# ApricityXX/PaddlePaddle

Hardware: AMD Instinct MI355X
Metric: tokens/sec GPT-3-13B sharding-3 + ResNet50 img/s, at 1/2/4/8 MI355X (higher is better)
Workload: dtype bf16; 1 GPU; model=GPT-3 13B (h5120 L40 a40 ffn20480 V50304), global_batch=16, seq_len=2048, micro_batch=4, accum_steps=4, parallelism=sharding_stage3_degree1, recompute=False, fused_head_ce=False, paired_wgrad=False, optimizer=AdamW fp32-master fused HIP, amp=O2 bf16, allocator=native auto-growth best-fit

## Files before the change

### csrc/dispatch/dispatch_gen.inc

```
PA_ENTRY(pa_rms_norm_fwd, "ippppllfip")
PA_ENTRY(pa_rms_norm_bwd, "ippppppllip")
PA_ENTRY(pa_rms_norm_bwd_res, "ipppppppllip")
PA_ENTRY(pa_layer_norm_fwd, "ippppppllfip")
PA_ENTRY(pa_layer_norm_bwd, "ipppppppppllip")
PA_ENTRY(pa_reduce_parts, "ippppiliip")
PA_ENTRY(pa_softmax_fwd, "ippllip")
PA_ENTRY(pa_softmax_bwd, "ipppllip")
PA_ENTRY(pa_softmax_ce_fwd, "ipppplllip")
PA_ENTRY(pa_softmax_ce_bwd, "ippppplllip")
PA_ENTRY(pa_ce_slice_fwd, "ipppplllip")
PA_ENTRY(pa_ce_slice_bwd, "ipppppllllip")
PA_ENTRY(pa_gelu_fwd, "ippliip")
PA_ENTRY(pa_gelu_bwd, "ipppliip")
PA_ENTRY(pa_swiglu_fwd, "ippplllip")
PA_ENTRY(pa_swiglu_bwd, "ippppplllip")
PA_ENTRY(pa_bias_gelu_fwd, "ipppllip")
PA_ENTRY(pa_rope_fwd, "ipppplllliip")
PA_ENTRY(pa_rope_rows, "iplpppllllliip")
PA_ENTRY(pa_adamw_multi, "ipplpfffffffpp")
PA_ENTRY(pa_adam_hyper_step, "ipffp")
PA_ENTRY(pa_sq_norm_multi, "ipplpp")
PA_ENTRY(pa_write_i64, "ipplp")
PA_ENTRY(pa_bn_set_target_wgs, "ii")
PA_ENTRY(pa_momentum_multi, "ipplpfffip")
PA_ENTRY(pa_multi_tensor_chunk, "l")
PA_ENTRY(pa_lamb_multi, "ipplplpppffffffip")
PA_ENTRY(pa_amp_check_unscale_multi, "ipplppp")
PA_ENTRY(pa_flash_attn_set_fwd_variant, "ii")
PA_ENTRY(pa_flash_attn_fwd, "ippppppiiiiiifip")
PA_ENTRY(pa_flash_attn_bwd, "ippppppppppppiiiiiifip")
PA_ENTRY(pa_flash_attn_fwd_ex, "ippppppiiiiiifipp")
PA_ENTRY(pa_flash_attn_bwd_ex, "ippppppppppppiiiiiifilpp")
PA_ENTRY(pa_flash_attn_bwd_ds, "ippppppppppppiiiiiifipp")
PA_ENTRY(pa_flash_attn_bwd_ds_ok, "iiiiii")
PA_ENTRY(pa_flash_attn_bwd_ds_bytes, "liiii")
PA_ENTRY(pa_fa_fm_stats, "ipiiiiillipp")
PA_ENTRY(pa_paged_decode_attn, "ippppppppiiiiiiillfp")
PA_ENTRY(pa_colsum, "ipppllip")
PA_ENTRY(pa_dwconv_fwd, "ipppppip")
PA_ENTRY(pa_dwconv_dgrad, "ipppppip")
PA_ENTRY(pa_dwconv_wgrad_parts, "ipp")
PA_ENTRY(pa_dwconv_wgrad, "ippppip")
PA_ENTRY(pa_gemm_bf16, "ippppplllllliiifiip")
PA_ENTRY(pa_gemm_bf16_pp, "ippppplllllliiifpp")
PA_ENTRY(pa_gemm_bf16_4w, "ippppplllllliiifpp")
PA_ENTRY(pa_gemm_bf16_res, "ippppplllllliipp")
PA_ENTRY(pa_gemm_bf16_dgelu, "ippppplllllliiip")
PA_ENTRY(pa_gemm_bf16_pp_segs, "ipiipppplllllliiifpp")
PA_ENTRY(pa_gemm_pp_ws_bytes, "llll")
PA_ENTRY(pa_gemm_pp_splitk_ws_bytes, "llli")
PA_ENTRY(pa_gemm_bf16_pp_splitk, "ippplllllliiifipp")
PA_ENTRY(pa_gemm_fp8, "ipppplllllliifiip")
PA_ENTRY(pa_gemm_fp8_set_kernel, "ii")
PA_ENTRY(pa_gemm_fp8_ws, "ipppplllllliifiipp")
PA_ENTRY(pa_gemm_fp8_ws_bytes, "llll")
PA_ENTRY(pa_gemm_fp8_dscale, "ipppplllllliifiipppp")
PA_ENTRY(pa_fp8_nparts, "l")
PA_ENTRY(pa_fp8_amax, "iplipp")
PA_ENTRY(pa_fp8_scale_update, "ipipippfiip")
PA_ENTRY(pa_fp8_quant, "iplliippppp")
PA_ENTRY(pa_gemm_bf16_4w_abl, "ippplllip")
PA_ENTRY(pa_gemm_small_m, "iplplplppiiiiip")
PA_ENTRY(pa_gemm_skinny, "ipppplllllliip")
PA_ENTRY(pa_wo_gemm, "ippppppppiiiiiiiip")
PA_ENTRY(pa_wo_gemm_splits, "illli")
PA_ENTRY(pa_wo_dequant, "ipppiiiip")
PA_ENTRY(pa_gemm_skinny_ok, "ill")
PA_ENTRY(pa_gemm_skinny_stats_chunks, "llll")
PA_ENTRY(pa_gemm_skinny_stats, "ippppllllllipp")
PA_ENTRY(pa_conv_skinny_stats_chunks, "llll")
PA_ENTRY(pa_conv_skinny_stats, "ippppplllpp")
PA_ENTRY(pa_conv_skinny, "ippppplllllllllllp")
PA_ENTRY(pa_conv_skinny_ok, "illll")
PA_ENTRY(pa_conv_skinny_wgrad, "ippppllllllp")
PA_ENTRY(pa_conv2d_nhwc_fwd, "ipppppiiiiiiiiiiiiip")
PA_ENTRY(pa_conv3d_ndhwc_fwd, "ipppppiiiiiiiiiiiiiiiiip")
PA_ENTRY(pa_conv2d_nhwc_fwd_stats, "ipppppiiiiiiiiiiiiipp")
PA_ENTRY(pa_gemm_stats_chunks, "ili")
PA_ENTRY(pa_slab_reduce_bf16, "ipplllip")
PA_ENTRY(pa_gemm_bf16_bnbwd, "ippplllllliiippppp")
PA_ENTRY(pa_conv2d_nhwc_fwd_bnbwd, "ippppiiiiiiiiiiiiippppp")
PA_ENTRY(pa_gemm_bf16_stats, "ipppplllllliiiipp")
PA_ENTRY(pa_conv2d_nhwc_wgrad, "ippppiiiiiiiiiiiiiiip")
PA_ENTRY(pa_bias_gelu_bwd, "ippppppllip")
PA_ENTRY(pa_dropout_add_fwd, "ippplfuip")
PA_ENTRY(pa_dropout_bwd, "ipplfuip")
PA_ENTRY(pa_dropout_bwd_colsum, "ipppllfuip")
PA_ENTRY(pa_colsum_nparts, "ll")
PA_ENTRY(pa_fold_partials, "ippllip")
PA_ENTRY(pa_bn_chunks, "ili")
PA_ENTRY(pa_bn_fwd_nhwc, "ipppppppppppliffiip")
PA_ENTRY(pa_bn_bwd_nhwc, "ippppppppppppliiipp")
PA_ENTRY(pa_bn_reduce_nhwc, "iipppppppliip")
PA_ENTRY(pa_bn_fwd_nhwc_mask, "ippppppppppppliffip")
PA_ENTRY(pa_bn_bwd_nhwc_mask, "ippppppppppppliip")
PA_ENTRY(pa_bn_bwd_apply_nhwc, "ippppppliipp")
PA_ENTRY(pa_bn_pre_ws, "lii")
PA_ENTRY(pa_bn_bwd_nhwc_pre, "ipppppppppippliipp")
PA_ENTRY(pa_bn_fwd_nhwc_pre, "ippppppppppipppliffip")
PA_ENTRY(pa_add_rms_norm_fwd, "ipppppllfip")
PA_ENTRY(pa_decode_rope_cache, "iplppppppiiiilip")
PA_ENTRY(pa_maxpool_nhwc_fwd, "ipppiiiiiiiiiip")
PA_ENTRY(pa_maxpool_nhwc_bwd, "ipppiiiiiiiiiip")
PA_ENTRY(pa_grouped_gemm, "iippppppiliiilllip")
PA_ENTRY(pa_moe_route, "ipiipppp")
PA_ENTRY(pa_version, "i")
```

### csrc/kernels/gemm.hip

```cpp
#include "common.h"
#include "gemm_plan.h"
#include "launch.h"
#include "mfma_tile.h"

#include <type_traits>

using namespace pa;

namespace {

constexpr int kBM = 256;
constexpr int kBK = 64;
constexpr int kThreads = 512;

enum EpiFlags : int {
  kEpiBias = 1,
  kEpiGelu = 2,
  kEpiAux = 4,
  kEpiAccum = 8,
  kEpiOutF32 = 16,
  kEpiStats = 32,
  kEpiStatsBwd = 64,
  kEpiGeluBwd = 128,
  kEpiColSum = 256,
// ... 246 lines not shown
#pragma unroll
    for (int i = 0; i < MR; ++i) {
      const int m = mrow0 + i * 16;
      if (m >= p.M) continue;
      float v[4];
#pragma unroll
      for (int e = 0; e < 4; ++e) v[e] = acc[i][j][e] * p.alpha + bv[e];
      const int64_t off = (int64_t)m * p.ldc + n;
      if (flags & kEpiAux) {
        *reinterpret_cast<uint2*>(p.aux + off) = make_uint2(pack_bf16(v[0], v[1]), pack_bf16(v[2], v[3]));
      }
      if (flags & kEpiGelu) {
#pragma unroll
        for (int e = 0; e < 4; ++e) v[e] = gelu_tanh(v[e]);
      }
      if (flags & kEpiOutF32) {
        float4* cp = reinterpret_cast<float4*>(reinterpret_cast<float*>(p.c) + off);
        if (flags & kEpiAccum) {
          const float4 o = *cp;
          v[0] += o.x; v[1] += o.y; v[2] += o.z; v[3] += o.w;
        }
        *cp = make_float4(v[0], v[1], v[2], v[3]);
      } else {
        uint2* cp = reinterpret_cast<uint2*>(reinterpret_cast<uint16_t*>(p.c) + off);
        if (flags & kEpiAccum) {
          const uint2 o = *cp;
          v[0] += lo_bf16(o.x); v[1] += hi_bf16(o.x); v[2] += lo_bf16(o.y); v[3] += hi_bf16(o.y);
        }
        const uint2 o = make_uint2(pack_bf16(v[0], v[1]), pack_bf16(v[2], v[3]));
        *cp = o;
        if (flags & kEpiStatsBwd) {
          stats_add_bwd(p, off, o, bsc, bsh, bmu, s1, s2);
        } else if (flags & kEpiStats) {
          stats_add2(o.x, s1, s2, 0);
          stats_add2(o.y, s1, s2, 2);
        }
      }
    }
    if (flags & kEpiStats) stats_store(p, tm * 2 + wm, p.tiles_m * 2, n, lane, s1, s2);
  }
}

constexpr int kEpiRowStride = 260;
constexpr int kEpiRowStrideBf16 = 264;

using H0_ = IntC<0>;
using H1_ = IntC<1>;
using H2_ = IntC<2>;
using H3_ = IntC<3>;
using True_ = IntC<1>;
using False_ = IntC<0>;

template <int NT>
__device__ __forceinline__ void epi_rows(const GemmArgs& p, const float* img, int m_base, int n0, int tid,
                                         const float* bv, float* cs) {
  constexpr int RS = kEpiRowStride;
  constexpr int RSTEP = NT / 32;
  constexpr int NSTEP = 128 / RSTEP;
  constexpr int G = 4;
  const int ec = (tid & 31) * 8, er = tid / 32;
  const int n = n0 + ec;
  if (n >= p.N) return;
  const int flags = p.flags;
  const bool f32 = flags & kEpiOutF32;
  const bool rd_pre = flags & kEpiGeluBwd, rd_res = (flags & kEpiResid) && !rd_pre;
  const bool rd_c = (flags & kEpiAccum) && !rd_pre && !rd_res;
#pragma unroll 1
  for (int g0 = 0; g0 < NSTEP; g0 += G) {
    uint4 rd[G][2];
    if (rd_pre || rd_res || rd_c) {
#pragma unroll
      for (int s = 0; s < G; ++s) {
        const int m = m_base + (g0 + s) * RSTEP + er;
        rd[s][0] = rd[s][1] = make_uint4(0u, 0u, 0u, 0u);
        if (m < p.M) {
          const int64_t off = (int64_t)m * p.ldc + n;
          if (rd_pre) {
            rd[s][0] = *reinterpret_cast<const uint4*>(p.aux + off);
          } else if (rd_res) {
            rd[s][0] = *reinterpret_cast<const uint4*>(p.res + off);
          } else if (f32) {
            rd[s][0] = *reinterpret_cast<const uint4*>(reinterpret_cast<const float*>(p.c) + off);
            rd[s][1] = *reinterpret_cast<const uint4*>(reinterpret_cast<const float*>(p.c) + off + 4);
          } else {
            rd[s][0] = *reinterpret_cast<const uint4*>(reinterpret_cast<const uint16_t*>(p.c) + off);
          }
        }
      }
    }
#pragma unroll
    for (int s = 0; s < G; ++s) {
      const int r = (g0 + s) * RSTEP + er;
      const int m = m_base + r;
      if (m >= p.M) break;
      float v[8];
      const f32x4 lo = *reinterpret_cast<const f32x4*>(img + r * RS + ec);
      const f32x4 hi = *reinterpret_cast<const f32x4*>(img + r * RS + ec + 4);
#pragma unroll
      for (int e = 0; e < 4; ++e) {
        v[e] = lo[e] * p.alpha + bv[e];
        v[4 + e] = hi[e] * p.alpha + bv[4 + e];
      }
      const int64_t off = (int64_t)m * p.ldc + n;
      if (flags & kEpiAux) store8<bf16>(reinterpret_cast<bf16*>(p.aux + off), v);
      if (flags & kEpiGelu) {
#pragma unroll
        for (int e = 0; e < 8; ++e) v[e] = gelu_tanh(v[e]);
      }
      float o[8];
      if (rd_pre || rd_res || (rd_c && !f32)) {
        const uint4 u = rd[s][0];
        o[0] = lo_bf16(u.x); o[1] = hi_bf16(u.x); o[2] = lo_bf16(u.y); o[3] = hi_bf16(u.y);
        o[4] = lo_bf16(u.z); o[5] = hi_bf16(u.z); o[6] = lo_bf16(u.w); o[7] = hi_bf16(u.w);
      } else if (rd_c) {
        const uint4 u0 = rd[s][0], u1 = rd[s][1];
        o[0] = __uint_as_float(u0.x); o[1] = __uint_as_float(u0.y); o[2] = __uint_as_float(u0.z);
        o[3] = __uint_as_float(u0.w); o[4] = __uint_as_float(u1.x); o[5] = __uint_as_float(u1.y);
        o[6] = __uint_as_float(u1.z); o[7] = __uint_as_float(u1.w);
      }
      if (rd_pre) {
#pragma unroll
        for (int e = 0; e < 8; ++e) v[e] *= gelu_tanh_grad_fast(o[e]);
      } else if (rd_c || rd_res) {
#pragma unroll
        for (int e = 0; e < 8; ++e) v[e] += o[e];
      }
      if (flags & kEpiColSum) {
#pragma unroll
        for (int e = 0; e < 8; ++e) cs[e] += v[e];
      }
      if (f32) store8<float>(reinterpret_cast<float*>(p.c) + off, v);
      else store8<bf16>(reinterpret_cast<bf16*>(reinterpret_cast<uint16_t*>(p.c) + off), v);
    }
  }
}

template <int NT>
__device__ __forceinline__ void colsum_finish(const GemmArgs& p, float* red, const float* cs, int tid, int m0,
                                              int n0) {
  constexpr int R = NT / 32;
  const int ec = (tid & 31) * 8, er = tid / 32;
  __syncthreads();
  *reinterpret_cast<float4*>(red + er * 256 + ec) = make_float4(cs[0], cs[1], cs[2], cs[3]);
  *reinterpret_cast<float4*>(red + er * 256 + ec + 4) = make_float4(cs[4], cs[5], cs[6], cs[7]);
  __syncthreads();
  for (int c = tid; c < 256; c += NT) {
    float s = 0.f;
#pragma unroll
    for (int r = 0; r < R; ++r) s += red[r * 256 + c];
    if (n0 + c < p.N) p.stats[(int64_t)(m0 >> 8) * p.N + n0 + c] = s;
  }
}

template <bool AK, bool BKM, int SEG = 0>
__global__ __launch_bounds__(kThreads, 1) void gemm256_kernel(GemmArgs p0) {
  GemmArgs p = split_view<AK, BKM>(p0);
  constexpr int HALF = 128 * kBK * 2;
  constexpr int STAGE = 4 * HALF;
  extern __shared__ __attribute__((aligned(16))) char smem[];

  const int tid = threadIdx.x, wave = tid >> 6, lane = tid & 63;
  const int wm = wave >> 2, wn = wave & 3;

  const int bid = (int)blockIdx.x;
  int pid;
  float* tail_out = nullptr;
  int kt0 = 0;
  if (p.tail_split > 0 && bid >= p.full_tiles) {
    const int u = bid - p.full_tiles;
    const int ks = u % p.tail_split;
    pid = p.full_tiles + u / p.tail_split;
    p.K /= p.tail_split;
    if constexpr (SEG == 0) {
      p.a += (int64_t)ks * p.K * (AK ? 1 : p.lda);
      p.b += (int64_t)ks * p.K * (BKM ? 1 : p.ldb);
    } else {
      kt0 = ks * (p.K / kBK);
    }
    tail_out = p.tail_ws + (int64_t)u * 65536;
  } else {
    pid = xcd_remap(bid, p.tail_split > 0 ? p.full_tiles : p.tiles_m * p.tiles_n);
  }
  int tm, tn;
  tile_coords(pid, p.tiles_m, p.tiles_n, &tm, &tn);
  const int m0 = tm * 256, n0 = tn * 256;
  const int nk = p.K / kBK;

  auto stage_half = [&](int t, int h, char* dst) {
    const int tg = SEG == 0 ? t : kt0 + t;
    int k0 = tg * kBK;
    const uint16_t* a = p.a;
    const uint16_t* b = p.b;
    int64_t lda = p.lda, ldb = p.ldb;
    if constexpr (SEG == 1) {
      const int s = seg_of(p, tg);
      k0 = (tg - pick4(s, 0, p.seg_end[0], p.seg_end[1], p.seg_end[2])) * kBK;
      a = pick4(s, p.seg_a[0], p.seg_a[1], p.seg_a[2], p.seg_a[3]);
      b = pick4(s, p.seg_b[0], p.seg_b[1], p.seg_b[2], p.seg_b[3]);
      lda = pick4(s, p.seg_lda[0], p.seg_lda[1], p.seg_lda[2], p.seg_lda[3]);
      ldb = pick4(s, p.seg_ldb[0], p.seg_ldb[1], p.seg_ldb[2], p.seg_ldb[3]);
    }
    if (h == 0 || h == 2) {
      stage<128, AK>(a, lda, m0 + (h == 2 ? 128 : 0), p.M, k0, dst, wave, lane);
    } else {
      int c0 = n0 + (h == 3 ? 128 : 0), cmax = p.N;
      if constexpr (SEG == 2) {
        const int s = seg_of(p, c0);
        const int start = pick4(s, 0, p.seg_end[0], p.seg_end[1], p.seg_end[2]);
        b = pick4(s, p.seg_b[0], p.seg_b[1], p.seg_b[2], p.seg_b[3]);
        ldb = pick4(s, p.seg_ldb[0], p.seg_ldb[1], p.seg_ldb[2], p.seg_ldb[3]);
        cmax = pick4(s, p.seg_end[0], p.seg_end[1], p.seg_end[2], p.seg_end[3]) - start;
        c0 -= start;
      }
      stage<128, BKM>(b, ldb, c0, cmax, k0, dst, wave, lane);
    }
  };
  auto issue = [&](int j) {
    const int t = j >> 2, h = j & 3;
    stage_half(t, h, smem + (t & 1) * STAGE + h * HALF);
  };
  auto issue_h = [&](int t, auto hc) {
    constexpr int h = decltype(hc)::value;
    stage_half(t, h, smem + (t & 1) * STAGE + h * HALF);
  };

  f32x4 acc[2][4][2][2];
#pragma unroll
  for (int a = 0; a < 2; ++a)
#pragma unroll
    for (int i = 0; i < 4; ++i)
#pragma unroll
      for (int b = 0; b < 2; ++b)
#pragma unroll
        for (int j = 0; j < 2; ++j) acc[a][i][b][j] = f32x4{0.f, 0.f, 0.f, 0.f};

  const int last_j = 4 * nk - 1;
  auto wait_for = [&](int phase, int jstar) {
    const int issued = min(phase + 6, last_j);
    vm_wait(2 * max(issued - jstar, 0));
  };
  const int npro = min(6, 4 * nk);
#pragma unroll 1
  for (int j = 0; j < npro; ++j) issue(j);
  vm_wait(2 * max(min(5, last_j) - 1, 0));
  bar();
  const bool lag = __builtin_amdgcn_readfirstlane(wm) == 1;
  if (lag) bar();

  bf16x8_t af[4][2], bl[2][2], br[2][2];
  const int ar = wm * 64, bc = wn * 32;

  auto ktile = [&](int t, auto steady) {
    constexpr bool S = decltype(steady)::value;
    const char* buf = smem + (t & 1) * STAGE;
    const int ph = 4 * t;
#pragma unroll
    for (int ks = 0; ks < 2; ++ks)
#pragma unroll
      for (int j = 0; j < 2; ++j) bl[j][ks] = frag<128, BKM>(buf + HALF, bc + j * 16, ks, lane);
#pragma unroll
    for (int ks = 0; ks < 2; ++ks)
#pragma unroll
      for (int i = 0; i < 4; ++i) af[i][ks] = frag<128, AK>(buf, ar + i * 16, ks, lane);
    if (S) {
      issue_h(t + 1, H2_{});
      asm volatile("s_waitcnt vmcnt(6)" ::: "memory");
    } else {
      if (ph + 6 <= last_j) issue(ph + 6);
      wait_for(ph, ph + 3);
    }
    bar();
    __builtin_amdgcn_s_setprio(1);
#pragma unroll
    for (int ks = 0; ks < 2; ++ks)
#pragma unroll
      for (int i = 0; i < 4; ++i)
#pragma unroll
        for (int j = 0; j < 2; ++j)
          acc[0][i][0][j] = __builtin_amdgcn_mfma_f32_16x16x32_bf16(bl[j][ks], af[i][ks], acc[0][i][0][j], 0, 0, 0);
    __builtin_amdgcn_s_setprio(0);
    bar();
#pragma unroll
    for (int ks = 0; ks < 2; ++ks)
#pragma unroll
      for (int j = 0; j < 2; ++j) br[j][ks] = frag<128, BKM>(buf + 3 * HALF, bc + j * 16, ks, lane);
    if (S) {
      issue_h(t + 1, H3_{});
      asm volatile("s_waitcnt vmcnt(10)" ::: "memory");
    } else {
      if (ph + 7 <= last_j) issue(ph + 7);
      wait_for(ph + 1, ph + 2);
    }
    bar();
    __builtin_amdgcn_s_setprio(1);
#pragma unroll
    for (int ks = 0; ks < 2; ++ks)
#pragma unroll
      for (int i = 0; i < 4; ++i)
#pragma unroll
        for (int j = 0; j < 2; ++j)
          acc[0][i][1][j] = __builtin_amdgcn_mfma_f32_16x16x32_bf16(br[j][ks], af[i][ks], acc[0][i][1][j], 0, 0, 0);
    __builtin_amdgcn_s_setprio(0);
    bar();
#pragma unroll
    for (int ks = 0; ks < 2; ++ks)
#pragma unroll
      for (int i = 0; i < 4; ++i) af[i][ks] = frag<128, AK>(buf + 2 * HALF, ar + i * 16, ks, lane);
    if (S) issue_h(t + 2, H0_{});
    else if (ph + 8 <= last_j) issue(ph + 8);
    bar();
    __builtin_amdgcn_s_setprio(1);
#pragma unroll
    for (int ks = 0; ks < 2; ++ks)
#pragma unroll
      for (int i = 0; i < 4; ++i)
#pragma unroll
        for (int j = 0; j < 2; ++j)
          acc[1][i][0][j] = __builtin_amdgcn_mfma_f32_16x16x32_bf16(bl[j][ks], af[i][ks], acc[1][i][0][j], 0, 0, 0);
    __builtin_amdgcn_s_setprio(0);
    bar();
    if (S) {
// ... 409 lines not shown
    const uint16_t* src =
        ok ? p.a + ((int64_t)(cr.pix[i] + (di * p.cH + hi) * p.cW + wi) * p.cC + c0 + lc * 8) : p.zero + lc * 8;
    glds16(src, img + q * 1024);
  }
}

template <bool AK, bool BKM, bool CONV = false>
__global__ __launch_bounds__(kThreads, 1) void gemm3s_kernel(GemmArgs p0) {
  const GemmArgs p = split_view<AK, BKM>(p0);
  constexpr int BN = kBN3;
  constexpr int A_BYTES = kBM * kBK * 2;
  constexpr int B_BYTES = BN * kBK * 2;
  constexpr int STAGE = A_BYTES + B_BYTES;
  constexpr int MR = 4, NR = 5;
  constexpr int NL = (kBM / 8 + 7) / 8 + (BN / 8 + 7) / 8;
  extern __shared__ __attribute__((aligned(16))) char smem[];

  const int tid = threadIdx.x, wave = tid >> 6, lane = tid & 63;
  const int wm = wave >> 1, wn = wave & 1;

  const int nwg = p.tiles_m * p.tiles_n;
  const int pid = xcd_remap((int)blockIdx.x, nwg);
  constexpr int GM = 8;
  const int per_group = GM * p.tiles_n;
  const int gid = pid / per_group;
  const int first_m = gid * GM;
  const int gsz = min(p.tiles_m - first_m, GM);
  const int tm = first_m + (pid % per_group) % gsz;
  const int tn = (pid % per_group) / gsz;
  const int m0 = tm * kBM, n0 = tn * BN;

  f32x4 acc[MR][NR];
#pragma unroll
  for (int i = 0; i < MR; ++i)
#pragma unroll
    for (int j = 0; j < NR; ++j) acc[i][j] = f32x4{0.f, 0.f, 0.f, 0.f};

  const int nk = p.K / kBK;
  ConvRows cr;
  if constexpr (CONV) cr = conv_rows(p, m0, wave, lane);
  auto stage_tile = [&](int t) {
    char* base = smem + (t % 3) * STAGE;
    if constexpr (CONV) stage_conv(p, cr, t * kBK, base, wave, lane);
    else stage_r<kBM, AK>(p.a, p.lda, m0, p.M, t * kBK, base, wave, lane);
    stage_r<BN, BKM>(p.b, p.ldb, n0, p.N, t * kBK, base + A_BYTES, wave, lane);
  };

  stage_tile(0);
  if (nk > 1) {
    stage_tile(1);
    asm volatile("s_waitcnt vmcnt(%0)" ::"n"(NL) : "memory");
  } else {
    asm volatile("s_waitcnt vmcnt(0)" ::: "memory");
  }
  bar();

#pragma unroll 1
  for (int t = 0; t < nk; ++t) {
    const bool pre = t + 2 < nk;
    if (pre) stage_tile(t + 2);
    const char* aimg = smem + (t % 3) * STAGE;
    const char* bimg = aimg + A_BYTES;
#pragma unroll
    for (int s = 0; s < 2; ++s) {
      bf16x8_t bf[NR];
#pragma unroll
      for (int j = 0; j < NR; ++j) bf[j] = frag_r<BN, BKM>(bimg, wn * 80 + j * 16, s, lane);
#pragma unroll
      for (int i = 0; i < MR; ++i) {
        const bf16x8_t af = frag_r<kBM, AK>(aimg, wm * 64 + i * 16, s, lane);
#pragma unroll
        for (int j = 0; j < NR; ++j)
          acc[i][j] = __builtin_amdgcn_mfma_f32_16x16x32_bf16(bf[j], af, acc[i][j], 0, 0, 0);
      }
    }
    if (pre) asm volatile("s_waitcnt vmcnt(%0)" ::"n"(NL) : "memory");
    else asm volatile("s_waitcnt vmcnt(0)" ::: "memory");
    bar();
  }

  const int flags = p.flags;
  const int mrow0 = m0 + wm * 64 + (lane & 15);
  const int ncol0 = n0 + wn * 80 + 4 * (lane >> 4);
#pragma unroll
  for (int j = 0; j < NR; ++j) {
    const int n = ncol0 + j * 16;
    if (n >= p.N) continue;
    float s1[4] = {0.f, 0.f, 0.f, 0.f}, s2[4] = {0.f, 0.f, 0.f, 0.f};
    float bsc[4] = {0.f, 0.f, 0.f, 0.f}, bsh[4] = {0.f, 0.f, 0.f, 0.f}, bmu[4] = {0.f, 0.f, 0.f, 0.f};
    if (flags & kEpiStatsBwd) bn_cols(p, n, bsc, bsh, bmu);
    float bv[4] = {0.f, 0.f, 0.f, 0.f};
    if (flags & kEpiBias) {
      const uint2 braw = *reinterpret_cast<const uint2*>(p.bias + n);
      bv[0] = lo_bf16(braw.x); bv[1] = hi_bf16(braw.x); bv[2] = lo_bf16(braw.y); bv[3] = hi_bf16(braw.y);
    }
#pragma unroll
    for (int i = 0; i < MR; ++i) {
      const int m = mrow0 + i * 16;
      if (m >= p.M) continue;
      float v[4];
#pragma unroll
      for (int e = 0; e < 4; ++e) v[e] = acc[i][j][e] * p.alpha + bv[e];
      const int64_t off = (int64_t)m * p.ldc + n;
      if (flags & kEpiAux)
        *reinterpret_cast<uint2*>(p.aux + off) = make_uint2(pack_bf16(v[0], v[1]), pack_bf16(v[2], v[3]));
      if (flags & kEpiGelu) {
#pragma unroll
        for (int e = 0; e < 4; ++e) v[e] = gelu_tanh(v[e]);
      }
      if (flags & kEpiOutF32) {
        float4* cp = reinterpret_cast<float4*>(reinterpret_cast<float*>(p.c) + off);
        if (flags & kEpiAccum) {
          const float4 o = *cp;
          v[0] += o.x; v[1] += o.y; v[2] += o.z; v[3] += o.w;
        }
        *cp = make_float4(v[0], v[1], v[2], v[3]);
      } else {
        uint2* cp = reinterpret_cast<uint2*>(reinterpret_cast<uint16_t*>(p.c) + off);
        if (flags & kEpiAccum) {
          const uint2 o = *cp;
          v[0] += lo_bf16(o.x); v[1] += hi_bf16(o.x); v[2] += lo_bf16(o.y); v[3] += hi_bf16(o.y);
        }
        const uint2 o = make_uint2(pack_bf16(v[0], v[1]), pack_bf16(v[2], v[3]));
        *cp = o;
        if (flags & kEpiStatsBwd) {
          stats_add_bwd(p, off, o, bsc, bsh, bmu, s1, s2);
        } else if (flags & kEpiStats) {
          stats_add2(o.x, s1, s2, 0);
          stats_add2(o.y, s1, s2, 2);
        }
      }
    }
    if (flags & kEpiStats) stats_store(p, tm * 4 + wm, p.tiles_m * 4, n, lane, s1, s2);
  }
}


template <class F>
int with_layout(int a_kmajor, int b_kmajor, F&& f) {
  if (a_kmajor && !b_kmajor) return f(std::true_type{}, std::false_type{});
  if (a_kmajor && b_kmajor) return f(std::true_type{}, std::true_type{});
  if (!a_kmajor && !b_kmajor) return f(std::false_type{}, std::false_type{});
  return f(std::false_type{}, std::true_type{});
}

template <bool AK, bool BKM, bool CONV = false>
int launch3s(GemmArgs a, int splits, hipStream_t st) {
  a.tiles_m = (a.M + kBM - 1) / kBM;
  a.tiles_n = (a.N + kBN3 - 1) / kBN3;
  constexpr int smem = 3 * (kBM + kBN3) * kBK * 2;
  return launch_lds<gemm3s_kernel<AK, BKM, CONV>>(dim3(a.tiles_m * a.tiles_n, splits), dim3(kThreads), smem, st, a);
}

template <bool AK, bool BKM, int SEG>
int launch256_seg(GemmArgs a, int splits, hipStream_t st, int grid) {
  a.tiles_m = (a.M + 255) / 256;
  a.tiles_n = (a.N + 255) / 256;
  if (!grid) {
    grid = a.tiles_m * a.tiles_n;
    a.tail_split = 0;
  }
  constexpr int kLoop = 2 * 4 * 128 * kBK * 2, kEpi0 = 128 * kEpiRowStride * 4, kEpi1 = 256 * kEpiRowStrideBf16 * 2;
  constexpr int kEpi = kEpi0 > kEpi1 ? kEpi0 : kEpi1;
  constexpr int smem = kLoop > kEpi ? kLoop : kEpi;
  return launch_lds<gemm256_kernel<AK, BKM, SEG>>(dim3(grid, splits), dim3(kThreads), smem, st, a);
}

template <bool AK, bool BKM>
int launch256(const GemmArgs& a0, int splits, hipStream_t st, int grid = 0, int seg = 0) {
  if (seg == 1) return launch256_seg<AK, BKM, 1>(a0, splits, st, grid);
  if (seg == 2) return launch256_seg<AK, BKM, 2>(a0, splits, st, grid);
  return launch256_seg<AK, BKM, 0>(a0, splits, st, grid);
}

template <bool AK, bool BKM>
int launch4w(const GemmArgs& g, int grid, hipStream_t st) {
  constexpr int kLoop = 4 * 2 * 256 * 32 * 2, kEpi = 128 * kEpiRowStride * 4;
  constexpr int smem = kLoop > kEpi ? kLoop : kEpi;
  return launch_lds<gemm4w_kernel<AK, BKM>>(dim3(grid), dim3(256), smem, st, g);
}

template <int BN, bool AK, bool BKM>
int launch(const GemmArgs& a0, int splits, hipStream_t st) {
  if constexpr (BN == 0) return launch256<AK, BKM>(a0, splits, st);
  if constexpr (BN == 160) return launch3s<AK, BKM>(a0, splits, st);
  GemmArgs a = a0;
  constexpr int NW = BN == 4 ? 4 : 8;
  constexpr int BNk = (BN == 0 || BN == 4) ? 256 : BN;
  a.tiles_m = (a.M + kBM - 1) / kBM;
  a.tiles_n = (a.N + BNk - 1) / BNk;
  constexpr int smem = 2 * (kBM + BNk) * kBK * 2;
  return launch_lds<gemm_bf16_kernel<BNk, AK, BKM, NW>>(dim3(a.tiles_m * a.tiles_n, splits), dim3(NW * 64), smem, st,
                                                        a);
}

int launch_bn(const GemmArgs& g, int bn, int a_kmajor, int b_kmajor, int splits, hipStream_t st) {
  return with_layout(a_kmajor, b_kmajor, [&](auto ak, auto bk) {
    constexpr bool AK = decltype(ak)::value, BKM = decltype(bk)::value;
    if (bn == 160) return launch<160, AK, BKM>(g, splits, st);
    if (bn == 128) return launch<128, AK, BKM>(g, splits, st);
    if (bn == 1) return launch<0, AK, BKM>(g, splits, st);
    if (bn == 4) return launch<4, AK, BKM>(g, splits, st);
    return launch<256, AK, BKM>(g, splits, st);
  });
}

constexpr int kSmBM = 64, kSmBN = 128, kSmNW = 4;

template <int kSmStages>
__global__ __launch_bounds__(kSmNW * 64, 1) void gemm_small_m_kernel(const uint16_t* __restrict__ a, int64_t lda,
                                                                    const uint16_t* __restrict__ b, int64_t ldb,
                                                                    float* __restrict__ ws, int M, int N, int k_per,
                                                                    const uint16_t* __restrict__ bias,
                                                                    uint16_t* __restrict__ c, int64_t ldc) {
  constexpr int A_BYTES = kSmBM * kBK * 2, B_BYTES = kSmBN * kBK * 2, STAGE = A_BYTES + B_BYTES;
  constexpr int NL = kSmBM / (8 * kSmNW) + kSmBN / (8 * kSmNW);
  extern __shared__ __attribute__((aligned(16))) char smem[];
  const int tid = threadIdx.x, wave = tid >> 6, lane = tid & 63;
  const int n0 = blockIdx.x * kSmBN;
  const int ks = blockIdx.y;
  const uint16_t* ap = a + (int64_t)ks * k_per;
  const uint16_t* bp = b + (int64_t)ks * k_per * ldb;
  const int nk = k_per / kBK;

  f32x4 acc[4][2];
#pragma unroll
  for (int i = 0; i < 4; ++i) acc[i][0] = acc[i][1] = f32x4{0.f, 0.f, 0.f, 0.f};

  auto stage_tile = [&](int t) {
    char* base = smem + (t % kSmStages) * STAGE;
    stage<kSmBM, true, kSmNW>(ap, lda, 0, M, t * kBK, base, wave, lane);
    stage<kSmBN, false, kSmNW>(bp, ldb, n0, N, t * kBK, base + A_BYTES, wave, lane);
  };
  const int pro = min(kSmStages - 1, nk);
  for (int t = 0; t < pro; ++t) stage_tile(t);
  if (pro >= 3) asm volatile("s_waitcnt vmcnt(%0)" ::"n"(2 * NL) : "memory");
  else if (pro == 2) asm volatile("s_waitcnt vmcnt(%0)" ::"n"(NL) : "memory");
  else asm volatile("s_waitcnt vmcnt(0)" ::: "memory");
  bar();

#pragma unroll 1
  for (int t = 0; t < nk; ++t) {
    if (t + kSmStages - 1 < nk) stage_tile(t + kSmStages - 1);
    const char* aimg = smem + (t % kSmStages) * STAGE;
    const char* bimg = aimg + A_BYTES;
#pragma unroll
    for (int s = 0; s < 2; ++s) {
      bf16x8_t bf[2];
#pragma unroll
      for (int j = 0; j < 2; ++j) bf[j] = frag<kSmBN, false>(bimg, wave * 32 + j * 16, s, lane);
#pragma unroll
      for (int i = 0; i < 4; ++i) {
        const bf16x8_t af = frag<kSmBM, true>(aimg, i * 16, s, lane);
#pragma unroll
        for (int j = 0; j < 2; ++j) acc[i][j] = __builtin_amdgcn_mfma_f32_16x16x32_bf16(bf[j], af, acc[i][j], 0, 0, 0);
      }
    }
    const int after = min(nk - 1, t + kSmStages - 1) - (t + 1);
    if (after >= 2) asm volatile("s_waitcnt vmcnt(%0)" ::"n"(2 * NL) : "memory");
    else if (after == 1) asm volatile("s_waitcnt vmcnt(%0)" ::"n"(NL) : "memory");
    else asm volatile("s_waitcnt vmcnt(0)" ::: "memory");
    bar();
  }
  if (gridDim.y == 1) {
#pragma unroll
    for (int i = 0; i < 4; ++i) {
      const int m = i * 16 + (lane & 15);
      if (m >= M) continue;
#pragma unroll
      for (int j = 0; j < 2; ++j) {
        const int n = n0 + wave * 32 + j * 16 + 4 * (lane >> 4);
        if (n >= N) continue;
        float v[4] = {acc[i][j][0], acc[i][j][1], acc[i][j][2], acc[i][j][3]};
        if (bias) {
          const uint2 braw = *reinterpret_cast<const uint2*>(bias + n);
          v[0] += lo_bf16(braw.x); v[1] += hi_bf16(braw.x); v[2] += lo_bf16(braw.y); v[3] += hi_bf16(braw.y);
        }
        *reinterpret_cast<uint2*>(c + (int64_t)m * ldc + n) = make_uint2(pack_bf16(v[0], v[1]), pack_bf16(v[2], v[3]));
      }
    }
    return;
  }
  float* out = ws + (int64_t)ks * M * N;
#pragma unroll
  for (int i = 0; i < 4; ++i) {
    const int m = i * 16 + (lane & 15);
    if (m >= M) continue;
#pragma unroll
    for (int j = 0; j < 2; ++j) {
      const int n = n0 + wave * 32 + j * 16 + 4 * (lane >> 4);
      if (n < N)
        *reinterpret_cast<float4*>(out + (int64_t)m * N + n) =
            make_float4(acc[i][j][0], acc[i][j][1], acc[i][j][2], acc[i][j][3]);
    }
  }
}

__global__ __launch_bounds__(256) void gemm_small_m_reduce_k(const float* __restrict__ ws, const uint16_t* __restrict__ bias,
                                                            uint16_t* __restrict__ c, int64_t ldc, int M, int N,
                                                            int splits) {
  const int64_t i4 = ((int64_t)blockIdx.x * 256 + threadIdx.x) * 4;
  if (i4 >= (int64_t)M * N) return;
  const int m = (int)(i4 / N), n = (int)(i4 % N);
  float4 acc = *reinterpret_cast<const float4*>(ws + i4);
  for (int s = 1; s < splits; ++s) {
    const float4 v = *reinterpret_cast<const float4*>(ws + (int64_t)s * M * N + i4);
    acc.x += v.x; acc.y += v.y; acc.z += v.z; acc.w += v.w;
  }
  if (bias) {
    const uint2 braw = *reinterpret_cast<const uint2*>(bias + n);
    acc.x += lo_bf16(braw.x); acc.y += hi_bf16(braw.x); acc.z += lo_bf16(braw.y); acc.w += hi_bf16(braw.y);
  }
  *reinterpret_cast<uint2*>(c + (int64_t)m * ldc + n) = make_uint2(pack_bf16(acc.x, acc.y), pack_bf16(acc.z, acc.w));
}

__global__ __launch_bounds__(256) void gemm_tail_reduce_k(GemmArgs p) {
  const int b = blockIdx.x;
  int tm, tn;
  tile_coords(p.full_tiles + b, p.tiles_m, p.tiles_n, &tm, &tn);
  const int e = (blockIdx.y * 256 + threadIdx.x) * 4;
  const int r = e >> 8, c = e & 255;
  const int m = tm * 256 + r, n = tn * 256 + c;
  if (m >= p.M || n >= p.N) return;
  const float* src = p.tail_ws + (int64_t)b * p.tail_split * 65536 + e;
  float4 a = *reinterpret_cast<const float4*>(src);
  for (int k = 1; k < p.tail_split; ++k) {
    const float4 v = *reinterpret_cast<const float4*>(src + (int64_t)k * 65536);
    a.x += v.x; a.y += v.y; a.z += v.z; a.w += v.w;
  }
  const int flags = p.flags;
  float bv[4] = {0.f, 0.f, 0.f, 0.f};
  if (flags & kEpiBias) {
    const uint2 braw = *reinterpret_cast<const uint2*>(p.bias + n);
    bv[0] = lo_bf16(braw.x); bv[1] = hi_bf16(braw.x); bv[2] = lo_bf16(braw.y); bv[3] = hi_bf16(braw.y);
  }
  float v[4] = {a.x * p.alpha + bv[0], a.y * p.alpha + bv[1], a.z * p.alpha + bv[2], a.w * p.alpha + bv[3]};
  const int64_t off = (int64_t)m * p.ldc + n;
  if (flags & kEpiAux)
    *reinterpret_cast<uint2*>(p.aux + off) = make_uint2(pack_bf16(v[0], v[1]), pack_bf16(v[2], v[3]));
  if (flags & kEpiGelu) {
#pragma unroll
    for (int q = 0; q < 4; ++q) v[q] = gelu_tanh(v[q]);
  }
  if (flags & kEpiResid) {
    const uint2 rr = *reinterpret_cast<const uint2*>(p.res + off);
    v[0] += lo_bf16(rr.x); v[1] += hi_bf16(rr.x); v[2] += lo_bf16(rr.y); v[3] += hi_bf16(rr.y);
  }
  if (flags & kEpiOutF32) {
    float4* cp = reinterpret_cast<float4*>(reinterpret_cast<float*>(p.c) + off);
    if (flags & kEpiAccum) {
      const float4 o = *cp;
      v[0] += o.x; v[1] += o.y; v[2] += o.z; v[3] += o.w;
    }
    *cp = make_float4(v[0], v[1], v[2], v[3]);
  } else {
    uint2* cp = reinterpret_cast<uint2*>(reinterpret_cast<uint16_t*>(p.c) + off);
    if (flags & kEpiAccum) {
      const uint2 o = *cp;
      v[0] += lo_bf16(o.x); v[1] += hi_bf16(o.x); v[2] += lo_bf16(o.y); v[3] += hi_bf16(o.y);
    }
    *cp = make_uint2(pack_bf16(v[0], v[1]), pack_bf16(v[2], v[3]));
  }
}

bool gemm_args(GemmArgs& g, const void* a, const void* b, void* c, const void* bias, void* aux, int64_t M, int64_t N,
               int64_t K, int64_t lda, int64_t ldb, int64_t ldc, int a_kmajor, int flags, float alpha) {
  if (!gemm_operands_ok(M, N, K, kBK, lda, ldb, ldc, a_kmajor != 0)) return false;
  g = GemmArgs{};
  g.a = (const uint16_t*)a; g.b = (const uint16_t*)b; g.c = c;
  g.bias = (const uint16_t*)bias; g.aux = (uint16_t*)aux;
  g.lda = lda; g.ldb = ldb; g.ldc = ldc;
  g.M = (int)M; g.N = (int)N; g.K = (int)K;
  g.flags = flags; g.alpha = alpha;
  return true;
}

void set_conv_geometry(GemmArgs& g, const void* zero, int D, int H, int W, int C, int Do, int Ho, int Wo, int KH,
                       int KW, int stride, int pad_d, int pad_h, int pad_w, int dil) {
  g.zero = (const uint16_t*)zero;
  g.cD = D; g.cDo = Do; g.cKHW = KH * KW; g.cPadD = pad_d;
  g.cH = H; g.cW = W; g.cC = C; g.cHo = Ho; g.cWo = Wo; g.cKW = KW; g.cStride = stride; g.cPadH = pad_h;
  g.cPadW = pad_w; g.cDil = dil;
}

int run_tile256(int kern, GemmArgs g, int a_kmajor, int b_kmajor, void* ws, hipStream_t st, int seg = 0,
                int force_split = 0) {
  if (g.M <= 0 || g.N <= 0 || g.K <= 0) return 0;
  TailPlan pl = force_split ? split_all_plan(g.M, g.N, force_split) : tail_plan(g.M, g.N, g.K, kBK, device_cus());
  if (!ws) pl = without_tail(pl);
  if (!force_split) g.c_split = (int64_t)g.M * g.ldc;
  g.tiles_m = (g.M + 255) / 256;
  g.tiles_n = (g.N + 255) / 256;
  g.full_tiles = pl.full_tiles;
  g.tail_split = pl.split;
  g.tail_ws = (float*)ws;
  const int rc = with_layout(a_kmajor, b_kmajor, [&](auto ak, auto bk) {
    constexpr bool AK = decltype(ak)::value, BKM = decltype(bk)::value;
    return kern == 2 ? launch4w<AK, BKM>(g, pl.grid, st) : launch256<AK, BKM>(g, 1, st, pl.grid, seg);
  });
  if (rc || !pl.split) return rc;
  hipLaunchKernelGGL(gemm_tail_reduce_k, dim3(pl.tiles - pl.full_tiles, 64), dim3(256), 0, st, g);
  return (int)hipGetLastError();
}

bool conv_fwd_args(GemmArgs& g, const void* x, const void* w, const void* bias, void* out, const void* zero, int N,
                   int D, int H, int W, int C, int Cout, int KD, int KH, int KW, int stride, int pad_d, int pad_h,
                   int pad_w, int dil, int Do, int Ho, int Wo, int flags) {
  if (C % kBK != 0 || Cout % 8 != 0 || N <= 0) return false;
  const int64_t K = (int64_t)KD * KH * KW * C;
  if (!gemm_args(g, x, w, out, bias, nullptr, (int64_t)N * Do * Ho * Wo, Cout, K, C, K, Cout, 1,
                 flags | (bias ? kEpiBias : 0), 1.f))
    return false;
  set_conv_geometry(g, zero, D, H, W, C, Do, Ho, Wo, KH, KW, stride, pad_d, pad_h, pad_w, dil);
  return true;
}

}

PA_EXPORT int64_t pa_gemm_pp_ws_bytes(int64_t M, int64_t N, int64_t K) {
  return tail_plan(M, N, K, kBK, device_cus()).ws_bytes;
}

PA_EXPORT int pa_gemm_bf16_pp(const void* a, const void* b, void* c, const void* bias, void* aux, int64_t M, int64_t N,
                              int64_t K, int64_t lda, int64_t ldb, int64_t ldc, int a_kmajor, int b_kmajor, int flags,
                              float alpha, void* ws, hipStream_t st) {
  GemmArgs g;
  if (!gemm_args(g, a, b, c, bias, aux, M, N, K, lda, ldb, ldc, a_kmajor, flags, alpha)) return 1;
  return run_tile256(1, g, a_kmajor, b_kmajor, ws, st);
}

PA_EXPORT int64_t pa_gemm_pp_splitk_ws_bytes(int64_t M, int64_t N, int splits) {
  return split_all_plan(M, N, splits).ws_bytes;
}

PA_EXPORT int pa_gemm_bf16_pp_splitk(const void* a, const void* b, void* c, int64_t M, int64_t N, int64_t K,
                                     int64_t lda, int64_t ldb, int64_t ldc, int a_kmajor, int b_kmajor, int flags,
                                     float alpha, int splits, void* ws, hipStream_t st) {
  if (splits < 1 || (K / kBK) % splits != 0 || !ws || (flags & ~(kEpiOutF32 | kEpiAccum))) return 1;
  GemmArgs g;
  if (!gemm_args(g, a, b, c, nullptr, nullptr, M, N, K, lda, ldb, ldc, a_kmajor, flags, alpha)) return 1;
  return run_tile256(1, g, a_kmajor, b_kmajor, ws, st, 0, splits);
}

PA_EXPORT int pa_gemm_bf16_pp_segs(const int64_t* seg, int nseg, int seg_k, const void* a, const void* b, void* c,
                                   const void* bias, int64_t M, int64_t N, int64_t K, int64_t lda, int64_t ldb,
                                   int64_t ldc, int a_kmajor, int b_kmajor, int flags, float alpha, void* ws,
                                   hipStream_t st) {
  if (nseg < 1 || nseg > 4 || (flags & (kEpiAux | kEpiStats))) return 1;
  GemmArgs g;
  if (!gemm_args(g, a, b, c, bias, nullptr, M, N, K, 0, 0, ldc, a_kmajor, flags, alpha)) return 1;
  if (M <= 0 || N <= 0) return 0;
  if (seg_k ? (flags & kEpiBias) != 0 : lda % 8 != 0) return 1;
  g.lda = lda; g.ldb = ldb;
  g.nseg = nseg; g.seg_k = seg_k;
  int64_t prev = 0;
  for (int s = 0; s < 4; ++s) {
    const int64_t* e = seg + 5 * (s < nseg ? s : nseg - 1);
    g.seg_a[s] = (const uint16_t*)e[0];
    g.seg_b[s] = (const uint16_t*)e[1];
    g.seg_lda[s] = e[2];
    g.seg_ldb[s] = e[3];
    if (s < nseg) {
      const int64_t end = e[4];
      if (end <= prev || e[2] % 8 != 0 || e[3] % 8 != 0) return 1;
      if (seg_k ? (end % kBK != 0) : (end % 128 != 0 && s + 1 < nseg)) return 1;
      g.seg_end[s] = (int)(seg_k ? end / kBK : end);
      prev = end;
    } else {
      g.seg_end[s] = g.seg_end[nseg - 1];
    }
  }
  if (seg_k ? prev != K : prev != N) return 1;
  return run_tile256(1, g, a_kmajor, b_kmajor, ws, st, nseg > 1 ? (seg_k ? 1 : 2) : 0);
}

PA_EXPORT int pa_gemm_bf16_4w(const void* a, const void* b, void* c, const void* bias, void* aux, int64_t M, int64_t N,
                              int64_t K, int64_t lda, int64_t ldb, int64_t ldc, int a_kmajor, int b_kmajor, int flags,
                              float alpha, void* ws, hipStream_t st) {
  GemmArgs g;
  if (!gemm_args(g, a, b, c, bias, aux, M, N, K, lda, ldb, ldc, a_kmajor, flags, alpha)) return 1;
  return run_tile256(2, g, a_kmajor, b_kmajor, ws, st);
}

PA_EXPORT int pa_gemm_bf16_res(const void* a, const void* b, void* c, const void* bias, const void* res, int64_t M,
                               int64_t N, int64_t K, int64_t lda, int64_t ldb, int64_t ldc, int a_kmajor, int b_kmajor,
                               void* ws, hipStream_t st) {
  if (!res || res == c) return 1;
  GemmArgs g;
  if (!gemm_args(g, a, b, c, bias, nullptr, M, N, K, lda, ldb, ldc, a_kmajor, (bias ? kEpiBias : 0) | kEpiResid, 1.f))
    return 1;
  g.res = (const uint16_t*)res;
  return run_tile256(1, g, a_kmajor, b_kmajor, ws, st);
}

PA_EXPORT int pa_gemm_bf16_dgelu(const void* a, const void* b, void* dh, const void* pre, float* colsum, int64_t M,
                                 int64_t N, int64_t K, int64_t lda, int64_t ldb, int64_t ldc, int a_kmajor,
                                 int b_kmajor, int kern, hipStream_t st) {
  if (!pre || !colsum || kern < 1 || kern > 2) return 1;
  GemmArgs g;
  if (!gemm_args(g, a, b, dh, nullptr, const_cast<void*>(pre), M, N, K, lda, ldb, ldc, a_kmajor,
                 kEpiGeluBwd | kEpiColSum, 1.f))
    return 1;
  g.stats = colsum;
  return run_tile256(kern, g, a_kmajor, b_kmajor, nullptr, st);
}

PA_EXPORT int pa_gemm_bf16_4w_abl(const void* a, const void* b, void* c, int64_t M, int64_t N, int64_t K, int abl,
                                  hipStream_t st) {
  GemmArgs g;
  if (N % 256 || M % 256 || !gemm_args(g, a, b, c, nullptr, nullptr, M, N, K, K, N, N, 1, 0, 1.f)) return 1;
  g.tiles_m = (int)(M / 256); g.tiles_n = (int)(N / 256);
  g.full_tiles = g.tiles_m * g.tiles_n;
  if (abl >= 6 && abl <= 8) {
    if (abl != 7) g.lda = 0;
    if (abl != 8) g.ldb = 0;
  }
  constexpr int smem = 128 * kEpiRowStride * 4;
  const dim3 grid(g.full_tiles), block(256);
  if (abl == 1) return launch_lds<gemm4w_kernel<true, false, 1>>(grid, block, smem, st, g);
  if (abl == 2) return launch_lds<gemm4w_kernel<true, false, 2>>(grid, block, smem, st, g);
  if (abl == 3) return launch_lds<gemm4w_kernel<true, false, 3>>(grid, block, smem, st, g);
  if (abl == 5) return launch_lds<gemm4w_kernel<true, false, 5>>(grid, block, smem, st, g);
  if (abl == 4) return launch_lds<gemm4w_kernel<true, false, 0, 5>>(grid, block, 5 * 32768, st, g);
  return launch_lds<gemm4w_kernel<true, false, 0>>(grid, block, smem, st, g);
}

PA_EXPORT int pa_gemm_bf16(const void* a, const void* b, void* c, const void* bias, void* aux, int64_t M, int64_t N,
                           int64_t K, int64_t lda, int64_t ldb, int64_t ldc, int a_kmajor, int b_kmajor, int flags,
                           float alpha, int bn, int splits, hipStream_t st) {
  if (splits < 1) splits = 1;
  if (K % splits != 0) return 1;
  if (splits > 1 && (flags & (kEpiBias | kEpiGelu | kEpiAux | kEpiAccum))) return 1;
  if (splits > 1 && !(flags & kEpiOutF32)) return 1;
  GemmArgs g;
  if (!gemm_args(g, a, b, c, bias, aux, M, N, K / splits, lda, ldb, ldc, a_kmajor, flags, alpha)) return 1;
  if (M <= 0 || N <= 0 || K <= 0) return 0;
  g.c_split = M * ldc;
  return launch_bn(g, bn, a_kmajor, b_kmajor, splits, st);
}

PA_EXPORT int pa_conv3d_ndhwc_fwd(const void* x, const void* w, const void* bias, void* out, const void* zero, int N,
                                  int D, int H, int W, int C, int Cout, int KD, int KH, int KW, int stride, int pad_d,
                                  int pad_h, int pad_w, int dil, int Do, int Ho, int Wo, hipStream_t st) {
  GemmArgs g;
  if (!conv_fwd_args(g, x, w, bias, out, zero, N, D, H, W, C, Cout, KD, KH, KW, stride, pad_d, pad_h, pad_w, dil, Do,
                     Ho, Wo, 0))
    return 1;
  return launch3s<true, true, true>(g, 1, st);
}

PA_EXPORT int pa_gemm_stats_chunks(int64_t M, int bn) { return (int)((M + kBM - 1) / kBM) * (bn == 160 ? 4 : 2); }

PA_EXPORT int pa_gemm_bf16_stats(const void* a, const void* b, void* c, const void* bias, int64_t M, int64_t N,
                                 int64_t K, int64_t lda, int64_t ldb, int64_t ldc, int a_kmajor, int b_kmajor,
                                 int flags, int bn, float* stats, hipStream_t st) {
  if (!stats || (flags & (kEpiOutF32 | kEpiGelu | kEpiAux))) return 1;
  if (bn != 160 && bn != 256 && bn != 128 && bn != 4) return 1;
  GemmArgs g;
  if (!gemm_args(g, a, b, c, bias, nullptr, M, N, K, lda, ldb, ldc, a_kmajor, flags | kEpiStats, 1.f)) return 1;
  if (M <= 0 || N <= 0 || K <= 0) return 0;
  g.c_split = M * ldc;
  g.stats = stats;
  return launch_bn(g, bn, a_kmajor, b_kmajor, 1, st);
}

PA_EXPORT int pa_gemm_bf16_bnbwd(const void* a, const void* b, void* c, int64_t M, int64_t N, int64_t K, int64_t lda,
                                 int64_t ldb, int64_t ldc, int a_kmajor, int b_kmajor, int bn, const void* bn_x,
                                 const float* bn_ss, const float* bn_mean, float* stats, hipStream_t st) {
  if (!stats || !bn_x || !bn_ss || !bn_mean) return 1;
  if (bn != 160 && bn != 256 && bn != 128 && bn != 4) return 1;
  GemmArgs g;
  if (!gemm_args(g, a, b, c, nullptr, nullptr, M, N, K, lda, ldb, ldc, a_kmajor, kEpiStats | kEpiStatsBwd, 1.f))
    return 1;
  if (M <= 0 || N <= 0 || K <= 0) return 0;
  g.c_split = M * ldc;
  g.stats = stats;
  g.bn_x = (const uint16_t*)bn_x; g.bn_ss = bn_ss; g.bn_mean = bn_mean;
  return launch_bn(g, bn, a_kmajor, b_kmajor, 1, st);
}

PA_EXPORT int pa_conv2d_nhwc_fwd(const void* x, const void* w, const void* bias, void* out, const void* zero, int N,
// ... 117 lines not shown
```

### csrc/kernels/gemm_plan.h

```cpp
#pragma once
#include <climits>
#include <cstdint>

namespace pa {

struct TailPlan {
  int tiles, full_tiles, split, grid;
  int64_t ws_bytes;
};

inline TailPlan make_tail_plan(int64_t tiles, int64_t full, int split) {
  const int64_t tail = split ? tiles - full : 0;
  return {(int)tiles, (int)(tiles - tail), split, (int)(tiles - tail + tail * split), tail * split * 65536 * 4};
}

inline int64_t tiles256(int64_t M, int64_t N) { return ((M + 255) / 256) * ((N + 255) / 256); }

inline TailPlan tail_plan(int64_t M, int64_t N, int64_t K, int k_tile, int cus) {
  const int64_t T = tiles256(M, N);
  const int64_t nk = K / k_tile;
  const int64_t r = T > cus ? T % cus : 0;
  if (r == 0 || 2 * r > cus) return make_tail_plan(T, T, 0);
  int sp = 1;
  while (r * sp * 2 <= cus && nk % (sp * 2) == 0 && nk / (sp * 2) >= 4) sp *= 2;
  return sp == 1 ? make_tail_plan(T, T, 0) : make_tail_plan(T, T - r, sp);
}

inline TailPlan split_all_plan(int64_t M, int64_t N, int splits) { return make_tail_plan(tiles256(M, N), 0, splits); }

inline TailPlan without_tail(const TailPlan& p) { return make_tail_plan(p.tiles, p.tiles, 0); }

inline bool gemm_operands_ok(int64_t M, int64_t N, int64_t K, int k_tile, int64_t lda, int64_t ldb, int64_t ldc,
                             bool a_kmajor) {
  if (M > INT_MAX || N > INT_MAX || K > INT_MAX) return false;
  if (K % k_tile != 0 || N % 8 != 0 || lda % 8 != 0 || ldb % 8 != 0 || ldc % 4 != 0) return false;
  return a_kmajor || M % 8 == 0;
}

}
```

### csrc/kernels/mfma_tile.h

```cpp
#pragma once
#include "common.h"

namespace pa {

typedef __attribute__((ext_vector_type(8))) __bf16 bf16x8_t;
typedef __attribute__((ext_vector_type(4))) float f32x4;
typedef __attribute__((ext_vector_type(4))) short s16x4;
typedef __attribute__((ext_vector_type(4))) int i32x4;
typedef __attribute__((ext_vector_type(4))) unsigned int u32x4;

union Frag8 {
  bf16x8_t v;
  uint4 u;
  u32x4 w;
  s16x4 h[2];
};

__device__ __forceinline__ void glds16(const void* g, const char* lds_wave_base) {
  const uint32_t m0 = __builtin_amdgcn_readfirstlane((uint32_t)reinterpret_cast<uintptr_t>(lds_wave_base));
  asm volatile("s_mov_b32 m0, %1\n\ts_nop 0\n\tglobal_load_lds_dwordx4 %0, off" ::"v"(g), "s"(m0) : "memory", "m0");
}
__device__ __forceinline__ void glds4(const void* g, const char* lds_wave_base) {
  const uint32_t m0 = __builtin_amdgcn_readfirstlane((uint32_t)reinterpret_cast<uintptr_t>(lds_wave_base));
  asm volatile("s_mov_b32 m0, %1\n\ts_nop 0\n\tglobal_load_lds_dword %0, off" ::"v"(g), "s"(m0) : "memory", "m0");
}

__device__ __forceinline__ s16x4 lds_tr(const char* p) {
  return __builtin_amdgcn_ds_read_tr16_b64_v4i16(
      (__attribute__((address_space(3))) s16x4*)(reinterpret_cast<uintptr_t>(p)));
}

__device__ __forceinline__ void bar() {
  asm volatile("" ::: "memory");
  __builtin_amdgcn_s_barrier();
  asm volatile("" ::: "memory");
  __builtin_amdgcn_sched_barrier(0);
}

__device__ __forceinline__ void vm_wait(int n) {
  switch (n) {
    case 0: asm volatile("s_waitcnt vmcnt(0)" ::: "memory"); break;
    case 2: asm volatile("s_waitcnt vmcnt(2)" ::: "memory"); break;
    case 4: asm volatile("s_waitcnt vmcnt(4)" ::: "memory"); break;
    case 6: asm volatile("s_waitcnt vmcnt(6)" ::: "memory"); break;
    case 8: asm volatile("s_waitcnt vmcnt(8)" ::: "memory"); break;
    case 10: asm volatile("s_waitcnt vmcnt(10)" ::: "memory"); break;
    default: asm volatile("s_waitcnt vmcnt(0)" ::: "memory"); break;
  }
}

constexpr __host__ __device__ __forceinline__ int k_swz(int row) { return (row >> 1) & 7; }
constexpr __host__ __device__ __forceinline__ int k32_swz(int row) { return ((row >> 3) & 1) << 1; }
constexpr __host__ __device__ __forceinline__ int mn_swz(int k) { return ((k & 3) | (((k >> 3) & 1) << 2)) << 1; }
template <int R>
constexpr __host__ __device__ __forceinline__ int mn_swz_r(int k) { return mn_swz(k) & (R / 8 - 1); }

template <int R>
constexpr bool mn_swz_ok() {
  for (int k = 0; k < 64; ++k) {
    const int s = mn_swz_r<R>(k);
    if (s % 2 != 0 || (R >= 128 && s != mn_swz(k))) return false;
    for (int c = 0; c < R / 8; ++c)
      if ((c ^ s) >= R / 8) return false;
  }
  return true;
}
static_assert(mn_swz_ok<64>() && mn_swz_ok<128>() && mn_swz_ok<256>(), "MN-major swizzle");

template <int R, bool KMAJ, int NW = 8, class T>
__device__ __forceinline__ void stage(const T* __restrict__ g, int64_t ld, int r0, int rmax, int k0, char* img,
                                      int wave, int lane) {
  constexpr int E = 16 / sizeof(T);
  constexpr int NQ = R / (8 * NW);
  static_assert(KMAJ || sizeof(T) == 2, "MN-major images hold 16-bit elements");
#pragma unroll
  for (int i = 0; i < NQ; ++i) {
    const int q = i * NW + wave;
    if constexpr (KMAJ) {
      const int row = q * 8 + (lane >> 3);
      const int lc = (lane & 7) ^ k_swz(row);
      int gr = r0 + row;
      gr = gr < rmax ? gr : rmax - 1;
      glds16(g + (int64_t)gr * ld + k0 + lc * E, img + q * 1024);
    } else {
      constexpr int CPR = R / 8;
      const int lin = q * 64 + lane;
      const int row = lin / CPR;
      const int lc = (lin % CPR) ^ mn_swz_r<R>(row);
      int gc = r0 + lc * 8;
      gc = gc < rmax ? gc : rmax - 8;
      glds16(g + (int64_t)(k0 + row) * ld + gc, img + q * 1024);
    }
  }
}

template <int R, bool KMAJ>
__device__ __forceinline__ bf16x8_t frag(const char* img, int rbase, int s, int lane) {
  Frag8 f;
  if constexpr (KMAJ) {
    const int row = rbase + (lane & 15);
    const int c = s * 4 + (lane >> 4);
    f.u = *reinterpret_cast<const uint4*>(img + row * 128 + ((c ^ k_swz(row)) << 4));
  } else {
    const int g = lane >> 4, i = lane & 15, q = i >> 2, pp = i & 3;
    const int col = rbase + pp * 4;
    const int lc = col >> 3, sub = (col & 7) * 2;
    const int k1 = s * 32 + g * 8 + q, k2 = k1 + 4;
    f.h[0] = lds_tr(img + k1 * (R * 2) + ((lc ^ mn_swz_r<R>(k1)) << 4) + sub);
    f.h[1] = lds_tr(img + k2 * (R * 2) + ((lc ^ mn_swz_r<R>(k2)) << 4) + sub);
  }
  return f.v;
}

__device__ __forceinline__ int xcd_remap(int bid, int nwg) {
  const int xcd = bid & 7, q = nwg >> 3, r = nwg & 7;
  return (xcd < r ? xcd * (q + 1) : r * (q + 1) + (xcd - r) * q) + (bid >> 3);
}

__device__ __forceinline__ void tile_coords(int pid, int tiles_m, int tiles_n, int* tm, int* tn) {
  constexpr int GM = 8;
  const int per_group = GM * tiles_n;
  const int first_m = (pid / per_group) * GM;
  const int gsz = min(tiles_m - first_m, GM);
  *tm = first_m + (pid % per_group) % gsz;
  *tn = (pid % per_group) / gsz;
}

template <int V>
struct IntC {
  static constexpr int value = V;
};

}
```

### csrc/kernels/pa_api.h

```cpp
#pragma once
#include <cstdint>

#include <hip/hip_runtime_api.h>

#define PA_EXPORT extern "C" __attribute__((visibility("default")))

struct PaAttnExtra {
  const int* cu_q; const int* cu_k;
  const void* mask; int64_t mask_kind; int64_t ms[3];
  const int* fm; int64_t fm_cols; int64_t fms[2];
  const int* fm_stats; int64_t fmst[2];
  double drop_p; uint64_t seed;
  int64_t lse_s[2];
  int64_t dtype;
};

PA_EXPORT int pa_gelu_fwd(const void* x, void* y, int64_t n, int approx, int dtype, hipStream_t st);
PA_EXPORT int pa_gelu_bwd(const void* x, const void* dy, void* dx, int64_t n, int approx, int dtype, hipStream_t st);
PA_EXPORT int pa_bias_gelu_fwd(const void* x, const void* b, void* y, int64_t rows, int64_t cols, int dtype,
                               hipStream_t st);
PA_EXPORT int pa_swiglu_fwd(const void* a, const void* b, void* y, int64_t rows, int64_t cols, int64_t ld, int dtype,
                            hipStream_t st);
PA_EXPORT int pa_swiglu_bwd(const void* a, const void* b, const void* dy, void* da, void* db, int64_t rows,
                            int64_t cols, int64_t ld_packed, int dtype, hipStream_t st);
PA_EXPORT int pa_rope_fwd(const void* x, const float* cs, const float* sn, void* out, int64_t B, int64_t S, int64_t H,
                          int64_t D, int flags, int dtype, hipStream_t st);
PA_EXPORT int pa_rope_rows(const void* x, int64_t ldx, const float* cs, const float* sn, void* out, int64_t ldo,
                           int64_t rows, int64_t S, int64_t NH, int64_t D, int flags, int dtype, hipStream_t st);

PA_EXPORT int64_t pa_multi_tensor_chunk();
PA_EXPORT int pa_adamw_multi(const int64_t* table, const int64_t* items, int64_t n_items, const float* inv_scale,
                             float lr, float b1, float b2, float eps, float wd_unused, float bc1, float bc2,
                             const float* hyper, hipStream_t st);
PA_EXPORT int pa_adam_hyper_step(float* hyper, float b1, float b2, hipStream_t st);
PA_EXPORT int pa_sq_norm_multi(const int64_t* table, const int64_t* items, int64_t n_items, float* partial,
                               hipStream_t st);
PA_EXPORT int pa_momentum_multi(const int64_t* table, const int64_t* items, int64_t n_items, const float* inv_scale,
                                float lr, float mu, float rescale, int nesterov, hipStream_t st);
PA_EXPORT int pa_write_i64(int64_t* dst, const int64_t* src, int64_t n, hipStream_t st);

PA_EXPORT int pa_amp_check_unscale_multi(const int64_t* table, const int64_t* items, int64_t n_items,
                                         const float* inv_scale, float* found_inf, hipStream_t st);

PA_EXPORT int pa_bn_set_target_wgs(int n);
PA_EXPORT int pa_bn_chunks(int64_t R, int C);
PA_EXPORT int pa_bn_fwd_nhwc(const void* x, const void* res, void* y, const float* w, const float* b, float* run_mean,
                             float* run_var, float* save_mean, float* save_rstd, float* partial, float* ss, int64_t R,
                             int C, float momentum, float eps, int relu, int training, hipStream_t st);
PA_EXPORT int pa_bn_bwd_nhwc(const void* dy, const void* x, const void* y, void* dx, void* dres, const float* w,
                             const float* mean, const float* rstd, float* dw, float* db, float* partial, float* coef,
                             int64_t R, int C, int relu, int global_stats, const float* ss, hipStream_t st);
PA_EXPORT int pa_bn_fwd_nhwc_mask(const void* x, const void* res, void* y, const float* w, const float* b,
                                  float* run_mean, float* run_var, float* save_mean, float* save_rstd, float* partial,
                                  float* ss, void* mbits, int64_t R, int C, float momentum, float eps, int training,
                                  hipStream_t st);
PA_EXPORT int pa_bn_bwd_nhwc_mask(const void* dy, const void* x, const void* mbits, void* dx, void* dres,
                                  const float* w, const float* mean, const float* rstd, float* dw, float* db,
                                  float* partial, float* coef, int64_t R, int C, int global_stats, hipStream_t st);
PA_EXPORT int64_t pa_bn_pre_ws(int chunks, int C);
PA_EXPORT int pa_bn_fwd_nhwc_pre(const void* x, const void* res, void* y, const float* w, const float* b,
                                 float* run_mean, float* run_var, float* save_mean, float* save_rstd,
                                 const float* stats, int chunks, float* ws, float* ss, void* mbits, int64_t R, int C,
                                 float momentum, float eps, int relu, hipStream_t st);
PA_EXPORT int pa_bn_bwd_nhwc_pre(const void* dy, const void* x, void* dx, const float* w, const float* mean,
                                 const float* rstd, float* dw, float* db, const float* stats, int chunks, float* ws,
                                 float* coef, int64_t R, int C, int global_stats, const float* ss, hipStream_t st);
PA_EXPORT int pa_bn_reduce_nhwc(int mode, const void* x, const void* dy, const void* y, const float* mean,
                                const float* ss, float* partial, float* sums, int64_t R, int C, int relu,
                                hipStream_t st);
PA_EXPORT int pa_bn_bwd_apply_nhwc(const void* dy, const void* x, const void* y, const float* coef, void* dx,
                                   void* dres, int64_t R, int C, int relu, const float* ss, hipStream_t st);

PA_EXPORT int pa_paged_decode_attn(const void* q, const void* kc, const void* vc, const int* tables, const int* lens,
                                   float* part_o, float* part_ml, void* out, int N, int H, int Hkv, int D, int bs,
                                   int max_blocks, int splits, int64_t blk_stride, int64_t head_stride, float scale,
                                   hipStream_t st);

PA_EXPORT int pa_add_rms_norm_fwd(const void* x, const void* r, const void* w, void* s_out, void* y, int64_t rows,
                                  int64_t cols, float eps, int dtype, hipStream_t st);
PA_EXPORT int pa_decode_rope_cache(const void* qkv, int64_t ld, const float* cs, const float* sn, const int64_t* pos,
                                   void* q_out, void* kc, void* vc, int B, int H, int Hkv, int D, int64_t Lc,
                                   int dtype, hipStream_t st);

PA_EXPORT int pa_dwconv_fwd(const void* x, const void* wt, const void* bias, void* y, const int* shape, int dtype,
                            hipStream_t st);
PA_EXPORT int pa_dwconv_dgrad(const void* dy, const void* wt, const void* x, void* dx, const int* shape, int dtype,
                              hipStream_t st);
PA_EXPORT int pa_dwconv_wgrad_parts(const int* shape, int* out );
PA_EXPORT int pa_dwconv_wgrad(const void* x, const void* dy, float* part, const int* shape, int dtype,
                              hipStream_t st);

PA_EXPORT int pa_flash_attn_set_fwd_variant(int v);
PA_EXPORT int pa_flash_attn_fwd_ex(const void* q, const void* k, const void* v, void* o, float* lse,
                                   const int64_t* strides, int B, int Sq, int Sk, int H, int Hk, int D, float scale,
                                   int causal, const PaAttnExtra* ex, hipStream_t st);
PA_EXPORT int pa_flash_attn_fwd(const void* q, const void* k, const void* v, void* o, float* lse,
                                const int64_t* strides, int B, int Sq, int Sk, int H, int Hk, int D, float scale,
                                int causal, hipStream_t st);
PA_EXPORT int pa_flash_attn_bwd_ds_ok(int D, int has_mask, int has_fm, int dropout, int varlen);
PA_EXPORT int pa_flash_attn_bwd_ex(const void* q, const void* k, const void* v, const void* o, const void* dout,
                                   const float* lse, void* dq, void* dk, void* dv, float* dq_acc, float* delta,
                                   const int64_t* strides, int B, int Sq, int Sk, int H, int Hk, int D, float scale,
                                   int causal, int64_t q_rows, const PaAttnExtra* ex, hipStream_t st);
PA_EXPORT int64_t pa_flash_attn_bwd_ds_bytes(int B, int Sq, int Sk, int H);
PA_EXPORT int pa_flash_attn_bwd_ds(const void* q, const void* k, const void* v, const void* o, const void* dout,
                                   const float* lse, void* dq, void* dk, void* dv, void* ds, float* delta,
                                   const int64_t* strides, int B, int Sq, int Sk, int H, int Hk, int D, float scale,
                                   int causal, const PaAttnExtra* ex, hipStream_t st);
PA_EXPORT int pa_flash_attn_bwd(const void* q, const void* k, const void* v, const void* o, const void* dout,
                                const float* lse, void* dq, void* dk, void* dv, float* dq_acc, float* delta,
                                const int64_t* strides, int B, int Sq, int Sk, int H, int Hk, int D, float scale,
                                int causal, hipStream_t st);
PA_EXPORT int pa_fa_fm_stats(const int* fm, int cols, int causal, int Sk, int Bm, int Hm, int64_t sb, int64_t sh,
                             int ntiles, int* stats, hipStream_t st);

PA_EXPORT int64_t pa_gemm_pp_ws_bytes(int64_t M, int64_t N, int64_t K);
PA_EXPORT int pa_gemm_bf16_pp(const void* a, const void* b, void* c, const void* bias, void* aux, int64_t M,
                              int64_t N, int64_t K, int64_t lda, int64_t ldb, int64_t ldc, int a_kmajor, int b_kmajor,
                              int flags, float alpha, void* ws, hipStream_t st);
PA_EXPORT int64_t pa_gemm_pp_splitk_ws_bytes(int64_t M, int64_t N, int splits);
PA_EXPORT int pa_gemm_bf16_pp_splitk(const void* a, const void* b, void* c, int64_t M, int64_t N, int64_t K,
                                     int64_t lda, int64_t ldb, int64_t ldc, int a_kmajor, int b_kmajor, int flags,
                                     float alpha, int splits, void* ws, hipStream_t st);
PA_EXPORT int pa_gemm_bf16_pp_segs(const int64_t* seg, int nseg, int seg_k, const void* a, const void* b, void* c,
                                   const void* bias, int64_t M, int64_t N, int64_t K, int64_t lda, int64_t ldb,
                                   int64_t ldc, int a_kmajor, int b_kmajor, int flags, float alpha, void* ws,
                                   hipStream_t st);
PA_EXPORT int pa_gemm_bf16_4w(const void* a, const void* b, void* c, const void* bias, void* aux, int64_t M,
                              int64_t N, int64_t K, int64_t lda, int64_t ldb, int64_t ldc, int a_kmajor, int b_kmajor,
                              int flags, float alpha, void* ws, hipStream_t st);
PA_EXPORT int pa_gemm_bf16_res(const void* a, const void* b, void* c, const void* bias, const void* res, int64_t M,
                               int64_t N, int64_t K, int64_t lda, int64_t ldb, int64_t ldc, int a_kmajor,
                               int b_kmajor, void* ws, hipStream_t st);
PA_EXPORT int pa_gemm_bf16_dgelu(const void* a, const void* b, void* dh, const void* pre, float* colsum, int64_t M,
                                 int64_t N, int64_t K, int64_t lda, int64_t ldb, int64_t ldc, int a_kmajor,
                                 int b_kmajor, int kern, hipStream_t st);
PA_EXPORT int pa_gemm_bf16_4w_abl(const void* a, const void* b, void* c, int64_t M, int64_t N, int64_t K, int abl,
                                  hipStream_t st);
PA_EXPORT int pa_gemm_bf16(const void* a, const void* b, void* c, const void* bias, void* aux, int64_t M, int64_t N,
                           int64_t K, int64_t lda, int64_t ldb, int64_t ldc, int a_kmajor, int b_kmajor, int flags,
                           float alpha, int bn, int splits, hipStream_t st);
PA_EXPORT int pa_conv3d_ndhwc_fwd(const void* x, const void* w, const void* bias, void* out, const void* zero, int N,
                                  int D, int H, int W, int C, int Cout, int KD, int KH, int KW, int stride, int pad_d,
                                  int pad_h, int pad_w, int dil, int Do, int Ho, int Wo, hipStream_t st);
PA_EXPORT int pa_gemm_stats_chunks(int64_t M, int bn);
PA_EXPORT int pa_gemm_bf16_stats(const void* a, const void* b, void* c, const void* bias, int64_t M, int64_t N,
                                 int64_t K, int64_t lda, int64_t ldb, int64_t ldc, int a_kmajor, int b_kmajor,
                                 int flags, int bn, float* stats, hipStream_t st);
PA_EXPORT int pa_gemm_bf16_bnbwd(const void* a, const void* b, void* c, int64_t M, int64_t N, int64_t K, int64_t lda,
                                 int64_t ldb, int64_t ldc, int a_kmajor, int b_kmajor, int bn, const void* bn_x,
                                 const float* bn_ss, const float* bn_mean, float* stats, hipStream_t st);
PA_EXPORT int pa_conv2d_nhwc_fwd(const void* x, const void* w, const void* bias, void* out, const void* zero, int N,
                                 int H, int W, int C, int Cout, int KH, int KW, int stride, int pad_h, int pad_w,
                                 int dil, int Ho, int Wo, hipStream_t st);
PA_EXPORT int pa_conv2d_nhwc_fwd_stats(const void* x, const void* w, const void* bias, void* out, const void* zero,
                                       int N, int H, int W, int C, int Cout, int KH, int KW, int stride, int pad_h,
                                       int pad_w, int dil, int Ho, int Wo, float* stats, hipStream_t st);
PA_EXPORT int pa_conv2d_nhwc_fwd_bnbwd(const void* x, const void* w, void* out, const void* zero, int N, int H, int W,
                                       int C, int Cout, int KH, int KW, int stride, int pad_h, int pad_w, int dil,
                                       int Ho, int Wo, const void* bn_x, const float* bn_ss, const float* bn_mean,
                                       float* stats, hipStream_t st);
PA_EXPORT int pa_conv2d_nhwc_wgrad(const void* x, const void* dy, float* ws, const void* zero, int N, int H, int W,
                                   int C, int Cout, int KH, int KW, int stride, int pad_h, int pad_w, int dil, int Ho,
                                   int Wo, int splits, int bn, hipStream_t st);
PA_EXPORT int pa_gemm_small_m(const void* a, int64_t lda, const void* b, int64_t ldb, void* c, int64_t ldc,
                              const void* bias, float* ws, int M, int N, int K, int splits, int stages,
                              hipStream_t st);
PA_EXPORT int pa_slab_reduce_bf16(const float* ws, void* c, int64_t ldc, int64_t M, int64_t N, int splits,
                                  hipStream_t st);

PA_EXPORT int64_t pa_gemm_fp8_ws_bytes(int64_t M, int64_t N, int64_t K);
PA_EXPORT int pa_gemm_fp8(const void* a, const void* b, void* c, const void* bias, int64_t M, int64_t N, int64_t K,
                          int64_t lda, int64_t ldb, int64_t ldc, int fmt_a, int fmt_b, float alpha, int act,
                          int out_f16, hipStream_t st);
PA_EXPORT int pa_gemm_fp8_ws(const void* a, const void* b, void* c, const void* bias, int64_t M, int64_t N, int64_t K,
                             int64_t lda, int64_t ldb, int64_t ldc, int fmt_a, int fmt_b, float alpha, int act,
                             int out_f16, void* ws, hipStream_t st);
PA_EXPORT int pa_gemm_fp8_dscale(const void* a, const void* b, void* c, const void* bias, int64_t M, int64_t N,
                                 int64_t K, int64_t lda, int64_t ldb, int64_t ldc, int fmt_a, int fmt_b, float alpha,
                                 int act, int out_f16, void* ws, const float* a_scale_inv, const float* b_scale_inv,
                                 hipStream_t st);
PA_EXPORT int pa_gemm_fp8_set_kernel(int k);

PA_EXPORT int pa_gemm_skinny_ok(int64_t N, int64_t K);
PA_EXPORT int pa_gemm_skinny(const void* a, const void* b, void* c, const void* bias, int64_t M, int64_t N, int64_t K,
                             int64_t lda, int64_t ldb, int64_t ldc, int b_kmajor, int flags, void* stream);
PA_EXPORT int64_t pa_gemm_skinny_stats_chunks(int64_t M, int64_t N, int64_t K);
PA_EXPORT int pa_gemm_skinny_stats(const void* a, const void* b, void* c, const void* bias, int64_t M, int64_t N,
                                   int64_t K, int64_t lda, int64_t ldb, int64_t ldc, int b_kmajor, float* stats,
                                   void* stream);
PA_EXPORT int pa_conv_skinny_ok(int64_t C, int64_t Cout, int64_t KH, int64_t KW);
PA_EXPORT int pa_conv_skinny(const void* x, const void* w, const void* bias, void* y, const void* zero_page,
                             int64_t N, int64_t H, int64_t W, int64_t C, int64_t Cout, int64_t KH, int64_t KW,
                             int64_t stride, int64_t pad, int64_t Ho, int64_t Wo, void* stream);
PA_EXPORT int64_t pa_conv_skinny_stats_chunks(int64_t N, int64_t H, int64_t W);
PA_EXPORT int pa_conv_skinny_stats(const void* x, const void* w, const void* bias, void* y, const void* zero_page,
                                   int64_t N, int64_t H, int64_t W, float* stats, void* stream);
PA_EXPORT int pa_conv_skinny_wgrad(const void* x, const void* dy, const void* zero_page, float* ws, int64_t N,
                                   int64_t H, int64_t W, int64_t C, int64_t Cout, int64_t splits, void* stream);

PA_EXPORT int pa_grouped_gemm(int mode, const void* a, const void* b, void* c, const void* bias, const int* offs,
                              const void* zero, int E, int64_t rows, int M, int N, int K, int64_t lda, int64_t ldb,
                              int64_t ldc, int flags, hipStream_t st);
PA_EXPORT int pa_moe_route(const int* eid, int n, int E, int* counts, int* offs, int* perm, hipStream_t st);

PA_EXPORT int pa_lamb_multi(const int64_t* table, const int64_t* items, int64_t n_items, const int64_t* offsets,
                            int64_t n_tensors, float* partial, float* trust, const float* inv_scale, float lr,
                            float b1, float b2, float eps, float bc1, float bc2, int always_adapt, hipStream_t st);

PA_EXPORT int pa_colsum(const void* x, void* out, float* ws, int64_t rows, int64_t cols, int dtype_acc,
                        hipStream_t st);
PA_EXPORT int pa_bias_gelu_bwd(const void* h, const void* b, const void* dy, void* dh, void* db, float* ws,
                               int64_t rows, int64_t cols, int dtype_acc, hipStream_t st);
PA_EXPORT int pa_dropout_add_fwd(const void* x, const void* res, void* out, int64_t n, float p, uint64_t seed,
                                 int dtype, hipStream_t st);
PA_EXPORT int pa_dropout_bwd(const void* dy, void* dx, int64_t n, float p, uint64_t seed, int dtype, hipStream_t st);
PA_EXPORT int pa_dropout_bwd_colsum(const void* dy, void* dx, float* ws, int64_t rows, int64_t cols, float p,
                                    uint64_t seed, int dtype, hipStream_t st);
PA_EXPORT int64_t pa_colsum_nparts(int64_t rows);
PA_EXPORT int pa_fold_partials(const float* ws, void* out, int64_t cols, int64_t nparts, int dtype_acc,
                               hipStream_t st);

PA_EXPORT int pa_rms_norm_fwd(const void* x, const void* w, void* y, float* rstd, int64_t rows, int64_t cols,
                              float eps, int dtype, hipStream_t st);
PA_EXPORT int pa_rms_norm_bwd(const void* dy, const void* x, const void* w, const float* rstd, void* dx,
                              float* dw_part, int64_t rows, int64_t cols, int dtype_np, hipStream_t st);
PA_EXPORT int pa_rms_norm_bwd_res(const void* dy, const void* x, const void* w, const float* rstd, void* dx,
                                  float* dw_part, void* res, int64_t rows, int64_t cols, int dtype_np,
                                  hipStream_t st);
PA_EXPORT int pa_layer_norm_fwd(const void* x, const void* w, const void* b, void* y, float* mean, float* rstd,
                                int64_t rows, int64_t cols, float eps, int dtype, hipStream_t st);
PA_EXPORT int pa_layer_norm_bwd(const void* dy, const void* x, const void* w, const float* mean, const float* rstd,
                                void* dx, float* dw_part, float* db_part, void* res, int64_t rows, int64_t cols,
                                int dtype_np, hipStream_t st);
PA_EXPORT int pa_reduce_parts(const float* pa, const float* pb, void* oa, void* ob, int nparts, int64_t cols, int dta,
                              int dtb, hipStream_t st);
PA_EXPORT int pa_version();

PA_EXPORT int pa_maxpool_nhwc_fwd(const void* x, void* y, void* arg, int N, int H, int W, int C, int Ho, int Wo,
                                  int K, int s, int p, int dtype, hipStream_t st);
PA_EXPORT int pa_maxpool_nhwc_bwd(const void* dy, const void* arg, void* dx, int N, int H, int W, int C, int Ho,
                                  int Wo, int K, int s, int p, int dtype, hipStream_t st);

PA_EXPORT int64_t pa_fp8_nparts();
PA_EXPORT int pa_fp8_amax(const void* x, int64_t n, int dtype, float* parts, hipStream_t st);
PA_EXPORT int pa_fp8_scale_update(const float* parts, int n_parts, float* history, int hist_len, float* scale,
                                  float* scale_inv, float fmax, int margin, int mode, hipStream_t st);
PA_EXPORT int pa_fp8_quant(const void* x, int64_t R, int64_t C, int in_dtype, int fmt, const float* scale, void* q,
                           void* qT, float* parts, hipStream_t st);

PA_EXPORT int pa_softmax_fwd(const void* x, void* y, int64_t rows, int64_t cols, int dtype, hipStream_t st);
PA_EXPORT int pa_softmax_bwd(const void* y, const void* dy, void* dx, int64_t rows, int64_t cols, int dtype,
                             hipStream_t st);
PA_EXPORT int pa_softmax_ce_fwd(const void* logits, const int64_t* labels, float* loss, float* lse, int64_t rows,
                                int64_t cols, int64_t ignore_index, int dtype, hipStream_t st);
PA_EXPORT int pa_softmax_ce_bwd(const void* logits, const int64_t* labels, const float* lse, const float* dloss,
                                void* dlogits, int64_t rows, int64_t cols, int64_t ignore_index, int dtype,
                                hipStream_t st);
PA_EXPORT int pa_ce_slice_fwd(const void* logits, const int64_t* labels, float* lse, float* tgt, int64_t rows,
                              int64_t cols, int64_t v0, int dtype, hipStream_t st);
PA_EXPORT int pa_ce_slice_bwd(const void* logits, const int64_t* labels, const float* lse, const float* dloss,
                              void* dlogits, int64_t rows, int64_t cols, int64_t v0, int64_t ignore_index, int dtype,
                              hipStream_t st);

PA_EXPORT int pa_wo_gemm_splits(int64_t M, int64_t N, int64_t K, int llm);
PA_EXPORT int pa_wo_gemm(const void* x, const void* xo, const float* sx, const void* w, const float* scale,
                         const void* bias, void* y, float* ws, int M, int N, int K, int ldx, int ldy, int bits,
                         int group, int splits, hipStream_t st);
PA_EXPORT int pa_wo_dequant(const void* w, const float* scale, void* out, int N, int K, int bits, int group,
                            hipStream_t st);
```

### paddlepaddle_amd/autograd/engine.py

```python
from __future__ import annotations

import torch

from ..framework.flags import get_flags

_HOOKS: dict = {}
_FINAL: list = []
_ACTIVE = [0]


def queue_callback(fn):
    if _ACTIVE[0]:
        _FINAL.append(fn)
    else:
        torch.autograd.Variable._execution_engine.queue_callback(fn)


def _drain():
    while _FINAL:
        _FINAL.pop(0)()


def engine_name():
    try:
        return str(get_flags("FLAGS_eager_backward_engine")["FLAGS_eager_backward_engine"])
    except Exception:
        return "torch"


def use_native():
    if engine_name() != "native":
        return False
    from ..utils import native
    m = native.module()
    return m is not None and hasattr(m, "run_backward")


def _edge(t):
    e = torch.autograd.graph.get_gradient_edge(t)
    return e.node, e.output_nr


def add_hook(t, fn):
    key = _edge(t)
    lst = _HOOKS.setdefault(key, [])
    lst.append(fn)

    def remove():
        if fn in lst:
            lst.remove(fn)
        if not lst:
            _HOOKS.pop(key, None)
    return remove


def runs_tensor_hooks():
    return _executor() is not None


def register_grad_hook(t, fn):
    if use_native() and not runs_tensor_hooks():
        rm = add_hook(t, fn)
        h = t.register_hook(fn)

        def remove():
            rm()
            h.remove()
        return remove
    h = t.register_hook(fn)
    return h.remove


def retain(t):
    import warnings
    import weakref
    if t.is_leaf:
        return
    ref = weakref.ref(t)

    def h(g):
        x = ref()
        if x is not None:
            with warnings.catch_warnings():
                warnings.simplefilter("ignore")
                cur = x.grad
            x.grad = g.detach() if cur is None else cur + g.detach()
        return None
    if runs_tensor_hooks():
        t.register_hook(h)
        return
    t.retain_grad()
    key = _edge(t)
    _HOOKS.setdefault(key, []).insert(0, h)


def _zeros_for(node, slot):
    m = node._input_metadata[slot]
    return torch.zeros(tuple(m.shape), dtype=m.dtype, device=m.device)


def _fix(g, node, slot):
    try:
        m = node._input_metadata[slot]
    except (IndexError, AttributeError, RuntimeError):
        return g
    if g.dtype != m.dtype and (m.dtype.is_floating_point or m.dtype.is_complex):
        g = g.to(m.dtype)
    shp = tuple(m.shape)
    if tuple(g.shape) != shp and len(shp) <= g.dim():
        try:
            g = g.sum_to_size(shp)
        except RuntimeError:
            pass
    return g


def _is_py(node):
    return isinstance(node, torch.autograd.function.BackwardCFunction)


_HELPERS = (_zeros_for, _fix, _is_py)


_EXEC = []


def _executor():
    if not _EXEC:
        try:
            from .. import _C_autograd
            _EXEC.append(_C_autograd)
        except ImportError:
            _EXEC.append(None)
    return _EXEC[0]


def _run(outs, grads, ins, create_graph, retain_graph=None):
    from ..utils import native
    for t in outs:
        if not t.requires_grad:
            raise RuntimeError("backward: the output tensor has stop_gradient=True (no grad node to start from)")
    keep = create_graph if retain_graph is None else bool(retain_graph)
    ex = _executor()
    _ACTIVE[0] += 1
    ok = False
    try:
        if ex is not None:
            res = ex.run_backward(list(zip(outs, grads)), list(ins), _HOOKS, keep, create_graph)
        else:
            roots = [(*_edge(t), g) for t, g in zip(outs, grads)]
            with torch.set_grad_enabled(create_graph):
                res = native.module().run_backward(roots, [_edge(t) for t in ins], _HOOKS, _HELPERS)
        ok = True
    finally:
        _ACTIVE[0] -= 1
        if not _ACTIVE[0] and not ok:
            for fn in _FINAL:
                owner = getattr(fn, "__self__", None)
                if owner is not None and getattr(owner, "_queued", False):
                    owner._queued = False
            _FINAL.clear()
    if not _ACTIVE[0]:
        _drain()
    return res


def backward(outs, grads, retain_graph=False):
    _run(outs, grads, [], False, retain_graph)
    if not retain_graph:
        for k in [k for k in _HOOKS if not isinstance(k[0], _ACC)]:
            del _HOOKS[k]


_ACC = type(torch.autograd.graph.get_gradient_edge(torch.zeros(1, requires_grad=True)).node)


def grad(outs, ins, grads, create_graph=False, allow_unused=False, retain_graph=None):
    for t in ins:
        if not t.requires_grad:
            raise RuntimeError("paddle.grad: an input tensor has stop_gradient=True")
    res = _run(outs, grads, ins, create_graph, retain_graph)
    for r in res:
        if r is None and not allow_unused:
            raise RuntimeError("paddle.grad: one of the inputs is not reachable from the outputs; "
                               "set allow_unused=True to return None for it")
    if not create_graph:
        res = [None if r is None else r.detach() for r in res]
    return res
```

### paddlepaddle_amd/framework/flags.py

```python
from __future__ import annotations

import os

_FLAGS = {
    "FLAGS_check_nan_inf": False,
    "FLAGS_check_nan_inf_level": 0,
    "FLAGS_use_hip_kernels": True,
    "FLAGS_cudnn_deterministic": False,
    "FLAGS_embedding_deterministic": 0,
    "FLAGS_fraction_of_gpu_memory_to_use": 0.92,
    "FLAGS_allocator_strategy": "auto_growth",
    "FLAGS_eager_delete_tensor_gb": 0.0,
    "FLAGS_use_cuda_graph": False,
    "FLAGS_enable_pir_api": False,
    "FLAGS_print_ir": False,
    "FLAGS_call_stack_level": 1,
    "FLAGS_dp_bucket_mb": 128,
    "FLAGS_sharding_bucket_mb": 256,
    "FLAGS_pir_native_interpreter": True,
    "FLAGS_eager_backward_engine": "native",
    "FLAGS_weight_only_dequant_cache_mb": 4096,
    "FLAGS_fused_grad_accumulation": True,
    "FLAGS_static_native_executor": "auto",
    "FLAGS_gemm_backend": "auto",
    "FLAGS_sharding_stage3_keep_params": "auto",
    "FLAGS_conv_per_direction": True,
    "FLAGS_conv_bn_fusion": True,
    "FLAGS_use_autotune": True,
    "FLAGS_autotune_range_begin": 0,
    "FLAGS_autotune_range_end": 1 << 30,
    "FLAGS_layout_autotune": False,
    "FLAGS_dataloader_autotune": False,
    "FLAGS_dataloader_tuning_steps": 8,
    "FLAGS_static_engine_native": "auto",
    "FLAGS_linear_wt_cache_mb": 0,
}

for _k in list(_FLAGS):
    if _k in os.environ:
        _v = os.environ[_k]
        _d = _FLAGS[_k]
        if isinstance(_d, bool):
            _FLAGS[_k] = _v.lower() in ("1", "true", "yes")
        elif isinstance(_d, int):
            _FLAGS[_k] = int(_v)
        elif isinstance(_d, float):
            _FLAGS[_k] = float(_v)
        else:
            _FLAGS[_k] = _v


def _norm(k):
    return k if k.startswith("FLAGS_") else "FLAGS_" + k


def set_flags(flags: dict):
    for k, v in flags.items():
        _FLAGS[_norm(k)] = v


def get_flags(flags):
    if isinstance(flags, str):
        flags = [flags]
    out = {}
    for k in flags:
        k = _norm(k)
        if k not in _FLAGS:
            raise ValueError(f"flag {k} not found")
        out[k] = _FLAGS[k]
    return out


def flag(k, default=None):
    return _FLAGS.get(_norm(k), default)
```

### paddlepaddle_amd/models/gpt.py

```python
from __future__ import annotations

import dataclasses
import math

import torch

from .. import nn
from ..framework.tensor import Tensor, _wrap
from ..nn import functional as F
from ..nn import initializer as I
from .. import ops as _ops


@dataclasses.dataclass
class GPTConfig:
    vocab_size: int = 50304
    hidden_size: int = 5120
    num_hidden_layers: int = 40
    num_attention_heads: int = 40
    intermediate_size: int = 20480
    max_position_embeddings: int = 2048
    hidden_dropout_prob: float = 0.1
    attention_probs_dropout_prob: float = 0.0
    initializer_range: float = 0.02
    layer_norm_eps: float = 1e-5
    tie_word_embeddings: bool = True
    use_recompute: bool = False
    recompute_granularity: str = "full"
    no_recompute_layers: tuple = ()
    tensor_parallel_degree: int = 1
    sequence_parallel: bool = False
    fuse_attention_qkv: bool = True
    fused_head_ce: bool = False

    @staticmethod
    def gpt3_13b(**kw):
        return GPTConfig(**kw)

    @staticmethod
    def gpt3_6_7b(**kw):
        d = dict(hidden_size=4096, num_hidden_layers=32, num_attention_heads=32, intermediate_size=16384)
        d.update(kw)
        return GPTConfig(**d)

    @staticmethod
    def gpt3_1_3b(**kw):
        d = dict(hidden_size=2048, num_hidden_layers=24, num_attention_heads=16, intermediate_size=8192)
        d.update(kw)
        return GPTConfig(**d)

    @staticmethod
    def gpt3_175b(**kw):
        d = dict(hidden_size=12288, num_hidden_layers=96, num_attention_heads=96, intermediate_size=49152)
        d.update(kw)
        return GPTConfig(**d)

    @staticmethod
    def tiny(**kw):
        d = dict(vocab_size=512, hidden_size=128, num_hidden_layers=2, num_attention_heads=2, intermediate_size=512,
                 max_position_embeddings=128, hidden_dropout_prob=0.0)
        d.update(kw)
        return GPTConfig(**d)

    def num_params(self):
        h, L, f, V, P = (self.hidden_size, self.num_hidden_layers, self.intermediate_size, self.vocab_size,
                         self.max_position_embeddings)
        per_layer = 4 * h * h + 4 * h + 2 * h * f + f + h + 4 * h
        return L * per_layer + V * h + P * h + 2 * h

    def flops_per_token(self, seq_len, recompute=False):
        n = self.num_params() - self.max_position_embeddings * self.hidden_size
        attn = 6 * self.num_hidden_layers * self.hidden_size * seq_len
        f = 6 * n + attn
        if recompute:
            f += 2 * n + attn / 3
        return f


def _tp():
    from ..parallel import tensor_parallel as tp
    return tp


def _sp():
    from ..parallel import sequence_parallel as sp
    return sp


def _use_sp(cfg):
    return cfg.sequence_parallel and cfg.tensor_parallel_degree > 1


class GPTEmbeddings(nn.Layer):
    def __init__(self, cfg: GPTConfig):
        super().__init__()
        init = I.Normal(0.0, cfg.initializer_range)
        if cfg.tensor_parallel_degree > 1:
            self.word_embeddings = _tp().VocabParallelEmbedding(cfg.vocab_size, cfg.hidden_size,
                                                                weight_attr=nn.ParamAttr(initializer=init))
        else:
            self.word_embeddings = nn.Embedding(cfg.vocab_size, cfg.hidden_size,
                                                weight_attr=nn.ParamAttr(initializer=init))
        self.position_embeddings = nn.Embedding(cfg.max_position_embeddings, cfg.hidden_size,
                                                weight_attr=nn.ParamAttr(initializer=init))
        self.dropout = nn.Dropout(cfg.hidden_dropout_prob)

        self.sp = _use_sp(cfg)
        if self.sp:
            _sp().mark_sequence_parallel(self.position_embeddings.weight)

    def forward(self, input_ids, position_ids=None):
        if self.sp:
            return self._forward_sp(input_ids, position_ids)
        if position_ids is None:
            S = input_ids.shape[-1]
            position_ids = _wrap(torch.arange(S, device=input_ids._t.device).unsqueeze(0))
        x = self.word_embeddings(input_ids)._t
        pe = self.position_embeddings(position_ids)._t
        p = self.dropout.p if self.training else 0.0
        return _wrap(_ops.dropout_add(x + pe, None, p, self.training))

    def _forward_sp(self, input_ids, position_ids):
        sp = _sp()
        ids = input_ids._t
        B, S = ids.shape[0], ids.shape[-1]
        emb = self.word_embeddings.local_lookup(ids).reshape(B * S, -1)
        x = sp.reduce_scatter_tokens(emb)
        r0, r1 = sp.token_block_range(B * S)
        if position_ids is None:
            pos = torch.arange(r0, r1, device=ids.device) % S
        else:
            pos = position_ids._t.expand(B, S).reshape(-1)[r0:r1]
        pe = torch.nn.functional.embedding(pos, self.position_embeddings.weight._t)
        p = self.dropout.p if self.training else 0.0
        return _wrap(_ops.dropout_add(x + pe, None, p, self.training))


class GPTAttention(nn.Layer):
    def __init__(self, cfg: GPTConfig):
        super().__init__()
        h = cfg.hidden_size
        self.num_heads = cfg.num_attention_heads
        self.head_dim = h // self.num_heads
        self.tp = cfg.tensor_parallel_degree
        init = I.Normal(0.0, cfg.initializer_range)
        out_init = I.Normal(0.0, cfg.initializer_range / math.sqrt(2.0 * cfg.num_hidden_layers))
        if self.tp > 1:
            tp = _tp()
            self.qkv_proj = tp.ColumnParallelLinear(h, 3 * h, weight_attr=nn.ParamAttr(initializer=init),
                                                    has_bias=True, gather_output=False)
            self.out_proj = tp.RowParallelLinear(h, h, weight_attr=nn.ParamAttr(initializer=out_init),
                                                 has_bias=True, input_is_parallel=True)
            self.local_heads = self.num_heads // self.tp
        else:
            self.qkv_proj = nn.Linear(h, 3 * h, weight_attr=nn.ParamAttr(initializer=init))
            self.out_proj = nn.Linear(h, h, weight_attr=nn.ParamAttr(initializer=out_init))
            self.local_heads = self.num_heads
        self.attn_dropout = cfg.attention_probs_dropout_prob
        self.sp = _use_sp(cfg)
        self.bs = None
        if self.sp:
            _sp().mark_sequence_parallel(self.out_proj.bias)

    def forward(self, x):
        if self.sp:
            return self._forward_sp(x)
        qkv = self.qkv_proj(x)._t
        B, S = qkv.shape[0], qkv.shape[1]
        qkv = qkv.view(B, S, self.local_heads, 3, self.head_dim)
        o = self._core(qkv)
        o = o.reshape(B, S, self.local_heads * self.head_dim)
        return self.out_proj(_wrap(o))

    def _core(self, qkv):
        def fn(t):
            return _ops.flash_attention_qkvpacked(t, causal=True, dropout=self.attn_dropout, training=self.training)
        if getattr(self, "_rc_core", False):
            from ..distributed.fleet.recompute import recompute
            return recompute(lambda a: _wrap(fn(a._t)), _wrap(qkv))._t
        return fn(qkv)

    def _forward_sp(self, x):
        sp = _sp()
        B, S = self.bs
        w, b = self.qkv_proj.weight._t, self.qkv_proj.bias._t
        t = x._t if x._t.dtype == w.dtype else x._t.to(w.dtype)
        qkv = sp.column_sp_linear(t, w, b)
        qkv = qkv.view(B, S, self.local_heads, 3, self.head_dim)
        o = _ops.flash_attention_qkvpacked(qkv, causal=True, dropout=self.attn_dropout, training=self.training)
        o = o.reshape(B * S, self.local_heads * self.head_dim)
        y = sp.row_sp_linear(o, self.out_proj.weight._t)
        return _wrap(y + self.out_proj.bias._t)


def _tracing():
    from ..framework.trace_hook import _active_program
    return _active_program() is not None


class GPTMLP(nn.Layer):
    def __init__(self, cfg: GPTConfig):
        super().__init__()
        h, f = cfg.hidden_size, cfg.intermediate_size
        init = I.Normal(0.0, cfg.initializer_range)
        out_init = I.Normal(0.0, cfg.initializer_range / math.sqrt(2.0 * cfg.num_hidden_layers))
        self.tp = cfg.tensor_parallel_degree
        if self.tp > 1:
            tp = _tp()
            self.linear1 = tp.ColumnParallelLinear(h, f, weight_attr=nn.ParamAttr(initializer=init), has_bias=True,
                                                   gather_output=False, fuse_bias_act="gelu")
            self.linear2 = tp.RowParallelLinear(f, h, weight_attr=nn.ParamAttr(initializer=out_init), has_bias=True,
                                                input_is_parallel=True)
        else:
            self.linear1 = nn.Linear(h, f, weight_attr=nn.ParamAttr(initializer=init))
            self.linear2 = nn.Linear(f, h, weight_attr=nn.ParamAttr(initializer=out_init))
        self.sp = _use_sp(cfg)
        if self.sp:
            _sp().mark_sequence_parallel(self.linear2.bias)

    def forward(self, x):
        if self.sp:
            sp = _sp()
            w1 = self.linear1.weight._t
            t = x._t if x._t.dtype == w1.dtype else x._t.to(w1.dtype)
            h = sp.column_sp_linear(t, w1, self.linear1.bias._t, act="gelu")
            y = sp.row_sp_linear(h, self.linear2.weight._t)
            return _wrap(y + self.linear2.bias._t)
        if self.tp > 1:
            h = self.linear1(x)
        else:
            w, b = self.linear1.weight._t, self.linear1.bias._t
            xt = x._t
            if xt.dtype != w.dtype:
                xt = xt.to(w.dtype)
            l2 = self.linear2
            w2, b2 = l2.weight._t, l2.bias._t
            if (w.dtype in (torch.bfloat16, torch.float16) and w2.dtype == w.dtype and b2.dtype == w.dtype
                    and not (l2._forward_pre_hooks or l2._forward_post_hooks or _tracing())):
                return _wrap(_ops.ffn_gelu(xt, w, b, w2, b2))
            h = _wrap(_ops.fused_linear(xt, w, b, act="gelu"))
        return self.linear2(h)


class GPTDecoderLayer(nn.Layer):
    def __init__(self, cfg: GPTConfig):
        super().__init__()
        self.norm1 = nn.LayerNorm(cfg.hidden_size, epsilon=cfg.layer_norm_eps)
        self.self_attn = GPTAttention(cfg)
        self.norm2 = nn.LayerNorm(cfg.hidden_size, epsilon=cfg.layer_norm_eps)
        self.mlp = GPTMLP(cfg)
        self.dropout1 = nn.Dropout(cfg.hidden_dropout_prob)
        self.dropout2 = nn.Dropout(cfg.hidden_dropout_prob)
        if _use_sp(cfg):
            _sp().mark_sequence_parallel(self.norm1.weight, self.norm1.bias, self.norm2.weight, self.norm2.bias)

    def _ln(self, norm, x):
        r, h = _ops.layer_norm_residual(x._t, norm.weight._t, norm.bias._t, norm._epsilon)
        return r, _wrap(h)

    def _attn(self, h):
        return _gpt_attn(self, h)

    def forward(self, x):
        p = self.dropout1.p if self.training else 0.0
        r, h = self._ln(self.norm1, x)
        x = _wrap(_ops.dropout_add(self._attn(h)._t, r, p, self.training))
        r, h = self._ln(self.norm2, x)
        x = _wrap(_ops.dropout_add(self.mlp(h)._t, r, p, self.training))
        return x


def _gpt_attn(layer, h):
    g = getattr(layer, "_rc", None)
    if g == "full_attn":
        from ..distributed.fleet.recompute import recompute
        return recompute(layer.self_attn, h)
    layer.self_attn._rc_core = g == "core_attn"
    return layer.self_attn(h)


class GPTModel(nn.Layer):
    def __init__(self, cfg: GPTConfig):
        super().__init__()
        self.config = cfg
        self.embeddings = GPTEmbeddings(cfg)
        self.layers = nn.LayerList([GPTDecoderLayer(cfg) for _ in range(cfg.num_hidden_layers)])
        self.norm = nn.LayerNorm(cfg.hidden_size, epsilon=cfg.layer_norm_eps)
        if _use_sp(cfg):
            _sp().mark_sequence_parallel(self.norm.weight, self.norm.bias)

    def forward(self, input_ids, position_ids=None):
        if _use_sp(self.config):
            bs = (input_ids.shape[0], input_ids.shape[-1])
            for layer in self.layers:
                layer.self_attn.bs = bs
        x = self.embeddings(input_ids, position_ids)
        rc = self.config.use_recompute and self.training
        gran = self.config.recompute_granularity
        skip = set(self.config.no_recompute_layers or ())
        if rc:
            from ..distributed.fleet.recompute import recompute
        for i, layer in enumerate(self.layers):
            on = rc and i not in skip
            if on and gran == "full":
                x = recompute(layer, x)
            else:
                layer._rc = gran if on else None
                x = layer(x)
        return self.norm(x)


class GPTForPretraining(nn.Layer):
    def __init__(self, cfg: GPTConfig):
        super().__init__()
        self.config = cfg
        self.gpt = GPTModel(cfg)
        if not cfg.tie_word_embeddings:
            self.lm_head_weight = self.create_parameter([cfg.vocab_size // max(cfg.tensor_parallel_degree, 1),
                                                         cfg.hidden_size],
# ... 46 lines not shown
```

### paddlepaddle_amd/ops/__init__.py

```python
from __future__ import annotations

from .activation import gelu, silu, swiglu, softmax, bias_gelu
from .norm import rms_norm, rms_norm_residual, layer_norm, layer_norm_residual, add_rms_norm
from .loss import softmax_cross_entropy
from .attention import flash_attention, attention_bhsd, flash_attention_qkvpacked, qkv_rope_attention, attention_reference, paged_decode_attention, dense_decode_attention
from .rope import apply_rotary, decode_rope_cache
from .linear import fused_linear, colsum, linear_nt, ffn_gelu
from .lm_head import lm_head_cross_entropy
from .dropout import dropout_add
from . import optim
from ._loader import has as has_kernel, hip_enabled_for, LIB_PATH
from .bn import batch_norm_act_nhwc
from . import conv, gemm, dwconv, quant
```

### paddlepaddle_amd/ops/_sigs.py

```python
import ctypes

_vp = ctypes.c_void_p
_i64 = ctypes.c_int64
_i32 = ctypes.c_int
_f32 = ctypes.c_float
_u64 = ctypes.c_uint64

SIGS = {
    "pa_rms_norm_fwd": [_vp, _vp, _vp, _vp, _i64, _i64, _f32, _i32, _vp],
    "pa_rms_norm_bwd": [_vp, _vp, _vp, _vp, _vp, _vp, _i64, _i64, _i32, _vp],
    "pa_rms_norm_bwd_res": [_vp, _vp, _vp, _vp, _vp, _vp, _vp, _i64, _i64, _i32, _vp],
    "pa_layer_norm_fwd": [_vp, _vp, _vp, _vp, _vp, _vp, _i64, _i64, _f32, _i32, _vp],
    "pa_layer_norm_bwd": [_vp, _vp, _vp, _vp, _vp, _vp, _vp, _vp, _vp, _i64, _i64, _i32, _vp],
    "pa_reduce_parts": [_vp, _vp, _vp, _vp, _i32, _i64, _i32, _i32, _vp],
    "pa_softmax_fwd": [_vp, _vp, _i64, _i64, _i32, _vp],
    "pa_softmax_bwd": [_vp, _vp, _vp, _i64, _i64, _i32, _vp],
    "pa_softmax_ce_fwd": [_vp, _vp, _vp, _vp, _i64, _i64, _i64, _i32, _vp],
    "pa_softmax_ce_bwd": [_vp, _vp, _vp, _vp, _vp, _i64, _i64, _i64, _i32, _vp],
    "pa_ce_slice_fwd": [_vp, _vp, _vp, _vp, _i64, _i64, _i64, _i32, _vp],
    "pa_ce_slice_bwd": [_vp, _vp, _vp, _vp, _vp, _i64, _i64, _i64, _i64, _i32, _vp],
    "pa_gelu_fwd": [_vp, _vp, _i64, _i32, _i32, _vp],
    "pa_gelu_bwd": [_vp, _vp, _vp, _i64, _i32, _i32, _vp],
    "pa_swiglu_fwd": [_vp, _vp, _vp, _i64, _i64, _i64, _i32, _vp],
    "pa_swiglu_bwd": [_vp, _vp, _vp, _vp, _vp, _i64, _i64, _i64, _i32, _vp],
    "pa_bias_gelu_fwd": [_vp, _vp, _vp, _i64, _i64, _i32, _vp],
    "pa_rope_fwd": [_vp, _vp, _vp, _vp, _i64, _i64, _i64, _i64, _i32, _i32, _vp],
    "pa_rope_rows": [_vp, _i64, _vp, _vp, _vp, _i64, _i64, _i64, _i64, _i64, _i32, _i32, _vp],
    "pa_adamw_multi": [_vp, _vp, _i64, _vp, _f32, _f32, _f32, _f32, _f32, _f32, _f32, _vp, _vp],
    "pa_adam_hyper_step": [_vp, _f32, _f32, _vp],
    "pa_sq_norm_multi": [_vp, _vp, _i64, _vp, _vp],
    "pa_write_i64": [_vp, _vp, _i64, _vp],
    "pa_bn_set_target_wgs": [_i32],
    "pa_momentum_multi": [_vp, _vp, _i64, _vp, _f32, _f32, _f32, _i32, _vp],
    "pa_multi_tensor_chunk": [],
    "pa_lamb_multi": [_vp, _vp, _i64, _vp, _i64, _vp, _vp, _vp, _f32, _f32, _f32, _f32, _f32, _f32, _i32, _vp],
    "pa_amp_check_unscale_multi": [_vp, _vp, _i64, _vp, _vp, _vp],
    "pa_flash_attn_set_fwd_variant": [_i32],
    "pa_flash_attn_fwd": [_vp, _vp, _vp, _vp, _vp, _vp, _i32, _i32, _i32, _i32, _i32, _i32, _f32, _i32, _vp],
    "pa_flash_attn_bwd": [_vp, _vp, _vp, _vp, _vp, _vp, _vp, _vp, _vp, _vp, _vp, _vp,
                          _i32, _i32, _i32, _i32, _i32, _i32, _f32, _i32, _vp],
    "pa_flash_attn_fwd_ex": [_vp, _vp, _vp, _vp, _vp, _vp, _i32, _i32, _i32, _i32, _i32, _i32, _f32, _i32, _vp,
                             _vp],
    "pa_flash_attn_bwd_ex": [_vp, _vp, _vp, _vp, _vp, _vp, _vp, _vp, _vp, _vp, _vp, _vp,
                             _i32, _i32, _i32, _i32, _i32, _i32, _f32, _i32, _i64, _vp, _vp],
    "pa_flash_attn_bwd_ds": [_vp, _vp, _vp, _vp, _vp, _vp, _vp, _vp, _vp, _vp, _vp, _vp,
                             _i32, _i32, _i32, _i32, _i32, _i32, _f32, _i32, _vp, _vp],
    "pa_flash_attn_bwd_ds_ok": [_i32, _i32, _i32, _i32, _i32],
    "pa_flash_attn_bwd_ds_bytes": [_i32, _i32, _i32, _i32],
    "pa_fa_fm_stats": [_vp, _i32, _i32, _i32, _i32, _i32, _i64, _i64, _i32, _vp, _vp],
    "pa_paged_decode_attn": [_vp, _vp, _vp, _vp, _vp, _vp, _vp, _vp, _i32, _i32, _i32, _i32, _i32, _i32, _i32,
                             _i64, _i64, _f32, _vp],
    "pa_colsum": [_vp, _vp, _vp, _i64, _i64, _i32, _vp],
    "pa_dwconv_fwd": [_vp, _vp, _vp, _vp, _vp, _i32, _vp],
    "pa_dwconv_dgrad": [_vp, _vp, _vp, _vp, _vp, _i32, _vp],
    "pa_dwconv_wgrad_parts": [_vp, _vp],
    "pa_dwconv_wgrad": [_vp, _vp, _vp, _vp, _i32, _vp],
    "pa_gemm_bf16": [_vp, _vp, _vp, _vp, _vp, _i64, _i64, _i64, _i64, _i64, _i64, _i32, _i32, _i32, _f32,
                     _i32, _i32, _vp],
    "pa_gemm_bf16_pp": [_vp, _vp, _vp, _vp, _vp, _i64, _i64, _i64, _i64, _i64, _i64, _i32, _i32, _i32, _f32,
                        _vp, _vp],
    "pa_gemm_bf16_4w": [_vp, _vp, _vp, _vp, _vp, _i64, _i64, _i64, _i64, _i64, _i64, _i32, _i32, _i32, _f32,
                        _vp, _vp],
    "pa_gemm_bf16_res": [_vp, _vp, _vp, _vp, _vp, _i64, _i64, _i64, _i64, _i64, _i64, _i32, _i32, _vp, _vp],
    "pa_gemm_bf16_dgelu": [_vp, _vp, _vp, _vp, _vp, _i64, _i64, _i64, _i64, _i64, _i64, _i32, _i32, _i32, _vp],
    "pa_gemm_bf16_pp_segs": [_vp, _i32, _i32, _vp, _vp, _vp, _vp, _i64, _i64, _i64, _i64, _i64, _i64, _i32, _i32,
                             _i32, _f32, _vp, _vp],
    "pa_gemm_pp_ws_bytes": [_i64, _i64, _i64],
    "pa_gemm_pp_splitk_ws_bytes": [_i64, _i64, _i32],
    "pa_gemm_bf16_pp_splitk": [_vp, _vp, _vp, _i64, _i64, _i64, _i64, _i64, _i64, _i32, _i32, _i32, _f32, _i32, _vp,
                               _vp],
    "pa_gemm_fp8": [_vp, _vp, _vp, _vp, _i64, _i64, _i64, _i64, _i64, _i64, _i32, _i32, _f32, _i32, _i32, _vp],
    "pa_gemm_fp8_set_kernel": [_i32],
    "pa_gemm_fp8_ws": [_vp, _vp, _vp, _vp, _i64, _i64, _i64, _i64, _i64, _i64, _i32, _i32, _f32, _i32, _i32, _vp, _vp],
    "pa_gemm_fp8_ws_bytes": [_i64, _i64, _i64],
    "pa_gemm_fp8_dscale": [_vp, _vp, _vp, _vp, _i64, _i64, _i64, _i64, _i64, _i64, _i32, _i32, _f32, _i32, _i32, _vp,
                           _vp, _vp, _vp],
    "pa_fp8_nparts": [],
    "pa_fp8_amax": [_vp, _i64, _i32, _vp, _vp],
    "pa_fp8_scale_update": [_vp, _i32, _vp, _i32, _vp, _vp, _f32, _i32, _i32, _vp],
    "pa_fp8_quant": [_vp, _i64, _i64, _i32, _i32, _vp, _vp, _vp, _vp, _vp],
    "pa_gemm_bf16_4w_abl": [_vp, _vp, _vp, _i64, _i64, _i64, _i32, _vp],
    "pa_gemm_small_m": [_vp, _i64, _vp, _i64, _vp, _i64, _vp, _vp, _i32, _i32, _i32, _i32, _i32, _vp],
    "pa_gemm_skinny": [_vp, _vp, _vp, _vp, _i64, _i64, _i64, _i64, _i64, _i64, _i32, _i32, _vp],
    "pa_wo_gemm": [_vp, _vp, _vp, _vp, _vp, _vp, _vp, _vp, _i32, _i32, _i32, _i32, _i32, _i32, _i32, _i32, _vp],
    "pa_wo_gemm_splits": [_i64, _i64, _i64, _i32],
    "pa_wo_dequant": [_vp, _vp, _vp, _i32, _i32, _i32, _i32, _vp],
    "pa_gemm_skinny_ok": [_i64, _i64],
    "pa_gemm_skinny_stats_chunks": [_i64, _i64, _i64],
    "pa_gemm_skinny_stats": [_vp, _vp, _vp, _vp, _i64, _i64, _i64, _i64, _i64, _i64, _i32, _vp, _vp],
    "pa_conv_skinny_stats_chunks": [_i64, _i64, _i64],
    "pa_conv_skinny_stats": [_vp, _vp, _vp, _vp, _vp, _i64, _i64, _i64, _vp, _vp],
    "pa_conv_skinny": [_vp, _vp, _vp, _vp, _vp] + [_i64] * 11 + [_vp],
    "pa_conv_skinny_ok": [_i64, _i64, _i64, _i64],
    "pa_conv_skinny_wgrad": [_vp, _vp, _vp, _vp, _i64, _i64, _i64, _i64, _i64, _i64, _vp],
    "pa_conv2d_nhwc_fwd": [_vp, _vp, _vp, _vp, _vp] + [_i32] * 13 + [_vp],
    "pa_conv3d_ndhwc_fwd": [_vp, _vp, _vp, _vp, _vp] + [_i32] * 17 + [_vp],
    "pa_conv2d_nhwc_fwd_stats": [_vp, _vp, _vp, _vp, _vp] + [_i32] * 13 + [_vp, _vp],
    "pa_gemm_stats_chunks": [_i64, _i32],
    "pa_slab_reduce_bf16": [_vp, _vp, _i64, _i64, _i64, _i32, _vp],
    "pa_gemm_bf16_bnbwd": [_vp, _vp, _vp, _i64, _i64, _i64, _i64, _i64, _i64, _i32, _i32, _i32, _vp, _vp, _vp, _vp,
                           _vp],
    "pa_conv2d_nhwc_fwd_bnbwd": [_vp, _vp, _vp, _vp] + [_i32] * 13 + [_vp, _vp, _vp, _vp, _vp],
    "pa_gemm_bf16_stats": [_vp, _vp, _vp, _vp, _i64, _i64, _i64, _i64, _i64, _i64, _i32, _i32, _i32, _i32, _vp,
                           _vp],
    "pa_conv2d_nhwc_wgrad": [_vp, _vp, _vp, _vp] + [_i32] * 15 + [_vp],
    "pa_bias_gelu_bwd": [_vp, _vp, _vp, _vp, _vp, _vp, _i64, _i64, _i32, _vp],
    "pa_dropout_add_fwd": [_vp, _vp, _vp, _i64, _f32, _u64, _i32, _vp],
    "pa_dropout_bwd": [_vp, _vp, _i64, _f32, _u64, _i32, _vp],
    "pa_dropout_bwd_colsum": [_vp, _vp, _vp, _i64, _i64, _f32, _u64, _i32, _vp],
    "pa_colsum_nparts": [_i64],
    "pa_fold_partials": [_vp, _vp, _i64, _i64, _i32, _vp],
    "pa_bn_chunks": [_i64, _i32],
    "pa_bn_fwd_nhwc": [_vp] * 11 + [_i64, _i32, _f32, _f32, _i32, _i32, _vp],
    "pa_bn_bwd_nhwc": [_vp] * 12 + [_i64, _i32, _i32, _i32, _vp, _vp],
    "pa_bn_reduce_nhwc": [_i32] + [_vp] * 7 + [_i64, _i32, _i32, _vp],
    "pa_bn_fwd_nhwc_mask": [_vp] * 12 + [_i64, _i32, _f32, _f32, _i32, _vp],
    "pa_bn_bwd_nhwc_mask": [_vp] * 12 + [_i64, _i32, _i32, _vp],
    "pa_bn_bwd_apply_nhwc": [_vp] * 6 + [_i64, _i32, _i32, _vp, _vp],
    "pa_bn_pre_ws": [_i32, _i32],
    "pa_bn_bwd_nhwc_pre": [_vp] * 9 + [_i32, _vp, _vp, _i64, _i32, _i32, _vp, _vp],
    "pa_bn_fwd_nhwc_pre": [_vp] * 10 + [_i32, _vp, _vp, _vp, _i64, _i32, _f32, _f32, _i32, _vp],
    "pa_add_rms_norm_fwd": [_vp, _vp, _vp, _vp, _vp, _i64, _i64, _f32, _i32, _vp],
    "pa_decode_rope_cache": [_vp, _i64, _vp, _vp, _vp, _vp, _vp, _vp, _i32, _i32, _i32, _i32, _i64, _i32, _vp],
    "pa_maxpool_nhwc_fwd": [_vp, _vp, _vp] + [_i32] * 10 + [_vp],
    "pa_maxpool_nhwc_bwd": [_vp, _vp, _vp] + [_i32] * 10 + [_vp],
    "pa_grouped_gemm": [_i32, _vp, _vp, _vp, _vp, _vp, _vp, _i32, _i64, _i32, _i32, _i32, _i64, _i64, _i64, _i32,
                        _vp],
    "pa_moe_route": [_vp, _i32, _i32, _vp, _vp, _vp, _vp],
    "pa_version": [],
}

RET_I64 = {"pa_fp8_nparts", "pa_flash_attn_bwd_ds_bytes", "pa_gemm_pp_ws_bytes", "pa_gemm_fp8_ws_bytes", "pa_gemm_pp_splitk_ws_bytes", "pa_bn_pre_ws", "pa_gemm_skinny_stats_chunks", "pa_conv_skinny_stats_chunks",
           "pa_colsum_nparts", "pa_multi_tensor_chunk"}
```

### paddlepaddle_amd/ops/gemm.py

```python
from __future__ import annotations

import json
import os

import torch

from . import _loader as L

EPI_BIAS, EPI_GELU, EPI_AUX, EPI_ACCUM, EPI_OUT_F32 = 1, 2, 4, 8, 16


def _layout(t, outer_dim):
    s0, s1 = t.stride()
    kdim = 1 - outer_dim
    if t.stride(kdim) == 1 and t.shape[kdim] >= 1:
        ld = t.stride(outer_dim)
        return (ld if t.shape[outer_dim] > 1 else t.shape[kdim]), True
    if t.stride(outer_dim) == 1:
        ld = t.stride(kdim)
        return (ld if t.shape[kdim] > 1 else t.shape[outer_dim]), False
    return None


def _operands(a, b):
# ... 16 lines not shown
    M, K = a.shape
    N = b.shape[1]
    if K % 64 or N % 8 or K == 0:
        return False
    la, lb = _layout(a, 0), _layout(b, 1)
    if la is None or lb is None or la[0] % 8 or lb[0] % 8:
        return False
    if not la[1] and M % 8:
        return False
    if a.data_ptr() % 16 or b.data_ptr() % 16:
        return False
    return True


def gemm(a, b, bias=None, gelu=False, aux=None, out=None, accumulate=False, alpha=1.0, out_dtype=None, bn=None):
    M, N, K, lda, ak, ldb, bk = _operands(a, b)
    if out is None:
        out = torch.empty(M, N, dtype=out_dtype or torch.bfloat16, device=a.device)
    assert out.stride(1) == 1 and out.stride(0) % 4 == 0
    flags = 0
    if bias is not None:
        flags |= EPI_BIAS
    if gelu:
        flags |= EPI_GELU
    if aux is not None:
        flags |= EPI_AUX
        assert aux.stride(0) == out.stride(0) and aux.dtype == torch.bfloat16
    if accumulate:
        flags |= EPI_ACCUM
    if out.dtype == torch.float32:
        flags |= EPI_OUT_F32
    if bn is None:
        bn = _pick_bn(M, N, bk)
    if bn in (1, 2) and L.has("pa_gemm_bf16_pp"):
        ws = _pp_workspace(M, N, K, a.device)
        fn = {1: "pa_gemm_bf16_pp", 2: "pa_gemm_bf16_4w"}[bn]
        L.call(fn, L.ptr(a), L.ptr(b), L.ptr(out), L.ptr(bias),
               L.ptr(aux), M, N, K, lda, ldb, out.stride(0), int(ak), int(bk), flags, float(alpha), L.ptr(ws),
               L.stream_ptr())
        return out
    L.call("pa_gemm_bf16", L.ptr(a), L.ptr(b), L.ptr(out), L.ptr(bias), L.ptr(aux), M, N, K, lda, ldb, out.stride(0),
           int(ak), int(bk), flags, float(alpha), int(bn), 1, L.stream_ptr())
    return out


def res_supported(a, b, res):
    return (supported(a, b) and L.has("pa_gemm_bf16_res") and res.dtype == torch.bfloat16 and res.dim() == 2
            and tuple(res.shape) == (a.shape[0], b.shape[1]) and res.stride(1) == 1
            and res.stride(0) == b.shape[1] and res.data_ptr() % 16 == 0 and b.shape[1] % 8 == 0)


def gemm_res(a, b, res, bias=None):
    M, N, K, lda, ak, ldb, bk = _operands(a, b)
    out = torch.empty(M, N, dtype=torch.bfloat16, device=a.device)
    ws = _pp_workspace(M, N, K, a.device)
    L.call("pa_gemm_bf16_res", L.ptr(a), L.ptr(b), L.ptr(out), L.ptr(bias), L.ptr(res), M, N, K, lda, ldb, N,
           int(ak), int(bk), L.ptr(ws), L.stream_ptr())
    return out


def gemm_dgelu_supported(a, b, pre):
    return (supported(a, b) and L.has("pa_gemm_bf16_dgelu") and pre.dtype == torch.bfloat16 and pre.dim() == 2
            and tuple(pre.shape) == (a.shape[0], b.shape[1]) and pre.stride(1) == 1 and pre.stride(0) == b.shape[1]
            and pre.data_ptr() % 16 == 0 and b.shape[1] % 8 == 0)


def gemm_dgelu(a, b, pre, kern=1):
    M, N, K, lda, ak, ldb, bk = _operands(a, b)
    dh = torch.empty(M, N, dtype=torch.bfloat16, device=a.device)
    parts = torch.empty(-(-M // 256), N, dtype=torch.float32, device=a.device)
    L.call("pa_gemm_bf16_dgelu", L.ptr(a), L.ptr(b), L.ptr(dh), L.ptr(pre), L.ptr(parts), M, N, K, lda, ldb, N,
           int(ak), int(bk), int(kern), L.stream_ptr())
    return dh, parts


def _seg_table(rows):
    return torch.tensor(rows, dtype=torch.int64)


def gemm_kseg_supported(As, Bs):
    if not (L.has("pa_gemm_bf16_pp_segs") and 1 <= len(As) <= 4 and len(As) == len(Bs)):
        return False
    M, N = As[0].shape[0], Bs[0].shape[1]
    la, lb = None, None
    for a, b in zip(As, Bs):
        if a.shape[0] != M or b.shape[1] != N or a.shape[1] != b.shape[0] or a.shape[1] % 64 or not supported(a, b):
            return False
        ka, kb = _layout(a, 0)[1], _layout(b, 1)[1]
        if la is None:
            la, lb = ka, kb
        elif (ka, kb) != (la, lb):
            return False
    return True


def gemm_kseg(As, Bs, out=None, accumulate=False, alpha=1.0):
    M, N, _, lda, ak, ldb, bk = _operands(As[0], Bs[0])
    K = sum(a.shape[1] for a in As)
    if out is None:
        out = torch.empty(M, N, dtype=torch.bfloat16, device=As[0].device)
    assert out.stride(1) == 1 and out.stride(0) % 4 == 0
    rows, end = [], 0
    for a, b in zip(As, Bs):
        end += a.shape[1]
        rows.append([a.data_ptr(), b.data_ptr(), _layout(a, 0)[0], _layout(b, 1)[0], end])
    flags = (EPI_ACCUM if accumulate else 0) | (EPI_OUT_F32 if out.dtype == torch.float32 else 0)
    ws = _pp_workspace(M, N, K, out.device)
    tab = _seg_table(rows)
    L.call("pa_gemm_bf16_pp_segs", tab.data_ptr(), len(rows), 1, L.ptr(As[0]), L.ptr(Bs[0]), L.ptr(out), L.ptr(None),
           M, N, K, lda, ldb, out.stride(0), int(ak), int(bk), flags, float(alpha), L.ptr(ws), L.stream_ptr())
    return out


def gemm_nseg_supported(a, Bs):
    if not (L.has("pa_gemm_bf16_pp_segs") and 1 <= len(Bs) <= 4):
        return False
    K = a.shape[1]
    lay = None
    for i, b in enumerate(Bs):
        if b.shape[0] != K or not supported(a, b) or (i + 1 < len(Bs) and b.shape[1] % 128):
            return False
        kb = _layout(b, 1)[1]
        if lay is None:
            lay = kb
        elif kb != lay:
            return False
    return True


def gemm_nseg(a, Bs, out=None, alpha=1.0):
    M, _, K, lda, ak, ldb, bk = _operands(a, Bs[0])
    N = sum(b.shape[1] for b in Bs)
    if out is None:
        out = torch.empty(M, N, dtype=torch.bfloat16, device=a.device)
    assert out.stride(1) == 1 and out.stride(0) % 4 == 0
    rows, end = [], 0
    for b in Bs:
        end += b.shape[1]
        rows.append([a.data_ptr(), b.data_ptr(), _layout(a, 0)[0], _layout(b, 1)[0], end])
    flags = EPI_OUT_F32 if out.dtype == torch.float32 else 0
    ws = _pp_workspace(M, N, K, a.device)
    tab = _seg_table(rows)
    L.call("pa_gemm_bf16_pp_segs", tab.data_ptr(), len(rows), 0, L.ptr(a), L.ptr(Bs[0]), L.ptr(out), L.ptr(None),
           M, N, K, lda, ldb, out.stride(0), int(ak), int(bk), flags, float(alpha), L.ptr(ws), L.stream_ptr())
    return out


def gemm_seg_supported(a1, a2, b1, b2):
    return gemm_kseg_supported([a1, a2], [b1, b2])


def gemm_seg(a1, a2, b1, b2, out=None, accumulate=False, alpha=1.0):
    return gemm_kseg([a1, a2], [b1, b2], out=out, accumulate=accumulate, alpha=alpha)


def gemm_bn_stats(a, b, bias=None, bn=None):
    M, N, K, lda, ak, ldb, bk = _operands(a, b)
    if bn is None:
        bn = 160 if bk else (256 if _pick_bn(M, N, bk) == 256 else 128)
    chunks = int(L.lib().pa_gemm_stats_chunks(M, bn))
    out = torch.empty(M, N, dtype=torch.bfloat16, device=a.device)
    stats = torch.empty(2 * chunks * N, dtype=torch.float32, device=a.device)
    L.call("pa_gemm_bf16_stats", L.ptr(a), L.ptr(b), L.ptr(out), L.ptr(bias), M, N, K, lda, ldb, N, int(ak),
           int(bk), EPI_BIAS if bias is not None else 0, bn, L.ptr(stats), L.stream_ptr())
    return out, stats, chunks


def gemm_splitk(a, b, splits, out_dtype=torch.bfloat16, bn=None):
    M, N, K, lda, ak, ldb, bk = _operands(a, b)
    ws = torch.empty(splits, M, N, dtype=torch.float32, device=a.device)
    if bn is None:
        bn = _pick_bn(M, N, bk)
    L.call("pa_gemm_bf16", L.ptr(a), L.ptr(b), L.ptr(ws), L.ptr(None), L.ptr(None), M, N, K, lda, ldb, N,
           int(ak), int(bk), EPI_OUT_F32, 1.0, int(bn), int(splits), L.stream_ptr())
    return reduce_slabs(ws, out_dtype)


def pp_splits(M, N, K, cus=256, max_ws_bytes=256 << 20):
    T = -(-M // 256) * -(-N // 256)
    nk = K // 64
    s = 1
    while T * s * 2 <= 2 * cus and nk % (s * 2) == 0 and nk // (s * 2) >= 4 and T * s * 2 * 262144 <= max_ws_bytes:
        s *= 2
    return s if s > 1 else 0


def gemm_pp_splitk_ok(a, b, splits):
    if not (splits and L.has("pa_gemm_bf16_pp_splitk") and a.dtype == torch.bfloat16 and b.dtype == torch.bfloat16
            and a.is_cuda and L.hip_enabled_for(a)):
        return False
    M, K = a.shape
    N = b.shape[1]
    la, lb = _layout(a, 0), _layout(b, 1)
    return (la is not None and lb is not None and K % 64 == 0 and (K // 64) % splits == 0 and N % 8 == 0
            and la[0] % 8 == 0 and lb[0] % 8 == 0 and (la[1] or M % 8 == 0))


def gemm_pp_splitk(a, b, splits, out_dtype=torch.bfloat16, out=None, accumulate=False):
    M, N, K, lda, ak, ldb, bk = _operands(a, b)
    if out is None:
        out = torch.empty(M, N, dtype=out_dtype, device=a.device)
    elif out.shape != (M, N) or out.stride(1) != 1 or out.stride(0) % 4 or out.dtype not in (torch.bfloat16,
                                                                                           torch.float32):
        raise ValueError("gemm_pp_splitk: out must be a row-major [M, N] bf16 / fp32 tensor")
    ws = torch.empty(int(L.lib().pa_gemm_pp_splitk_ws_bytes(M, N, splits)) // 4, dtype=torch.float32,
                     device=a.device)
    flags = (EPI_OUT_F32 if out.dtype == torch.float32 else 0) | (EPI_ACCUM if accumulate else 0)
    L.call("pa_gemm_bf16_pp_splitk", L.ptr(a), L.ptr(b), L.ptr(out), M, N, K, lda, ldb, out.stride(0), int(ak),
           int(bk), flags, 1.0, int(splits), L.ptr(ws), L.stream_ptr())
    return out


def reduce_slabs(ws, out_dtype):
    splits, M, N = ws.shape
    if out_dtype == torch.bfloat16 and N % 4 == 0 and L.has("pa_slab_reduce_bf16"):
        out = torch.empty(M, N, dtype=torch.bfloat16, device=ws.device)
        L.call("pa_slab_reduce_bf16", L.ptr(ws), L.ptr(out), N, M, N, int(splits), L.stream_ptr())
        return out
    return ws.sum(0, dtype=torch.float32).to(out_dtype) if splits > 1 else ws[0].to(out_dtype)


def skinny_supported(a, b):
    if not (L.has("pa_gemm_skinny") and a.dtype == torch.bfloat16 and b.dtype == torch.bfloat16 and a.is_cuda):
        return False
    M, K = a.shape
    N = b.shape[1]
    if a.stride(1) != 1 or a.stride(0) % 8 or M < 1024 or not L.lib().pa_gemm_skinny_ok(N, K):
        return False
    return (b.stride(0) == 1 and b.stride(1) % 8 == 0) or (b.stride(1) == 1 and b.stride(0) % 8 == 0)


def gemm_skinny(a, b, bias=None, out=None, accumulate=False, relu=False):
    M, K = a.shape
    N = b.shape[1]
    if out is None:
        out = torch.empty(M, N, dtype=torch.bfloat16, device=a.device)
    assert out.stride(1) == 1 and out.stride(0) % 8 == 0 and out.dtype == torch.bfloat16
    bk = b.stride(0) == 1
    ldb = b.stride(1) if bk else b.stride(0)
    flags = (1 if bias is not None else 0) | (2 if accumulate else 0) | (4 if relu else 0)
    L.call("pa_gemm_skinny", L.ptr(a), L.ptr(b), L.ptr(out), L.ptr(bias), M, N, K, a.stride(0), ldb, out.stride(0),
           int(bk), flags, L.stream_ptr())
    return out


def gemm_skinny_bn_stats(a, b, bias=None):
    M, K = a.shape
    N = b.shape[1]
    chunks = int(L.lib().pa_gemm_skinny_stats_chunks(M, N, K))
    if chunks <= 0:
        return None
    out = torch.empty(M, N, dtype=torch.bfloat16, device=a.device)
    stats = torch.empty(2 * chunks * N, dtype=torch.float32, device=a.device)
    bk = b.stride(0) == 1
    ldb = b.stride(1) if bk else b.stride(0)
    L.call("pa_gemm_skinny_stats", L.ptr(a), L.ptr(b), L.ptr(out), L.ptr(bias), M, N, K, a.stride(0), ldb, N, int(bk),
           L.ptr(stats), L.stream_ptr())
    return out, stats, chunks


def pick_splits(M, N, K, bn=256, cus=256, max_ws_bytes=256 << 20):
    tiles = -(-M // 256) * -(-N // bn)
    s = 1
    while tiles * s * 2 <= 2 * cus and K % (s * 2 * 64) == 0 and (s * 2) * M * N * 4 <= max_ws_bytes:
        s *= 2
    return s


def _pick_bn(M, N, b_kmajor, cus=256):
    if M >= 1024 and N >= 1024 and -(-M // 256) * -(-N // 256) >= cus:
        return 1
    if b_kmajor:
        return 160

    def eff(bn):
        t = -(-M // 256) * -(-N // bn)
        waves = -(-t // cus)
        return t / (waves * cus) * (1.0 if bn == 256 else 0.9)
    return 256 if eff(256) >= eff(128) else 128


_CHOICE = {}
_TABLE_LOADED = False
_TUNING_DIR = os.path.join(os.path.dirname(os.path.abspath(__file__)), "tuning")


def _arch():
    try:
        return torch.cuda.get_device_properties(torch.cuda.current_device()).gcnArchName.split(":")[0]
    except Exception:
        return "unknown"


def _canon(key):
    def c(v):
        if isinstance(v, (bool, int, float, str)) or v is None:
            return v
        if isinstance(v, (tuple, list)):
            return tuple(c(x) for x in v)
        return str(v)
    return tuple(c(v) for v in key)


def _key_str(key):
    def j(v):
        return [j(x) for x in v] if isinstance(v, tuple) else v
# ... 172 lines not shown
```

### paddlepaddle_amd/ops/linear.py

```python
from __future__ import annotations

import torch
import torch.nn.functional as F

from . import _loader as L
from . import dropout as _dropout
from . import gemm as G
from .activation import bias_gelu, gelu
from ..framework.trace_hook import static_op


def colsum(x2d, acc=None):
    rows, cols = x2d.shape
    pre = _dropout.take_colsum(x2d) if x2d.is_cuda else None
    if pre is not None:
        out = acc if acc is not None else torch.empty(cols, dtype=x2d.dtype, device=x2d.device)
        L.call("pa_fold_partials", L.ptr(pre[0]), L.ptr(out), cols, pre[1], L.dcode(x2d) | ((acc is not None) << 8),
               L.stream_ptr())
        return out
    if L.hip_enabled_for(x2d) and x2d.dtype in L._DT and cols % 8 == 0 and x2d.is_contiguous():
        out = acc if acc is not None else torch.empty(cols, dtype=x2d.dtype, device=x2d.device)
        ws = torch.empty(256 * cols, dtype=torch.float32, device=x2d.device)
        L.call("pa_colsum", L.ptr(x2d), L.ptr(out), L.ptr(ws), rows, cols,
               L.dcode(x2d) | ((acc is not None) << 8), L.stream_ptr())
# ... 171 lines not shown

def _wgrad(x2, dy2, acc=None):
    xt = x2.t()
    if G.supported(xt, dy2):
        key = ("wgrad", xt.shape[0], dy2.shape[1], xt.shape[1], None if acc is None else acc.dtype)
        sk = G.pp_splits(*key[1:4]) if -(-key[1] // 256) * -(-key[2] // 256) < 256 else 0
        sk = sk if G.gemm_pp_splitk_ok(xt, dy2, sk) and (acc is None or acc.is_contiguous()) else 0
        if acc is None:
            cands = {"blas": lambda: torch.mm(xt, dy2), "hip": lambda: G.gemm(xt, dy2)}
            if sk:
                cands["hip_sk"] = lambda: G.gemm_pp_splitk(xt, dy2, sk, dy2.dtype)
        else:
            scratch = []

            def _s():
                if not scratch:
                    scratch.append(torch.zeros_like(acc))
                return scratch[0]
            cands = {"blas": lambda: _s().addmm_(xt, dy2),
                     "hip": lambda: G.gemm(xt, dy2, out=_s(), accumulate=True)}
            if sk:
                cands["hip_sk"] = lambda: G.gemm_pp_splitk(xt, dy2, sk, out=_s(), accumulate=True)
        ch = G.choose(key, cands)
        if ch == "hip":
            if acc is None:
                return G.gemm(xt, dy2)
            G.gemm(xt, dy2, out=acc, accumulate=True)
            return acc
        if ch == "hip_sk":
            if acc is None:
                return G.gemm_pp_splitk(xt, dy2, sk, dy2.dtype)
            G.gemm_pp_splitk(xt, dy2, sk, out=acc, accumulate=True)
            return acc
    if acc is None:
        return torch.mm(xt, dy2)
    return acc.addmm_(xt, dy2)


import contextlib
import types

_ZB = types.SimpleNamespace(queue=None, route=False)


@contextlib.contextmanager
def defer_weight_grads(queue):
    prev = getattr(_ZB, "queue", None)
    _ZB.queue = queue
    try:
        yield queue
    finally:
        _ZB.queue = prev


@contextlib.contextmanager
def zero_bubble_forward(enable=True):
    prev = getattr(_ZB, "route", False)
    _ZB.route = enable
    try:
        yield
    finally:
        _ZB.route = prev


def capture_forward_mode():
    return {"zb": getattr(_ZB, "route", False)}


class forward_mode:

    def __init__(self, mode):
        self.mode = mode
        self.prev = []

    def __enter__(self):
        self.prev.append(getattr(_ZB, "route", False))
        _ZB.route = self.mode["zb"]
        return self

    def __exit__(self, *exc):
        _ZB.route = self.prev.pop()
        return False


def apply_weight_grads(queue):
    for w, x2, dy2 in queue:
        ent = _main_grad_of(w)
        if ent is not None and ent[1].dtype == dy2.dtype:
            _wgrad(x2, dy2, acc=ent[1])
            ent[2](w)
            continue
        if w.grad_fn is not None:
            torch.autograd.backward(w, _wgrad(x2, dy2))
            continue
        if w.grad is None:
            w.grad = _wgrad(x2, dy2).to(w.dtype)
        elif w.grad.dtype == dy2.dtype and w.grad.is_contiguous():
            _wgrad(x2, dy2, acc=w.grad)
        else:
            w.grad.add_(_wgrad(x2, dy2))
        for h in (getattr(w, "_post_accumulate_grad_hooks", None) or {}).values():
            h(w)
    queue.clear()


_PAIR = types.SimpleNamespace(mode=None, jobs={})


@contextlib.contextmanager
def pair_weight_grads(mode):
    if mode not in ("defer", "merge", None):
        raise ValueError(f"pair_weight_grads: unknown mode {mode!r}")
    prev = _PAIR.mode
    _PAIR.mode = mode
    try:
        yield
    finally:
        _PAIR.mode = prev
        if mode == "merge":
            flush_paired_weight_grads()


def flush_paired_weight_grads():
    jobs = list(_PAIR.jobs.values())
    _PAIR.jobs.clear()
    for w, x2, dy2, buf, on_ready in jobs:
        _wgrad(x2, dy2, acc=buf)
        on_ready(w)


def pending_weight_grads():
    return len(_PAIR.jobs)


def _wgrad_pair(xa, dya, xb, dyb, acc):
    xta, xtb = xa.t(), xb.t()
    if G.gemm_seg_supported(xta, xtb, dya, dyb):
        key = ("wgrad2", xta.shape[0], dya.shape[1], xta.shape[1] + xtb.shape[1], acc.dtype)
        scratch = []

        def _s():
            if not scratch:
                scratch.append(torch.zeros_like(acc))
            return scratch[0]
        cands = {"hip": lambda: G.gemm_seg(xta, xtb, dya, dyb, out=_s(), accumulate=True),
                 "blas": lambda: (_s().addmm_(xta, dya), _s().addmm_(xtb, dyb))}
        if G.choose(key, cands) == "hip":
            G.gemm_seg(xta, xtb, dya, dyb, out=acc, accumulate=True)
            return
    _wgrad(xa, dya, acc=acc)
    _wgrad(xb, dyb, acc=acc)


def _main_grad_wgrad(w, x2, dy2, buf, on_ready):
    mode = _PAIR.mode
    if mode is not None:
        job = _PAIR.jobs.pop(id(w), None)
        if job is not None:
            _wgrad_pair(job[1], job[2], x2, dy2, buf)
            on_ready(w)
            return
        if mode == "defer":
            _PAIR.jobs[id(w)] = (w, x2, dy2, buf, on_ready)
            return
    _wgrad(x2, dy2, acc=buf)
    on_ready(w)


def _leaf_weights(*ws):
    return tuple(w if (isinstance(w, torch.Tensor) and w.requires_grad and w.is_leaf) else None for w in ws)


def _w_ident(w, leaf, needed):
    if not needed:
        return w
    if leaf is not None:
        return leaf
    return w if w.grad_fn is not None else None


def _mm_grads(x2, w, dy2, need_x, need_w, dx_hook=None, wid=_SAME):
    dx = _dgrad(dy2, w) if need_x else None
    fin = dx_hook(dx) if (dx_hook is not None and dx is not None) else None
    dw = None
    if wid is _SAME:
        wid = w
    q = getattr(_ZB, "queue", None)
    if need_w and q is not None and wid is not None:
        q.append((wid, x2, dy2))
        need_w = False
    if need_w and wid is None:
        dw = _wgrad(x2, dy2)
        need_w = False
    if need_w:
        w = wid
        ent = _main_grad_of(w)
        if ent is not None and ent[1].dtype == dy2.dtype:
            _, buf, on_ready = ent
            _main_grad_wgrad(w, x2, dy2, buf, on_ready)
        else:
            dw = _wgrad(x2, dy2)
    if fin is not None:
        fin()
    return dx, dw


class _GradHook(torch.autograd.Function):

    @staticmethod
    def forward(ctx, x, hook):
        ctx.hook = hook
        return x.view_as(x)

    @staticmethod
    def backward(ctx, g):
        g = g.contiguous()
        fin = ctx.hook(g)
        if fin is not None:
            fin()
        return g, None


class _LinearFn(torch.autograd.Function):

    @staticmethod
    def forward(ctx, x, w, b, dx_hook=None, residual=None):
        shape = x.shape
        x2 = x.reshape(-1, shape[-1])
        if residual is not None:
            y = _fwd_mm_res(x2, w, b, residual.reshape(-1, w.shape[1]).contiguous())
        else:
            y = _fwd_mm(x2, w, b)
        ctx.res_shape = None if residual is None else residual.shape
        ctx.save_for_backward(x2, w)
        ctx.w_leaf = _leaf_weights(w)[0]
        ctx.has_b = b is not None
        ctx.bias = b
        ctx.shape = shape
        ctx.dx_hook = dx_hook
        return y.view(*shape[:-1], w.shape[1])

    @staticmethod
    def backward(ctx, dy):
        x2, w = ctx.saved_tensors
        dy2 = dy.reshape(-1, dy.shape[-1])
        if dy2.dtype != x2.dtype:
            dy2 = dy2.to(x2.dtype)
        if not dy2.is_contiguous():
            dy2 = dy2.contiguous()
        dx, dw = _mm_grads(x2, w, dy2, ctx.needs_input_grad[0], ctx.needs_input_grad[1], ctx.dx_hook,
                           wid=_w_ident(w, ctx.w_leaf, ctx.needs_input_grad[1]))
        db = None
        if ctx.has_b and ctx.needs_input_grad[2]:
            mg = _vector_main_grad(ctx.bias, dy2.dtype)
            if mg is not None:
                colsum(dy2, acc=mg[0])
                mg[1](ctx.bias)
            else:
                db = colsum(dy2)
        if dx is not None:
            dx = dx.view(ctx.shape)
        dres = dy.reshape(ctx.res_shape) if (ctx.res_shape is not None and ctx.needs_input_grad[4]) else None
        return dx, dw, db, None, dres


class _LinearBiasGeluFn(torch.autograd.Function):
    @staticmethod
    def forward(ctx, x, w, b, dx_hook=None):
        shape = x.shape
        x2 = x.reshape(-1, shape[-1])
        y, h, bb = _fwd_bias_gelu(x2, w, b)
        ctx.save_for_backward(x2, w, bb, h)
        ctx.w_leaf = _leaf_weights(w)[0]
        ctx.bias = b
        ctx.shape = shape
        ctx.dx_hook = dx_hook
        return y.view(*shape[:-1], w.shape[1])

    @staticmethod
    def backward(ctx, dy):
        x2, w, b, h = ctx.saved_tensors
        dy2 = dy.reshape(-1, dy.shape[-1]).to(h.dtype).contiguous()
        rows, cols = h.shape
        dh = torch.empty_like(h)
        mg = _vector_main_grad(ctx.bias, b.dtype) if ctx.needs_input_grad[2] else None
        db = mg[0] if mg is not None else torch.empty(cols, dtype=b.dtype, device=b.device)
        ws = torch.empty(256 * cols, dtype=torch.float32, device=h.device)
        L.call("pa_bias_gelu_bwd", L.ptr(h), L.ptr(b), L.ptr(dy2), L.ptr(dh), L.ptr(db), L.ptr(ws), rows, cols,
               L.dcode(h) | ((mg is not None) << 8), L.stream_ptr())
        if mg is not None:
            mg[1](ctx.bias)
            db = None
        dx, dw = _mm_grads(x2, w, dh, ctx.needs_input_grad[0], ctx.needs_input_grad[1], ctx.dx_hook,
                           wid=_w_ident(w, ctx.w_leaf, ctx.needs_input_grad[1]))
        if dx is not None:
            dx = dx.view(ctx.shape)
        return dx, dw, db, None


def _bias_gelu_bwd(h, b, dg, db_acc=None):
    rows, cols = h.shape
    dh = torch.empty_like(h)
    db = db_acc if db_acc is not None else torch.empty(cols, dtype=b.dtype, device=b.device)
    ws = torch.empty(256 * cols, dtype=torch.float32, device=h.device)
    L.call("pa_bias_gelu_bwd", L.ptr(h), L.ptr(b), L.ptr(dg), L.ptr(dh), L.ptr(db), L.ptr(ws), rows, cols,
           L.dcode(h) | ((db_acc is not None) << 8), L.stream_ptr())
    return dh, db


def _dgrad_gelu(dy2, w2, h, b1, pre_biased, db_acc=None):
    w2t = w2.t()
    rows, cols = h.shape

    def split(acc=None):
        return _bias_gelu_bwd(h, b1, _dgrad(dy2, w2), acc)

# ... 236 lines not shown
```

### paddlepaddle_amd/parallel/data_parallel.py

```python
from __future__ import annotations

import contextlib

import torch
import torch.distributed as dist

from ..autograd.engine import queue_callback as _queue_callback
from ..distributed import collective as C
from ..framework.flags import flag
from ..framework.tensor import Tensor, _wrap
from ..nn.layer.layers import Layer
from ..utils import native


class _Bucket:
    __slots__ = ("params", "flat", "offsets", "pending", "work", "ready", "id")

    def __init__(self, params, dtype, device):
        self.params = params
        n = sum(p._t.numel() for p in params)
        self.flat = torch.zeros(n, dtype=dtype, device=device)
        self.offsets = []
        off = 0
        for p in params:
            self.offsets.append(off)
            off += p._t.numel()
        self.pending = len(params)
        self.work = None
        self.ready = set()

    def view(self, i):
        p = self.params[i]
        o = self.offsets[i]
        return self.flat[o:o + p._t.numel()].view_as(p._t)


class DataParallel(Layer):
    def __init__(self, layers, strategy=None, comm_buffer_size=None, last_comm_buffer_size=8,
                 find_unused_parameters=False, group=None):
        super().__init__()
        self._layers = layers
        self.find_unused_parameters = find_unused_parameters
        self.group = group
        self._sync_enabled = True
        self._world = C.get_world_size(group)
        self._buckets = []
        self._param_loc = {}
        self._queued = False
        self._next_launch = 0
        self._order = []
        if self._world > 1:
            self._broadcast_params()
            self._build_buckets(comm_buffer_size, last_comm_buffer_size)

    def _broadcast_params(self):
        src = self.group.ranks[0] if self.group is not None else 0
        with torch.no_grad():
            for p in self._layers.parameters():
                dist.broadcast(p._t.data, src=src, group=C._pg(self.group))
            for b in self._layers.buffers():
                dist.broadcast(b._t.data, src=src, group=C._pg(self.group))

    def _build_buckets(self, comm_mb, last_mb):
        params = [p for p in self._layers.parameters() if not p.stop_gradient]
        by_key = {}
        for p in params:
            by_key.setdefault((p._t.dtype, p._t.device), []).append(p)
        mb = comm_mb if comm_mb is not None else flag("FLAGS_dp_bucket_mb", 128)
        for (dt, dev), ps in by_key.items():
            sizes = [p._t.numel() * p._t.element_size() for p in ps]
            first = native.plan_buckets(sizes, int(last_mb * 2 ** 20))
            first_idx = first[0] if first else []
            rest = [i for i in range(len(ps)) if i not in set(first_idx)]
            plan = [first_idx]
            if rest:
                sub = native.plan_buckets([sizes[i] for i in rest], int(mb * 2 ** 20))
                plan += [[rest[j] for j in b] for b in sub]
            for idxs in plan:
                if not idxs:
                    continue
                b = _Bucket([ps[i] for i in idxs], dt, dev)
                bi = len(self._buckets)
                b.id = bi
                self._buckets.append(b)
                for j, p in enumerate(b.params):
                    self._param_loc[id(p)] = (bi, j)
                    p._t.grad = b.view(j)
                    p._dp_bucket = (b, j)
                    p._t.register_post_accumulate_grad_hook(self._make_hook(p))
        reg = {id(p): i for i, p in enumerate(params)}
        self._order = sorted(range(len(self._buckets)),
                             key=lambda bi: -min(reg[id(p)] for p in self._buckets[bi].params))

    def _make_hook(self, p):
        def hook(t):
            self._on_grad_ready(p)
        return hook

    def _on_grad_ready(self, p):
        if not self._sync_enabled or self._world == 1:
            return
        bi, j = self._param_loc[id(p)]
        b = self._buckets[bi]
        v = b.view(j)
        g = p._t.grad
        if g is None or g.data_ptr() != v.data_ptr():
            if g is not None:
                v.copy_(g)
            p._t.grad = v
        if not self._queued:
            self._queued = True
            _queue_callback(self._finalize)
        if j in b.ready:
            return
        b.ready.add(j)
        if len(b.ready) == len(b.params):
            self._launch_ready()

    def _launch_ready(self):
        while self._next_launch < len(self._buckets):
            b = self._buckets[self._order[self._next_launch]]
            if b.work is not None or len(b.ready) < len(b.params):
                break
            self._launch(b)
            self._next_launch += 1

    def _launch(self, b):
        from ..distributed import collective_check as _cc
        pg = C._pg(self.group)
        with _cc.label(f"dp bucket {b.id}") if _cc.enabled() else contextlib.nullcontext():
            if dist.get_backend(pg) == "nccl":
                b.work = dist.all_reduce(b.flat, op=dist.ReduceOp.AVG, group=pg, async_op=True)
            else:
                b.flat.mul_(1.0 / self._world)
                b.work = dist.all_reduce(b.flat, op=dist.ReduceOp.SUM, group=pg, async_op=True)

    def _finalize(self):
        while self._next_launch < len(self._buckets):
            self._launch(self._buckets[self._order[self._next_launch]])
            self._next_launch += 1
        for b in self._buckets:
            b.work.wait()
            b.work = None
            b.ready = set()
        self._next_launch = 0
        self._queued = False
        from ..distributed import collective_check as _cc
        if _cc.enabled():
            _cc.check_collectives("DataParallel backward")

    def forward(self, *inputs, **kwargs):
        return self._layers(*inputs, **kwargs)

    @contextlib.contextmanager
    def no_sync(self):
        prev = self._sync_enabled
        self._sync_enabled = False
        try:
            yield
        finally:
            self._sync_enabled = prev

    def state_dict(self, *args, **kwargs):
        return self._layers.state_dict(*args, **kwargs)

    def set_state_dict(self, state_dict, use_structured_name=True):
        return self._layers.set_state_dict(state_dict, use_structured_name)

    set_dict = set_state_dict
    load_dict = set_state_dict

    def scale_loss(self, loss):
        return loss

    def apply_collective_grads(self):
        pass

    def parameters(self, include_sublayers=True):
        return self._layers.parameters(include_sublayers)

    def named_parameters(self, prefix="", include_sublayers=True, remove_duplicate=True):
        return self._layers.named_parameters(prefix, include_sublayers, remove_duplicate)
```

### paddlepaddle_amd/parallel/sharding.py

```python
from __future__ import annotations

import contextlib

import os

import torch
import torch.distributed as dist

from ..autograd.engine import queue_callback as _queue_callback, register_grad_hook as _register_grad_hook
from ..distributed import collective as C
from ..framework.tensor import Parameter, Tensor, _wrap
from ..nn.layer.common import LayerList
from ..nn.layer.layers import Layer


def _is_nccl(pg):
    return dist.get_backend(pg) == "nccl"


_VECTOR_MAIN_GRAD = os.environ.get("PADDLE_AMD_VECTOR_MAIN_GRAD", "1") != "0"


class _Flat:

# ... 209 lines not shown
        if hasattr(opt, "_apply_decay_param_fun"):
            opt._apply_decay_param_fun = (lambda n, _d=decay_ids: n in _d)
        clip = getattr(opt, "_grad_clip", None)
        if clip is not None and hasattr(clip, "_extra_sq_norm_fn") and (
                self.world > 1 or self.mp_group is not None or self.pp_group is not None):
            pg, shard_sum = self.pg, self.world > 1
            mp_pg = self.mp_group.process_group if self.mp_group is not None else None
            pp_pg = self.pp_group.process_group if self.pp_group is not None else None

            def _param_sq(params):
                from ..ops.optim import global_sq_norm
                dev = params[0]._t.device
                dg = [p._t.grad for p in params if getattr(p, "is_distributed", False)]
                rg = [p._t.grad for p in params if not getattr(p, "is_distributed", False)]
                sq_d = (global_sq_norm(dg) if dg else torch.zeros((), device=dev)).float().reshape(1).clone()
                sq_r = (global_sq_norm(rg) if rg else torch.zeros((), device=dev)).float().reshape(1)
                if mp_pg is not None:
                    dist.all_reduce(sq_d, group=mp_pg)
                sq = sq_d + sq_r
                if shard_sum:
                    dist.all_reduce(sq, group=pg)
                if pp_pg is not None:
                    dist.all_reduce(sq, group=pp_pg)
                return sq[0]
            clip._param_sq_fn = _param_sq
            if mp_pg is None and pp_pg is None and shard_sum:
                def _allreduce_sq(sq):
                    dist.all_reduce(sq, group=pg)
                    return sq
                clip._extra_sq_norm_fn = _allreduce_sq

    def _install_hooks(self):
        for ui, u in enumerate(self.units):
            hook = self._make_grad_hook(u)
            for f in u.flats:
                f.ready_fn = hook
                for p in f.params:
                    p._t.register_post_accumulate_grad_hook(hook)
            if ui == 0:
                continue
            u.layer.register_forward_pre_hook(self._make_fwd_pre(ui))
            u.layer.register_forward_post_hook(self._make_fwd_post(ui))

    def _make_fwd_pre(self, ui):
        def hook(layer, inputs):
            u = self.units[ui]
            self._gather(u)
            self._wait_gather(u)
            if self.stage == 3 and torch.is_grad_enabled() and ui + 1 < len(self.units):
                self._gather(self.units[ui + 1])
            return None
        return hook

    def _make_fwd_post(self, ui):
        def hook(layer, inputs, out):
            u = self.units[ui]
            if torch.is_grad_enabled():
                t = out._t if isinstance(out, Tensor) else None
                if t is not None and t.requires_grad:
                    _register_grad_hook(t, self._make_pre_backward(ui))
            if self.stage == 3 and not self._in_backward and not self.keep_params:
                self._release(u)
            return None
        return hook

    def _make_pre_backward(self, ui):
        def hook(g):
            self._in_backward = True
            self._queue_finalize()
            u = self.units[ui]
            self._gather(u)
            self._wait_gather(u)
            for f in u.flats:
                f.alloc_full_grad()
            if self.stage == 3 and ui - 1 >= 1:
                self._gather(self.units[ui - 1])
            return None
        return hook

    def _make_grad_hook(self, u):
        def hook(t):
            self._queue_finalize()
            u.ready.add(id(t))
            if not self._sync:
                return
            if u is not self.units[0] and len(u.ready) == u.n_params:
                self._reduce_scatter(u)
                if self.stage == 3 and not self.keep_params:
                    self._release(u)
        return hook

    def _queue_finalize(self):
        if not self._queued:
            self._queued = True
            _queue_callback(self._finalize_backward)

    def _gather(self, u):
        from ..distributed import collective_check as _cc
        if _cc.enabled() and not (u.gathered or self.world == 1):
            with _cc.label(f"ag unit {self.units.index(u)}"):
                return self._gather_impl(u)
        return self._gather_impl(u)

    def _gather_impl(self, u):
        if u.gathered or self.world == 1:
            u.gathered = True
            return
        for f in u.flats:
            f.alloc_full()
            out = f.gbuf
            inp = f.shard._t.detach()
            if inp.dtype != out.dtype:
                inp = inp.to(out.dtype)
            u.gather_work.append(dist.all_gather_into_tensor(out, inp, group=self.pg, async_op=True))
        u.gathered = True

    def _wait_gather(self, u):
        for w in u.gather_work:
            w.wait()
        u.gather_work = []

    def _release(self, u):
        if self.stage != 3 or self.world == 1:
            return
        self._wait_gather(u)
        for f in u.flats:
            f.free_full()
        u.gathered = False

    def _reduce_scatter(self, u):
        from ..distributed import collective_check as _cc
        if _cc.enabled():
            with _cc.label(f"rs unit {self.units.index(u)}"):
                return self._reduce_scatter_impl(u)
        return self._reduce_scatter_impl(u)

    def _reduce_scatter_impl(self, u):
        for f in u.flats:
            f.fold_param_grads()
            fg = f.full_grad
            if self.world == 1:
                continue
            tmp = torch.empty(f.shard_size, dtype=fg.dtype, device=fg.device)
            if _is_nccl(self.pg):
                w = dist.reduce_scatter_tensor(tmp, fg, op=dist.ReduceOp.AVG, group=self.pg, async_op=True)
            else:
                fg.mul_(1.0 / self.world)
                w = dist.reduce_scatter_tensor(tmp, fg, op=dist.ReduceOp.SUM, group=self.pg, async_op=True)
            u.rs_work.append(w)
            u.rs_tmp.append((f, tmp))
        u.ready = set()

    def _finalize_backward(self):
        if not self._sync:
            for u in self.units:
                u.ready = set()
                if self.stage == 3 and u is not self.units[0] and not self.keep_params:
                    self._release(u)
            self._queued = False
            self._in_backward = False
            return
        for u in self.units:
            if u.ready or (not u.rs_tmp and any(f.full_grad is not None for f in u.flats)):
                self._reduce_scatter(u)
        for u in self.units:
            for w in u.rs_work:
                w.wait()
            for f, tmp in u.rs_tmp:
                f.shard_grad.add_(tmp.float())
                f.drop_full_grad()
            u.rs_work, u.rs_tmp = [], []
            if self.world == 1:
                continue
            if self.stage == 3 and u is not self.units[0]:
                if not self.keep_params:
                    self._release(u)
            else:
                for f in u.flats:
                    if f.full_grad is not None:
                        f.drop_full_grad()
        self._queued = False
        self._in_backward = False

    def shard_grads(self):
        if self.world == 1:
            return [f.alloc_full_grad() for u in self.units for f in u.flats]
        return [f.shard_grad for u in self.units for f in u.flats]

    def comm_groups(self):
        out = [self.group] if self.world > 1 else []
        return out + [g for g in (self.dp_group, self.mp_group, self.pp_group, self.sep_group) if g is not None]

    @torch.no_grad()
    def step(self):
        from ..distributed import collective_check as _cc
        if _cc.enabled():
            _cc.check_collectives("sharding step")
        dp_work = []
        sp_mp = self.mp_group is not None
        sp = []
        for u in self.units:
            for f in u.flats:
                if self.world == 1:
                    f.shard._t.grad = f.alloc_full_grad()
                else:
                    f.shard._t.grad = f.shard_grad
                if sp_mp and getattr(f, "sequence_parallel", False):
                    sp.append(f.shard._t.grad)
                    continue
                if self.sep_group is not None:
                    dist.all_reduce(f.shard._t.grad, group=self.sep_group.process_group)
                if self.dp_group is not None:
                    g = f.shard._t.grad
                    g.mul_(1.0 / self.dp_group.nranks)
                    dp_work.append(dist.all_reduce(g, group=self.dp_group.process_group, async_op=True))
        if sp:
            flat = torch.cat([g.reshape(-1).float() for g in sp])
            dist.all_reduce(flat, group=self.mp_group.process_group)
            if self.sep_group is not None:
                dist.all_reduce(flat, group=self.sep_group.process_group)
            if self.dp_group is not None:
                flat.mul_(1.0 / self.dp_group.nranks)
                dp_work.append(dist.all_reduce(flat, group=self.dp_group.process_group, async_op=True))
        for w in dp_work:
            w.wait()
        if sp:
            off = 0
            for g in sp:
                g.copy_(flat[off:off + g.numel()].view_as(g))
                off += g.numel()
        if self.offload:
            self._offload_step()
        else:
            self.inner_opt.step()
        if self.world == 1:
            return
        for u in self.units:
            if self.stage == 3 and u is not self.units[0]:
                if self.keep_params:
                    u.gathered = False
                continue
            for f in u.flats:
                dist.all_gather_into_tensor(f.gbuf, f.shard._t.detach().to(f.full.dtype), group=self.pg)

    def _state_slots(self, p):
        opt = self.inner_opt
        out = [(d, id(p)) for d in opt._accumulators.values() if id(p) in d]
        if id(p) in opt._master_weights:
            out.append((opt._master_weights, id(p)))
        return out

    @staticmethod
    def _host_copy(t):
        return torch.empty(t.shape, dtype=t.dtype, pin_memory=True)

    def _swap_in(self, shards, dev):
        if dev.type != "cuda":
            return None
        cs = self._copy_stream
        cs.wait_stream(torch.cuda.current_stream(dev))
        with torch.cuda.stream(cs):
            for p in shards:
                for d, k in self._state_slots(p):
                    h = d[k]
                    if h.device.type == "cpu":
                        g = torch.empty(h.shape, dtype=h.dtype, device=dev)
                        g.copy_(h, non_blocking=True)
                        g._pa_host = h
                        d[k] = g
        ev = torch.cuda.Event()
        ev.record(cs)
        return ev

    def _swap_out(self, shards, dev):
        if dev.type != "cuda":
            return
        cs = self._copy_stream
        cs.wait_stream(torch.cuda.current_stream(dev))
        bufs = []
        with torch.cuda.stream(cs):
            for p in shards:
                for d, k in self._state_slots(p):
                    g = d[k]
                    if g.device.type == "cpu":
                        continue
                    h = getattr(g, "_pa_host", None)
                    if h is None:
                        h = self._host_copy(g)
                    h.copy_(g, non_blocking=True)
                    g.record_stream(cs)
                    bufs.append(g)
                    d[k] = h
        ev = torch.cuda.Event()
        ev.record(cs)
        if self._inflight:
            pev, _ = self._inflight.pop(0)
            torch.cuda.current_stream(dev).wait_event(pev)
        self._inflight.append((ev, bufs))

    @torch.no_grad()
    def _offload_step(self):
        from ..ops.linear import bump_weight_epoch
        opt = self.inner_opt
        bump_weight_epoch()
        opt._step_count += 1
        opt._apply_clip()
# ... 167 lines not shown
```

Measured before the change: 13570 tokens/s.

## Group attention out_proj and qkv_proj weight-grad GEMMs into one paired launch

Adds a paired GEMM kernel entry that runs two problems sharing K in a single launch. Tile scheduling and the split-K tail plan cover the combined tile count. In the GPT attention block, the out_proj weight-grad is deferred and executed together with the qkv_proj weight-grad, aiming to cut tail-wave underutilization and launch overhead. An autotuner chooses between the paired and separate paths. Flush hooks in the autograd engine, data-parallel and sharding paths ensure deferred jobs still run, at the cost of extra bookkeeping and possible ordering or memory-lifetime changes.

```diff
diff --git a/csrc/dispatch/dispatch_gen.inc b/csrc/dispatch/dispatch_gen.inc
--- a/csrc/dispatch/dispatch_gen.inc
+++ b/csrc/dispatch/dispatch_gen.inc
@@ -48,6 +48,8 @@
 PA_ENTRY(pa_gemm_bf16_dgelu, "ippppplllllliiip")
 PA_ENTRY(pa_gemm_bf16_pp_segs, "ipiipppplllllliiifpp")
 PA_ENTRY(pa_gemm_pp_ws_bytes, "llll")
+PA_ENTRY(pa_gemm_pp_pair_ws_bytes, "llllll")
+PA_ENTRY(pa_gemm_bf16_pp_pair, "ipiiffpp")
 PA_ENTRY(pa_gemm_pp_splitk_ws_bytes, "llli")
 PA_ENTRY(pa_gemm_bf16_pp_splitk, "ippplllllliiifipp")
 PA_ENTRY(pa_gemm_fp8, "ipppplllllliifiip")
diff --git a/csrc/kernels/gemm.hip b/csrc/kernels/gemm.hip
--- a/csrc/kernels/gemm.hip
+++ b/csrc/kernels/gemm.hip
@@ -422,8 +422,33 @@
   }
 }
 
-template <bool AK, bool BKM, int SEG = 0>
-__global__ __launch_bounds__(kThreads, 1) void gemm256_kernel(GemmArgs p0) {
+__device__ __forceinline__ GemmArgs pair_select(const GemmArgs& p1, const GemmArgs& p2, bool second) {
+  GemmArgs p = p1;
+  p.a = second ? p2.a : p1.a;
+  p.b = second ? p2.b : p1.b;
+  p.c = second ? p2.c : p1.c;
+  p.lda = second ? p2.lda : p1.lda;
+  p.ldb = second ? p2.ldb : p1.ldb;
+  p.ldc = second ? p2.ldc : p1.ldc;
+  p.M = second ? p2.M : p1.M;
+  p.N = second ? p2.N : p1.N;
+  p.tiles_m = second ? p2.tiles_m : p1.tiles_m;
+  p.tiles_n = second ? p2.tiles_n : p1.tiles_n;
+  p.flags = second ? p2.flags : p1.flags;
+  p.alpha = second ? p2.alpha : p1.alpha;
+  return p;
+}
+
+struct PairTail {
+  GemmArgs p2;
+  int t1, tiles;
+};
+__device__ __forceinline__ const PairTail& pair_tail(const PairTail& q) { return q; }
+
+template <bool AK, bool BKM, int SEG = 0, class... Pair>
+__global__ __launch_bounds__(kThreads, 1) void gemm256_kernel(GemmArgs p0, Pair... pair) {
+  constexpr bool PAIR = sizeof...(Pair) != 0;
+  static_assert(!PAIR || (sizeof...(Pair) == 1 && SEG == 0), "the pair entry: one PairTail, plain operands");
   GemmArgs p = split_view<AK, BKM>(p0);
   constexpr int HALF = 128 * kBK * 2;
   constexpr int STAGE = 4 * HALF;
@@ -436,7 +461,28 @@
   int pid;
   float* tail_out = nullptr;
   int kt0 = 0;
-  if (p.tail_split > 0 && bid >= p.full_tiles) {
+  if constexpr (PAIR) {
+    const PairTail& q = pair_tail(pair...);
+    const GemmArgs& p2 = q.p2;
+    const int t1 = q.t1, tiles = q.tiles;
+    const int full = p0.full_tiles, split = p0.tail_split;
+    int tile, ks = 0;
+    if (split > 0 && bid >= full) {
+      const int u = bid - full;
+      ks = u % split;
+      tile = full + u / split;
+      tail_out = p0.tail_ws + (int64_t)u * 65536;
+    } else {
+      const int whole = split > 0 ? full : tiles, w1 = min(t1, whole);
+      tile = bid < w1 ? xcd_remap(bid, w1) : w1 + xcd_remap(bid - w1, whole - w1);
+    }
+    p = pair_select(p0, p2, pair_problem(tile, t1, &pid) != 0);
+    if (tail_out) {
+      p.K /= split;
+      p.a += (int64_t)ks * p.K * (AK ? 1 : p.lda);
+      p.b += (int64_t)ks * p.K * (BKM ? 1 : p.ldb);
+    }
+  } else if (p.tail_split > 0 && bid >= p.full_tiles) {
     const int u = bid - p.full_tiles;
     const int ks = u % p.tail_split;
     pid = p.full_tiles + u / p.tail_split;
@@ -1152,6 +1198,12 @@
   return launch_lds<gemm3s_kernel<AK, BKM, CONV>>(dim3(a.tiles_m * a.tiles_n, splits), dim3(kThreads), smem, st, a);
 }
 
+constexpr int smem256() {
+  constexpr int kLoop = 2 * 4 * 128 * kBK * 2, kEpi0 = 128 * kEpiRowStride * 4, kEpi1 = 256 * kEpiRowStrideBf16 * 2;
+  constexpr int kEpi = kEpi0 > kEpi1 ? kEpi0 : kEpi1;
+  return kLoop > kEpi ? kLoop : kEpi;
+}
+
 template <bool AK, bool BKM, int SEG>
 int launch256_seg(GemmArgs a, int splits, hipStream_t st, int grid) {
   a.tiles_m = (a.M + 255) / 256;
@@ -1160,10 +1212,7 @@
     grid = a.tiles_m * a.tiles_n;
     a.tail_split = 0;
   }
-  constexpr int kLoop = 2 * 4 * 128 * kBK * 2, kEpi0 = 128 * kEpiRowStride * 4, kEpi1 = 256 * kEpiRowStrideBf16 * 2;
-  constexpr int kEpi = kEpi0 > kEpi1 ? kEpi0 : kEpi1;
-  constexpr int smem = kLoop > kEpi ? kLoop : kEpi;
-  return launch_lds<gemm256_kernel<AK, BKM, SEG>>(dim3(grid, splits), dim3(kThreads), smem, st, a);
+  return launch_lds<gemm256_kernel<AK, BKM, SEG>>(dim3(grid, splits), dim3(kThreads), smem256(), st, a);
 }
 
 template <bool AK, bool BKM>
@@ -1314,10 +1363,9 @@
   *reinterpret_cast<uint2*>(c + (int64_t)m * ldc + n) = make_uint2(pack_bf16(acc.x, acc.y), pack_bf16(acc.z, acc.w));
 }
 
-__global__ __launch_bounds__(256) void gemm_tail_reduce_k(GemmArgs p) {
-  const int b = blockIdx.x;
+__device__ __forceinline__ void tail_reduce_tile(const GemmArgs& p, int pid, int b) {
   int tm, tn;
-  tile_coords(p.full_tiles + b, p.tiles_m, p.tiles_n, &tm, &tn);
+  tile_coords(pid, p.tiles_m, p.tiles_n, &tm, &tn);
   const int e = (blockIdx.y * 256 + threadIdx.x) * 4;
   const int r = e >> 8, c = e & 255;
   const int m = tm * 256 + r, n = tn * 256 + c;
@@ -1361,6 +1409,16 @@
     }
     *cp = make_uint2(pack_bf16(v[0], v[1]), pack_bf16(v[2], v[3]));
   }
+}
+
+__global__ __launch_bounds__(256) void gemm_tail_reduce_k(GemmArgs p) {
+  tail_reduce_tile(p, p.full_tiles + (int)blockIdx.x, (int)blockIdx.x);
+}
+
+__global__ __launch_bounds__(256) void gemm_tail_reduce_pair_k(GemmArgs p1, GemmArgs p2, int t1) {
+  int pid = 0;
+  const bool second = pair_problem(p1.full_tiles + (int)blockIdx.x, t1, &pid) != 0;
+  tail_reduce_tile(pair_select(p1, p2, second), pid, (int)blockIdx.x);
 }
 
 bool gemm_args(GemmArgs& g, const void* a, const void* b, void* c, const void* bias, void* aux, int64_t M, int64_t N,
@@ -1403,6 +1461,25 @@
   return (int)hipGetLastError();
 }
 
+int run_pair256(GemmArgs g1, GemmArgs g2, void* ws, hipStream_t st) {
+  PairPlan pp = pair_plan(g1.M, g1.N, g2.M, g2.N, g1.K, kBK, device_cus());
+  if (!ws) pp.plan = without_tail(pp.plan);
+  const TailPlan& pl = pp.plan;
+  for (GemmArgs* g : {&g1, &g2}) {
+    g->tiles_m = (g->M + 255) / 256;
+    g->tiles_n = (g->N + 255) / 256;
+    g->full_tiles = pl.full_tiles;
+    g->tail_split = pl.split;
+    g->tail_ws = (float*)ws;
+  }
+  const PairTail tail{g2, pp.t1, pl.tiles};
+  const int rc =
+      launch_lds<gemm256_kernel<false, false, 0, PairTail>>(dim3(pl.grid), dim3(kThreads), smem256(), st, g1, tail);
+  if (rc || !pl.split) return rc;
+  hipLaunchKernelGGL(gemm_tail_reduce_pair_k, dim3(pl.tiles - pl.full_tiles, 64), dim3(256), 0, st, g1, g2, pp.t1);
+  return (int)hipGetLastError();
+}
+
 bool conv_fwd_args(GemmArgs& g, const void* x, const void* w, const void* bias, void* out, const void* zero, int N,
                    int D, int H, int W, int C, int Cout, int KD, int KH, int KW, int stride, int pad_d, int pad_h,
                    int pad_w, int dil, int Do, int Ho, int Wo, int flags) {
@@ -1427,6 +1504,24 @@
   GemmArgs g;
   if (!gemm_args(g, a, b, c, bias, aux, M, N, K, lda, ldb, ldc, a_kmajor, flags, alpha)) return 1;
   return run_tile256(1, g, a_kmajor, b_kmajor, ws, st);
+}
+
+PA_EXPORT int64_t pa_gemm_pp_pair_ws_bytes(int64_t M1, int64_t N1, int64_t M2, int64_t N2, int64_t K) {
+  return pair_plan(M1, N1, M2, N2, K, kBK, device_cus()).plan.ws_bytes;
+}
+
+PA_EXPORT int pa_gemm_bf16_pp_pair(const int64_t* prob, int a_kmajor, int b_kmajor, float alpha1, float alpha2,
+                                   void* ws, hipStream_t st) {
+  if (!prob || a_kmajor || b_kmajor || prob[5] != prob[10 + 5]) return 1;
+  GemmArgs g[2];
+  for (int i = 0; i < 2; ++i) {
+    const int64_t* e = prob + 10 * i;
+    if (e[3] <= 0 || e[4] <= 0 || e[5] <= 0 || (e[9] & ~(int64_t)(kEpiAccum | kEpiOutF32))) return 1;
+    if (!gemm_args(g[i], (const void*)e[0], (const void*)e[1], (void*)e[2], nullptr, nullptr, e[3], e[4], e[5], e[6],
+                   e[7], e[8], 0, (int)e[9], i ? alpha2 : alpha1))
+      return 1;
+  }
+  return run_pair256(g[0], g[1], ws, st);
 }
 
 PA_EXPORT int64_t pa_gemm_pp_splitk_ws_bytes(int64_t M, int64_t N, int splits) {
diff --git a/csrc/kernels/gemm_plan.h b/csrc/kernels/gemm_plan.h
--- a/csrc/kernels/gemm_plan.h
+++ b/csrc/kernels/gemm_plan.h
@@ -16,14 +16,42 @@
 
 inline int64_t tiles256(int64_t M, int64_t N) { return ((M + 255) / 256) * ((N + 255) / 256); }
 
-inline TailPlan tail_plan(int64_t M, int64_t N, int64_t K, int k_tile, int cus) {
-  const int64_t T = tiles256(M, N);
+inline TailPlan tail_plan_tiles(int64_t T, int64_t K, int k_tile, int cus) {
   const int64_t nk = K / k_tile;
   const int64_t r = T > cus ? T % cus : 0;
   if (r == 0 || 2 * r > cus) return make_tail_plan(T, T, 0);
   int sp = 1;
   while (r * sp * 2 <= cus && nk % (sp * 2) == 0 && nk / (sp * 2) >= 4) sp *= 2;
   return sp == 1 ? make_tail_plan(T, T, 0) : make_tail_plan(T, T - r, sp);
+}
+
+inline TailPlan tail_plan(int64_t M, int64_t N, int64_t K, int k_tile, int cus) {
+  return tail_plan_tiles(tiles256(M, N), K, k_tile, cus);
+}
+
+struct PairPlan {
+  TailPlan plan;
+  int t1;
+};
+
+inline PairPlan pair_plan(int64_t M1, int64_t N1, int64_t M2, int64_t N2, int64_t K, int k_tile, int cus) {
+  const int64_t t1 = tiles256(M1, N1);
+  return {tail_plan_tiles(t1 + tiles256(M2, N2), K, k_tile, cus), (int)t1};
+}
+
+constexpr int pair_problem(int tile, int t1, int* local) {
+  const int second = tile >= t1;
+  *local = second ? tile - t1 : tile;
+  return second;
+}
+
+constexpr void tile_coords(int pid, int tiles_m, int tiles_n, int* tm, int* tn) {
+  constexpr int GM = 8;
+  const int per_group = GM * tiles_n;
+  const int first_m = (pid / per_group) * GM;
+  const int gsz = tiles_m - first_m < GM ? tiles_m - first_m : GM;
+  *tm = first_m + (pid % per_group) % gsz;
+  *tn = (pid % per_group) / gsz;
 }
 
 inline TailPlan split_all_plan(int64_t M, int64_t N, int splits) { return make_tail_plan(tiles256(M, N), 0, splits); }
diff --git a/csrc/kernels/mfma_tile.h b/csrc/kernels/mfma_tile.h
--- a/csrc/kernels/mfma_tile.h
+++ b/csrc/kernels/mfma_tile.h
@@ -1,5 +1,6 @@
 #pragma once
 #include "common.h"
+#include "gemm_plan.h"
 
 namespace pa {
 
@@ -117,14 +118,6 @@
   return (xcd < r ? xcd * (q + 1) : r * (q + 1) + (xcd - r) * q) + (bid >> 3);
 }
 
-__device__ __forceinline__ void tile_coords(int pid, int tiles_m, int tiles_n, int* tm, int* tn) {
-  constexpr int GM = 8;
-  const int per_group = GM * tiles_n;
-  const int first_m = (pid / per_group) * GM;
-  const int gsz = min(tiles_m - first_m, GM);
-  *tm = first_m + (pid % per_group) % gsz;
-  *tn = (pid % per_group) / gsz;
-}
 
 template <int V>
 struct IntC {
diff --git a/csrc/kernels/pa_api.h b/csrc/kernels/pa_api.h
--- a/csrc/kernels/pa_api.h
+++ b/csrc/kernels/pa_api.h
@@ -118,6 +118,9 @@
 PA_EXPORT int pa_gemm_bf16_pp(const void* a, const void* b, void* c, const void* bias, void* aux, int64_t M,
                               int64_t N, int64_t K, int64_t lda, int64_t ldb, int64_t ldc, int a_kmajor, int b_kmajor,
                               int flags, float alpha, void* ws, hipStream_t st);
+PA_EXPORT int64_t pa_gemm_pp_pair_ws_bytes(int64_t M1, int64_t N1, int64_t M2, int64_t N2, int64_t K);
+PA_EXPORT int pa_gemm_bf16_pp_pair(const int64_t* prob, int a_kmajor, int b_kmajor, float alpha1, float alpha2,
+                                   void* ws, hipStream_t st);
 PA_EXPORT int64_t pa_gemm_pp_splitk_ws_bytes(int64_t M, int64_t N, int splits);
 PA_EXPORT int pa_gemm_bf16_pp_splitk(const void* a, const void* b, void* c, int64_t M, int64_t N, int64_t K,
                                      int64_t lda, int64_t ldb, int64_t ldc, int a_kmajor, int b_kmajor, int flags,
diff --git a/paddlepaddle_amd/autograd/engine.py b/paddlepaddle_amd/autograd/engine.py
--- a/paddlepaddle_amd/autograd/engine.py
+++ b/paddlepaddle_amd/autograd/engine.py
@@ -155,11 +155,17 @@
     finally:
         _ACTIVE[0] -= 1
         if not _ACTIVE[0] and not ok:
-            for fn in _FINAL:
+            pending = list(_FINAL)
+            _FINAL.clear()
+            for fn in pending:
                 owner = getattr(fn, "__self__", None)
                 if owner is not None and getattr(owner, "_queued", False):
                     owner._queued = False
-            _FINAL.clear()
+                if getattr(fn, "run_on_failure", False):
+                    try:
+                        fn()
+                    except Exception:
+                        pass
     if not _ACTIVE[0]:
         _drain()
     return res
diff --git a/paddlepaddle_amd/framework/flags.py b/paddlepaddle_amd/framework/flags.py
--- a/paddlepaddle_amd/framework/flags.py
+++ b/paddlepaddle_amd/framework/flags.py
@@ -34,6 +34,7 @@
     "FLAGS_dataloader_tuning_steps": 8,
     "FLAGS_static_engine_native": "auto",
     "FLAGS_linear_wt_cache_mb": 0,
+    "FLAGS_group_wgrad": True,
 }
 
 for _k in list(_FLAGS):
diff --git a/paddlepaddle_amd/models/gpt.py b/paddlepaddle_amd/models/gpt.py
--- a/paddlepaddle_amd/models/gpt.py
+++ b/paddlepaddle_amd/models/gpt.py
@@ -6,6 +6,7 @@
 import torch
 
 from .. import nn
+from ..framework.flags import flag as _flag
 from ..framework.tensor import Tensor, _wrap
 from ..nn import functional as F
 from ..nn import initializer as I
@@ -165,6 +166,11 @@
     def forward(self, x):
         if self.sp:
             return self._forward_sp(x)
+        if self.training:
+            if _flag("FLAGS_group_wgrad", True):
+                _ops.group_weight_grads(self.out_proj.weight._t, self.qkv_proj.weight._t)
+            else:
+                _ops.ungroup_weight_grads(self.out_proj.weight._t)
         qkv = self.qkv_proj(x)._t
         B, S = qkv.shape[0], qkv.shape[1]
         qkv = qkv.view(B, S, self.local_heads, 3, self.head_dim)
diff --git a/paddlepaddle_amd/ops/__init__.py b/paddlepaddle_amd/ops/__init__.py
--- a/paddlepaddle_amd/ops/__init__.py
+++ b/paddlepaddle_amd/ops/__init__.py
@@ -5,7 +5,7 @@
 from .loss import softmax_cross_entropy
 from .attention import flash_attention, attention_bhsd, flash_attention_qkvpacked, qkv_rope_attention, attention_reference, paged_decode_attention, dense_decode_attention
 from .rope import apply_rotary, decode_rope_cache
-from .linear import fused_linear, colsum, linear_nt, ffn_gelu
+from .linear import fused_linear, colsum, linear_nt, ffn_gelu, group_weight_grads, ungroup_weight_grads
 from .lm_head import lm_head_cross_entropy
 from .dropout import dropout_add
 from . import optim
diff --git a/paddlepaddle_amd/ops/_sigs.py b/paddlepaddle_amd/ops/_sigs.py
--- a/paddlepaddle_amd/ops/_sigs.py
+++ b/paddlepaddle_amd/ops/_sigs.py
@@ -66,6 +66,8 @@
     "pa_gemm_bf16_pp_segs": [_vp, _i32, _i32, _vp, _vp, _vp, _vp, _i64, _i64, _i64, _i64, _i64, _i64, _i32, _i32,
                              _i32, _f32, _vp, _vp],
     "pa_gemm_pp_ws_bytes": [_i64, _i64, _i64],
+    "pa_gemm_pp_pair_ws_bytes": [_i64, _i64, _i64, _i64, _i64],
+    "pa_gemm_bf16_pp_pair": [_vp, _i32, _i32, _f32, _f32, _vp, _vp],
     "pa_gemm_pp_splitk_ws_bytes": [_i64, _i64, _i32],
     "pa_gemm_bf16_pp_splitk": [_vp, _vp, _vp, _i64, _i64, _i64, _i64, _i64, _i64, _i32, _i32, _i32, _f32, _i32, _vp,
                                _vp],
@@ -131,4 +133,4 @@
 }
 
 RET_I64 = {"pa_fp8_nparts", "pa_flash_attn_bwd_ds_bytes", "pa_gemm_pp_ws_bytes", "pa_gemm_fp8_ws_bytes", "pa_gemm_pp_splitk_ws_bytes", "pa_bn_pre_ws", "pa_gemm_skinny_stats_chunks", "pa_conv_skinny_stats_chunks",
-           "pa_colsum_nparts", "pa_multi_tensor_chunk"}
+           "pa_colsum_nparts", "pa_multi_tensor_chunk", "pa_gemm_pp_pair_ws_bytes"}
diff --git a/paddlepaddle_amd/ops/gemm.py b/paddlepaddle_amd/ops/gemm.py
--- a/paddlepaddle_amd/ops/gemm.py
+++ b/paddlepaddle_amd/ops/gemm.py
@@ -192,6 +192,37 @@
 
 def gemm_seg(a1, a2, b1, b2, out=None, accumulate=False, alpha=1.0):
     return gemm_kseg([a1, a2], [b1, b2], out=out, accumulate=accumulate, alpha=alpha)
+
+
+def _pair_out_ok(out, M, N):
+    return (out.dim() == 2 and tuple(out.shape) == (M, N) and out.stride(1) == 1 and out.stride(0) % 4 == 0
+            and out.dtype in (torch.bfloat16, torch.float32) and out.data_ptr() % 16 == 0)
+
+
+def gemm_pair_supported(a1, b1, out1, a2, b2, out2):
+    if not (L.has("pa_gemm_bf16_pp_pair") and supported(a1, b1) and supported(a2, b2)):
+        return False
+    if a1.shape[1] != a2.shape[1] or not a1.shape[0] or not a2.shape[0]:
+        return False
+    for a, b in ((a1, b1), (a2, b2)):
+        if _layout(a, 0)[1] or _layout(b, 1)[1]:
+            return False
+    return _pair_out_ok(out1, a1.shape[0], b1.shape[1]) and _pair_out_ok(out2, a2.shape[0], b2.shape[1])
+
+
+def gemm_pair(a1, b1, out1, a2, b2, out2, accumulate=(False, False), alpha=(1.0, 1.0), tail=True):
+    rows = []
+    for a, b, out, acc in ((a1, b1, out1, accumulate[0]), (a2, b2, out2, accumulate[1])):
+        M, N, K, lda, _, ldb, _ = _operands(a, b)
+        flags = (EPI_ACCUM if acc else 0) | (EPI_OUT_F32 if out.dtype == torch.float32 else 0)
+        rows.append([a.data_ptr(), b.data_ptr(), out.data_ptr(), M, N, K, lda, ldb, out.stride(0), flags])
+    ws = None
+    if tail:
+        nb = int(L.lib().pa_gemm_pp_pair_ws_bytes(rows[0][3], rows[0][4], rows[1][3], rows[1][4], rows[0][5]))
+        ws = torch.empty(nb // 4, dtype=torch.float32, device=out1.device) if nb else None
+    tab = torch.tensor(rows, dtype=torch.int64)
+    L.call("pa_gemm_bf16_pp_pair", tab.data_ptr(), 0, 0, float(alpha[0]), float(alpha[1]), L.ptr(ws), L.stream_ptr())
+    return out1, out2
 
 
 def gemm_bn_stats(a, b, bias=None, bn=None):
diff --git a/paddlepaddle_amd/ops/linear.py b/paddlepaddle_amd/ops/linear.py
--- a/paddlepaddle_amd/ops/linear.py
+++ b/paddlepaddle_amd/ops/linear.py
@@ -347,6 +347,91 @@
     _wgrad(xb, dyb, acc=acc)
 
 
+_GROUP = types.SimpleNamespace(partner={}, jobs={})
+
+
+def group_weight_grads(first, second):
+    ent = _GROUP.partner.get(id(first))
+    if ent is not None and ent[0]() is first and ent[1]() is second:
+        return
+    key = id(first)
+
+    def _drop(ref):
+        e = _GROUP.partner.get(key)
+        if e is not None and (e[0] is ref or e[1] is ref):
+            del _GROUP.partner[key]
+    _GROUP.partner[key] = (weakref.ref(first, _drop), weakref.ref(second, _drop))
+
+
+def ungroup_weight_grads(first):
+    _GROUP.partner.pop(id(first), None)
+
+
+def pending_grouped_weight_grads():
+    return len(_GROUP.jobs)
+
+
+def _run_group_job_alone(job):
+    w, x2, dy2, buf, on_ready, _ = job
+    _wgrad(x2, dy2, acc=buf)
+    on_ready(w)
+
+
+def flush_grouped_weight_grads():
+    while _GROUP.jobs:
+        _run_group_job_alone(_GROUP.jobs.popitem()[1])
+
+
+flush_grouped_weight_grads.run_on_failure = True
+
+
+def _wgrad_group(xa, dya, acca, xb, dyb, accb):
+    xta, xtb = xa.t(), xb.t()
+    if G.gemm_pair_supported(xta, dya, acca, xtb, dyb, accb):
+        key = ("wgrad_grp", xta.shape[0], dya.shape[1], xtb.shape[0], dyb.shape[1], xta.shape[1], acca.dtype)
+        scratch = {}
+
+        def _s(acc):
+            if id(acc) not in scratch:
+                scratch[id(acc)] = torch.zeros_like(acc)
+            return scratch[id(acc)]
+        cands = {"sep": lambda: (_wgrad(xa, dya, acc=_s(acca)), _wgrad(xb, dyb, acc=_s(accb))),
+                 "hip": lambda: G.gemm_pair(xta, dya, _s(acca), xtb, dyb, _s(accb), accumulate=(True, True))}
+        if G.choose(key, cands) == "hip":
+            G.gemm_pair(xta, dya, acca, xtb, dyb, accb, accumulate=(True, True))
+            return
+    _wgrad(xa, dya, acc=acca)
+    _wgrad(xb, dyb, acc=accb)
+
+
+def _grouped_wgrad(w, x2, dy2, buf, on_ready):
+    job = _GROUP.jobs.pop(id(w), None)
+    if job is not None:
+        if job[5]() is not w:
+            _run_group_job_alone(job)
+        else:
+            fw, fx, fdy, fbuf, fready, _ = job
+            _wgrad_group(fx, fdy, fbuf, x2, dy2, buf)
+            fready(fw)
+            on_ready(w)
+            return True
+    ent = _GROUP.partner.get(id(w))
+    if ent is None or ent[0]() is not w:
+        return False
+    second = ent[1]()
+    sent = None if second is None else _main_grad_of(second)
+    if (sent is None or not second.requires_grad or sent[1].dtype != dy2.dtype or buf.dtype != dy2.dtype
+            or not buf.is_contiguous() or not sent[1].is_contiguous()):
+        return False
+    stale = _GROUP.jobs.pop(id(second), None)
+    if stale is not None:
+        _run_group_job_alone(stale)
+    _GROUP.jobs[id(second)] = (w, x2, dy2, buf, on_ready, ent[1])
+    from ..autograd.engine import queue_callback
+    queue_callback(flush_grouped_weight_grads)
+    return True
+
+
 def _main_grad_wgrad(w, x2, dy2, buf, on_ready):
     mode = _PAIR.mode
     if mode is not None:
@@ -357,6 +442,9 @@
             return
         if mode == "defer":
             _PAIR.jobs[id(w)] = (w, x2, dy2, buf, on_ready)
+            return
+    elif (_GROUP.partner or _GROUP.jobs) and getattr(_ZB, "queue", None) is None:
+        if _grouped_wgrad(w, x2, dy2, buf, on_ready):
             return
     _wgrad(x2, dy2, acc=buf)
     on_ready(w)
diff --git a/paddlepaddle_amd/parallel/data_parallel.py b/paddlepaddle_amd/parallel/data_parallel.py
--- a/paddlepaddle_amd/parallel/data_parallel.py
+++ b/paddlepaddle_amd/parallel/data_parallel.py
@@ -136,6 +136,8 @@
                 b.work = dist.all_reduce(b.flat, op=dist.ReduceOp.SUM, group=pg, async_op=True)
 
     def _finalize(self):
+        from ..ops.linear import flush_grouped_weight_grads
+        flush_grouped_weight_grads()
         while self._next_launch < len(self._buckets):
             self._launch(self._buckets[self._order[self._next_launch]])
             self._next_launch += 1
diff --git a/paddlepaddle_amd/parallel/sharding.py b/paddlepaddle_amd/parallel/sharding.py
--- a/paddlepaddle_amd/parallel/sharding.py
+++ b/paddlepaddle_amd/parallel/sharding.py
@@ -385,6 +385,8 @@
         u.ready = set()
 
     def _finalize_backward(self):
+        from ..ops.linear import flush_grouped_weight_grads
+        flush_grouped_weight_grads()
         if not self._sync:
             for u in self.units:
                 u.ready = set()
```

Measured after the change: 13670 tokens/s (median of 6 runs). No clear change (+0.7%).
